# lmb-freiburg/neural-point-cloud-diffusion

Hardware: AMD Instinct MI355X
Metric: denoiser train steps/sec (+ rendered rays/sec under 'render'), SRN-Cars 512pt x 128d (higher is better)
Workload: dtype bf16; 1 GPU; BASELINE configs[1]: denoiser fwd/bwd + AdamW + EMA, 512 points x 128-d latents, width 1024 / 24 layers / 16 heads (seq 513), bf16 autocast; global_batch=64, per_gpu_batch=64, parallelism=dp1, rng=weights seed 1234 on every rank; timestep / noise draws seed 42 + rank

## Files before the change

include/npcd_hip.h:

```cpp
#ifndef NPCD_HIP_H
#define NPCD_HIP_H

#include <assert.h>
#include <stddef.h>
#include <stdint.h>

#ifdef __cplusplus
extern "C" {
#endif

#define NPCD_OK 0
#define NPCD_ERR_ARG (-1)
#define NPCD_ERR_UNSUPPORTED (-2)
#define NPCD_ERR_HIP (-3)

#define NPCD_BF16 0
#define NPCD_F16 1
#define NPCD_F32 2
#define NPCD_F64 3

int npcd_abi_version(void);
const char* npcd_error_string(int code);
const char* npcd_last_hip_error(void);

typedef struct npcd_attn_args {
    const void *q, *k, *v;
    void* out;
    float* lse;
    const void* dout;
    void *dq, *dk, *dv;
    float* delta;
    float* colsum_part;
    void* workspace;
    int64_t qkv_sb, qkv_sn, qkv_sh;
    int64_t out_sb, out_sn, out_sh;
    int64_t g_sb, g_sn, g_sh;
    int32_t B, n, H, d, dtype;
    float scale;
} npcd_attn_args;
static_assert(sizeof(npcd_attn_args) == 192 && offsetof(npcd_attn_args, scale) == 188, "npcd_attn_args is part of the ABI");

int64_t npcd_attn_fwd_workspace_floats(int B, int n, int H);
int npcd_attn_fwd(const npcd_attn_args* a, void* stream);

int64_t npcd_attn_fwd_fp8_workspace_bytes(int B, int n, int H);
int npcd_attn_fwd_fp8(const npcd_attn_args* a, void* stream);

int64_t npcd_attn_bwd_workspace_floats(int B, int n, int H);
int npcd_attn_bwd_colsum_rows(int B, int n, int H);
int npcd_attn_bwd(const npcd_attn_args* a, int passes, void* stream);

int64_t npcd_attn_bwd_fused_slab_floats(int B, int n, int H);
int npcd_attn_bwd_fused(const npcd_attn_args* a, void* stream);

typedef struct npcd_grid_params {
    float voxel_size[3];
    int32_t voxel_scale[3];
    int32_t kernel_size[3];
    int32_t max_points_per_voxel;
    int32_t max_occ_voxels_per_example;
    float range_min[3];
    float range_max[3];
    int32_t dims[3];
    int32_t cdims[3];
    int32_t grid_level;
} npcd_grid_params;
#define NPCD_GRID_FINE 0
#define NPCD_GRID_SCALED 1

int64_t npcd_grid_workspace_bytes(const npcd_grid_params* g, int B, int N);

int npcd_grid_build(const npcd_grid_params* g, const float* points, const int32_t* counts,
                    int B, int N, void* workspace, void* stream);

int npcd_grid_query(const npcd_grid_params* g, const void* workspace, const float* points,
                    int B, int N, int R, int S, int M, int k, float r, int mode,
                    const float* x, const float* rays_o, const float* rays_d,
                    const float* t0, const float* t1,
                    int32_t* sample_idx, float* sample_loc, int32_t* slot_sample, int32_t* nsel,
                    void* stream);

int npcd_grid_query_compact(const npcd_grid_params* g, const void* workspace, const float* points,
                            int B, int N, int R, int S, int M, int k, float r,
                            const float* rays_o, const float* rays_d, const float* t0, const float* t1,
                            int32_t* counter, int32_t capacity, int32_t* ray_base, int32_t* ray_nsel,
                            uint64_t* ray_bits, int32_t* nb_idx, float* pts, void* stream);

int64_t npcd_grid_query_order_ws_bytes(int B, int R, int M, int k);
int npcd_grid_query_compact_ordered(const npcd_grid_params* g, const void* workspace, const float* points,
                                    int B, int N, int R, int S, int M, int k, float r,
                                    const float* rays_o, const float* rays_d, const float* t0, const float* t1,
                                    int32_t* counter, int32_t capacity, int32_t* ray_base, int32_t* ray_nsel,
                                    uint64_t* ray_bits, int32_t* nb_idx, float* pts, void* order_ws, void* stream);

int64_t npcd_ray_gen_ws_floats(int V, int res, int n_ids);
int npcd_ray_gen(const float* extr, const float* intr, int V, int res, float box,
                 float* rays_o, float* rays_d, float* t0, float* t1, float* limits_ws, void* stream);
int npcd_ray_gen_subset(const float* extr, const float* intr, int V, int res, float box, const int32_t* pixel_ids, int n_ids,
                        float* rays_o, float* rays_d, float* t0, float* t1, float* limits_ws, void* stream);

#define NPCD_SHADE_NONFINITE_PAIRS 1
#define NPCD_SHADE_NONFINITE_HEADS 2
int64_t npcd_shade_wpack_bytes(int feat_dim, int n_freqs, int hidden);
int64_t npcd_shade_workspace_bytes(int max_points, int hidden);
int npcd_shade_pack_weights(const float* const* weights_host, const float* const* biases_host,
                            int feat_dim, int n_freqs, int hidden, void* wpack_host);
int npcd_shade_points(const void* wpack, int feat_dim, int n_freqs, int hidden,
                      const int32_t* nb_idx, const float* pts, const float* kp_pos, const float* kp_feat,
                      const int32_t* n_points_dev, int max_points, int k,
                      float* sigma, float* rgb, void* workspace, int32_t* status, void* stream);

int npcd_shade_points_dir(const void* wpack, int feat_dim, int n_freqs, int hidden,
                          const int32_t* nb_idx, const float* pts, const float* kp_pos, const float* kp_feat,
                          const int32_t* n_points_dev, int max_points, int k,
                          float* sigma, float* rgb, void* workspace, const float* dir_bias, const int32_t* point_ray,
                          int32_t* status, void* stream);

int64_t npcd_pairs_x2_wpack_bytes(int feat_dim);
int npcd_pairs_x2_pack(const float* const* weights_host, const float* const* biases_host, int feat_dim, void* wpack_host);
int npcd_pairs_x2(const void* wpack, int feat_dim, const int32_t* nb_idx, const float* pts, const float* kp_pos, const float* kp_feat,
                  const int32_t* n_points_dev, int max_points, int k, float* G, void* stream);
int64_t npcd_points_x2_wpack_bytes(void);
int npcd_points_x2_pack(const float* const* weights_host, const float* const* biases_host, int c0_in_dim, void* wpack_host);
int npcd_points_x2(const void* wpack, const float* feat, const int32_t* n_points_dev, int max_points, float* sigma, float* rgb,
                   const float* dir_bias, const int32_t* point_ray, void* stream);
int npcd_points_x2_train(const void* wpack, const float* feat, int max_points, float* save, float* pre, void* stream);
int npcd_points_x2_pack_dev(const float* const* weights_dev, const float* const* biases_dev, int c0_in_dim, void* wpack_dev, void* stream);

int64_t npcd_ray_march_ws_floats(int Nr);
int npcd_ray_march(const float* sigma, const float* rgb, const uint8_t* slot_valid, const float* slot_loc,
                   const int32_t* point_base, const float* rays_o, const float* rays_d, const float* t1,
                   int Nr, int M, int white_back, float* mask, float* depth, float* channels,
                   float* depth_ws, void* stream);

int npcd_ray_march_bwd(const float* sigma, const float* rgb, const uint8_t* slot_valid, const float* slot_loc,
                       const int32_t* point_base, const float* rays_o, const float* rays_d, const float* t1,
                       int Nr, int M, int white_back, const float* depth_ws, const float* g_mask, const float* g_depth,
                       const float* g_chan, float* dsigma, float* drgb, void* stream);

int npcd_add_ln_fwd_dt(const float* x_in, const void* delta, const float* gamma, const float* beta,
                       float* x_out, void* y, float* mean, float* rstd, int T, int W, float eps, int dtype, void* stream);
int npcd_ln_bwd_blocks(int T);
int npcd_ln_bwd_dt(const void* dy, const float* x, const float* mean, const float* rstd, const float* gamma,
                   const float* dres, float* dx, void* dxb, float* part_gamma, float* part_beta,
                   float* part_col, int T, int W, int dtype, void* stream);
int npcd_colsum_scratch_rows(void);
int npcd_colsum_finalize(const float* part, int nblk, int N, float* out, int accumulate, void* stream);
#define NPCD_COLSUM_MAX_JOBS 8
typedef struct NpcdColsumJob {
    const float* part;
    float* out;
    int nblk, N, accumulate, reserved;
} NpcdColsumJob;
int npcd_colsum_finalize_batch(const NpcdColsumJob* jobs, int njobs, void* stream);
int npcd_gelu_fwd_dt(const void* h, void* g, int64_t numel, int dtype, void* stream);
int npcd_colsum_blocks(int T);
int npcd_gelu_bwd_dt(const void* dg, const void* h, void* dh, float* part, int T, int N, int dtype, void* stream);
int npcd_colsum_dt(const void* a, float* part, int T, int N, int dtype, void* stream);
int npcd_small_wgrad_blocks(int T);
int npcd_small_wgrad(const void* dy, const void* x, float* part, int T, int J, int K, void* stream);
int npcd_adamw_ema_dt(float* p, float* g, float* m, float* v, float* ema, void* shadow, int shadow_dtype, int64_t numel,
                      float lr, float beta1, float beta2, float eps, float weight_decay, int step,
                      float ema_decay, int zero_grad, void* stream);
int npcd_cast_f32_dt(const float* src, void* dst, int64_t numel, int dtype, void* stream);

typedef struct NpcdScalerCtl {
    int32_t found_inf, step, growth_tracker, skipped;
    float loss_scale, inv_scale, grad_norm, clip_coef, bc1, bc2_sqrt;
    int32_t reserved[6];
} NpcdScalerCtl;
int npcd_grad_stats_blocks(void);
int npcd_grad_stats(const float* g, int64_t n, double* work, double* out, void* stream);
int npcd_scaler_finalize(const double* stats, int nslots, NpcdScalerCtl* ctl, int scaling, int clip, float max_norm,
                         float beta1, float beta2, float growth_factor, float backoff_factor, int growth_interval, void* stream);
int npcd_adamw_ema_gated(float* p, float* g, float* m, float* v, float* ema, void* shadow, int shadow_dtype, int64_t numel,
                         float lr, float beta1, float beta2, float eps, float weight_decay, double ema_decay, int zero_grad,
                         const NpcdScalerCtl* ctl, void* stream);

int npcd_wgrad_slices(int T, int N, int K);
int npcd_wgrad(const void* dy, const void* x, float* out, float* workspace, int T, int N, int K, int dtype, void* stream);
int npcd_wgrad_group(int count, const void* const* dy, const void* const* x, float* const* out, const int* N, const int* K, int T,
                     int dtype, void* stream);
int npcd_wgrad_group_blocks(int tiles_per_block, int max_products, int products_per_block);

int npcd_linear_fwd(const void* x, const void* w, const void* bias, void* y, int M, int N, int K, int dtype, void* stream);
int npcd_linear_gelu_fwd(const void* x, const void* w, const void* bias, void* h, void* g, int M, int N, int K, int dtype, void* stream);
int npcd_linear_dgelu_rows(int M);
int npcd_linear_dgelu_bwd(const void* dy, const void* wt, const void* h, void* dh, float* part, int M, int N, int K, int dtype, void* stream);
int npcd_linear128_fwd(const void* x, const void* w, const void* bias, void* y, int M, int N, int K, int dtype, void* stream);
int npcd_transpose_16(const void* in, void* out, int R, int C, void* stream);
int npcd_transpose16_group(int count, const void* const* in, void* const* out, const int* R, const int* C, void* stream);

int npcd_sum_slices(const float* part, float* out, int S, int64_t numel, void* stream);

int npcd_ddpm_reverse_step(const float* x_t, const void* eps, int eps_dtype, const float* noise, float* x_prev, float* x0_out,
                           const int64_t* t, int B, int64_t per_sample, const float* tab_recip, const float* tab_recipm1,
                           const float* tab_coef1, const float* tab_coef2, const float* tab_logvar, float clip_lo, float clip_hi,
                           int has_clip, void* stream);

#define NPCD_SAMPLER_REVERSE 0
#define NPCD_SAMPLER_HOLD 1
typedef struct NpcdSamplerTensor {
    const float* x_t;
    const void* eps;
    const float* noise;
    const float* known;
    float* out;
    float* x0_out;
    int64_t per_sample;
    float clip_lo, clip_hi;
    int32_t has_clip, mode, eps_dtype, reserved;
} NpcdSamplerTensor;
int npcd_sampler_step(const NpcdSamplerTensor* coords, const NpcdSamplerTensor* feats, const int64_t* t, const float* table, int T,
                      int B, int deterministic, void* stream);

int npcd_sampler_step_keep(const NpcdSamplerTensor* coords, const NpcdSamplerTensor* feats, const uint8_t* keep_coords,
                           const uint8_t* keep_feats, int64_t n_points, const int64_t* t, const float* table, int T, int B,
                           int deterministic, void* stream);

int npcd_sampler_step_multistep(const NpcdSamplerTensor* coords, const NpcdSamplerTensor* feats, float* hist_coords, float* hist_feats,
                                const uint8_t* keep_coords, const uint8_t* keep_feats, int64_t n_points, const int64_t* t,
                                const float* table, int T, int B, void* stream);

int npcd_q_sample(const float* x0, const float* noise, const int64_t* t, const float* tab_sqrt_acp, const float* tab_sqrt_1macp,
                  float* x_t, int B, int64_t per_sample, void* stream);
int npcd_eps_mse_blocks(void);
int npcd_eps_mse_fwd(const float* noise, const void* eps, int eps_dtype, int64_t numel, float* pointwise, float* part, float* loss,
                     void* stream);
int npcd_eps_mse_bwd(const float* noise, const void* eps, int eps_dtype, int64_t numel, const float* upstream_dev, void* grad,
                     void* stream);

int npcd_ray_march_compact(const float* sigma, const float* rgb, const uint64_t* ray_bits, const float* pts,
                           const int32_t* ray_base, const float* rays_o, const float* rays_d, const float* t1,
                           int Nr, int M, int capacity, int white_back, float* mask, float* depth, float* channels,
                           float* depth_ws, void* stream);

int64_t npcd_render_lim_words(int B, int R);
int npcd_render_rays_query(const npcd_grid_params* grid, const void* workspace, const float* points, int B, int N, const float* extr,
                           const float* intr, int views, int res, float box, int S, int M, int k, float r, float* rays_o, float* rays_d,
                           float* t0, float* t1, int32_t* counter, int32_t capacity, int32_t* ray_base, int32_t* ray_nsel,
                           uint64_t* ray_bits, int32_t* nb_idx, float* pts, void* order_ws, uint32_t* lim_part, void* stream);
int npcd_ray_march_compact_fused(const float* sigma, const float* rgb, const uint64_t* ray_bits, const float* pts, const int32_t* ray_base,
                                 const float* rays_o, const float* rays_d, const float* t0, const float* t1, const uint32_t* lim_part,
                                 int lim_pairs, int Nr, int M, int capacity, int white_back, float* mask, float* depth,
                                 float* channels, float* depth_ws, void* stream);

int npcd_pair_input_fwd(const int64_t* flat, const int64_t* owner, const float* pts, const float* kp_pos, const float* kp_feat,
                        int feat_dim, int n_freqs, int64_t n_pairs, float* x0, float* w, void* stream);
int npcd_pair_input_bwd(const int64_t* flat, const float* dx0, int feat_dim, int n_cols, int64_t n_pairs, float* dfeat, void* stream);
int npcd_leaky_bwd_blocks(int64_t rows);
int npcd_leaky_bwd_colsum(const void* dz, const void* z, void* dy, float* part, int64_t rows, int N, float slope, int dtype,
                          void* stream);
int npcd_pair_aggregate(int backward, const float* src, const float* w, const int64_t* off, const int64_t* cnt, int channels,
                        int64_t n_points, float* dst, void* stream);

#define NPCD_PAIR_MLP_BF16 0
#define NPCD_PAIR_MLP_X2 1
int64_t npcd_pair_mlp_wpack_bytes(int feat_dim, int precision);
int npcd_pair_mlp_pack(const float* const* weights_dev, const float* const* biases_dev, int feat_dim, int precision, void* wpack_dev,
                       void* stream);
int npcd_pair_mlp_fwd(const void* wpack, int feat_dim, int precision, const int64_t* nb_idx, const float* pts, const float* kp_pos,
                      const float* kp_feat, const int64_t* off, int64_t n_points, int k, int64_t n_pairs, void* x0, void* acts,
                      float* wn, float* G, void* stream);
int npcd_pair_mlp_bwd_slabs(int64_t n_pairs, int precision);
int64_t npcd_pair_mlp_bwd_workspace_floats(int feat_dim, int64_t n_pairs, int precision);
int npcd_pair_mlp_bwd(const void* wpack, int feat_dim, int precision, const float* dG, const int64_t* owner, const float* wn,
                      const void* x0, const void* acts, int64_t n_pairs, void* dact, float* dfeat, float* part, float* const* dW,
                      float* const* db, void* stream);

int npcd_split3_bf16(const float* x, const float* bias, void* out, int64_t rows, int K, int gelu, void* stream);
int npcd_add_ln_split3_bf16(const float* x, const float* o, const float* bias, const float* gamma, const float* beta, float* xnew,
                            void* out, int64_t rows, int W, float eps, void* stream);

#define NPCD_SPLIT_WEIGHTS_MAX 8
typedef struct NpcdSplitWeight {
    const float* w;
    void* fwd;
    void* dgrad;
    int N, K;
} NpcdSplitWeight;
int npcd_add_ln_split3_stats_bf16(const float* x, const float* o, const float* bias, const float* gamma, const float* beta, float* xnew,
                                  void* out, float* mean, float* rstd, int64_t rows, int W, float eps, void* stream);
int npcd_split_weights_bf16(const NpcdSplitWeight* desc, int count, void* stream);
int npcd_ln_bwd_split3_bf16(const float* dy, const float* x, const float* mean, const float* rstd, const float* gamma,
                            const float* dres, float* dx, void* dx3, float* part_gamma, float* part_beta, float* part_col, int T, int W,
                            void* stream);
int npcd_split3_colsum_bf16(const float* a, const float* h, const float* bias, void* out, float* part, int T, int N, int gelu,
                            void* stream);

int64_t npcd_stage1_reg_workspace_floats(int B);
int npcd_stage1_reg_fwd(const float* coords, const int32_t* nb, int64_t nb_ld, const float* feats, int64_t feats_ld, const float* mean,
                        const float* log_var, int64_t kl_ld, int B, int N, int k, int F, float weight_tv, float weight_kl, int dtype,
                        float* tv_pointwise, float* tv_total, float* kl_pointwise, float* kl_total, float* workspace, void* stream);
int npcd_stage1_reg_bwd(const float* coords, const int32_t* nb, int64_t nb_ld, const float* feats, int64_t feats_ld, const float* mean,
                        const float* log_var, int64_t kl_ld, int B, int N, int k, int F, float weight_tv, float weight_kl, int dtype,
                        const float* g_tv_total, const float* g_tv_pointwise, const float* g_kl_total, const float* g_kl_pointwise,
                        float* dfeats, float* dmean, float* dlog_var, void* stream);

int npcd_fps_resident_points(void);
int npcd_fps_max_points(void);
int npcd_fps(const float* points, const int32_t* lengths, const int32_t* ks, const int32_t* start, int64_t* idx_out, float* pts_out,
             int N, int P, int Kmax, void* stream);

int npcd_chamfer_max_points(void);
int npcd_chamfer_directed(const float* x, const int32_t* x_len, const float* y, const int32_t* y_len, float* out, int M, int P, int N,
                          int Q, void* stream);

int npcd_emd_max_points(void);
int npcd_emd_directed(const float* x, const int32_t* x_len, const float* y, const int32_t* y_len, float* out, int M, int P, int N, int Q,
                      void* stream);

int npcd_occupancy_max_resolution(void);
int npcd_occupancy_clouds_per_workgroup(int n, int P, int R);
int npcd_occupancy_grid(const float* points, const int32_t* lengths, const float* lattice, const uint8_t* k_lo, const uint8_t* k_hi,
                        int32_t* counts, int32_t* clouds, int32_t* cells, int n, int P, int R, void* stream);

int npcd_image_metrics_tile(int* rows_host, int* cols_host);
int64_t npcd_image_metrics_workspace_bytes(int V, int C, int H, int W, int w);
int npcd_image_metrics(const float* pred, const float* target, int V, int C, int H, int W, int64_t pred_sv, int64_t pred_sc,
                       int64_t pred_sh, int64_t pred_sw, int64_t target_sv, int64_t target_sc, int64_t target_sh, int64_t target_sw,
                       const double* taps, int w, double n, double data_range, double* workspace, double* mse, double* ssim, double* map,
                       void* stream);

int npcd_moments_tile(int* tile_host);
int npcd_moments_max_features(void);
int npcd_moments_update(const void* x, int dtype, int64_t ld, int64_t r0, int64_t r1, int D, const double* shift, double* sum, double* gram,
                        void* stream);
int npcd_moments_finish(const double* sum, const double* gram, const double* shift, int D, int64_t n, double* mean, double* cov,
                        void* stream);
int npcd_kid_tile(int* tile_host);
int64_t npcd_kid_workspace_bytes(int S, int m);
int npcd_kid_subsets(const void* fake, const void* real, int dtype, int Nf, int Nr, int D, int64_t ldf, int64_t ldr, const int32_t* idx_f,
                     const int32_t* idx_r, int S, int m, double* workspace, double* out, void* stream);

int npcd_feature_knn_max_k(void);
int64_t npcd_feature_rows_workspace_bytes(int n, int m, int k, int splits);
int npcd_feature_knn(const void* x, const void* y, int dtype, int n, int m, int D, int64_t ldx, int64_t ldy, int exclude_self, int k,
                     int splits, double* workspace, double* out, void* stream);
int npcd_feature_ball_counts(const void* x, const void* y, int dtype, int n, int m, int D, int64_t ldx, int64_t ldy, const double* rho_y,
                             int splits, double* workspace, int32_t* cnt, double* near, void* stream);

#ifdef __cplusplus
}
#endif
#endif
```

neural-point-cloud-diffusion_amd/csrc/elementwise.hip:

```cpp
#include <math.h>

#include <stdlib.h>

#include "common.h"

namespace npcd {

constexpr int kMaxChunks = 8;

template <class E>
struct V {
    typedef E x4 __attribute__((ext_vector_type(4)));
    typedef E x8 __attribute__((ext_vector_type(8)));
};
template <class X4>
__device__ __forceinline__ f32x4 to_f32(X4 v) { return f32x4{(float)v[0], (float)v[1], (float)v[2], (float)v[3]}; }
template <class E>
__device__ __forceinline__ typename V<E>::x4 from_f32(f32x4 v) { return typename V<E>::x4{(E)v[0], (E)v[1], (E)v[2], (E)v[3]}; }
__device__ __forceinline__ f32x4 bf16x4_to_f32(bf16x4 v) { return to_f32(v); }
__device__ __forceinline__ bf16x4 f32_to_bf16x4(f32x4 v) { return from_f32<__bf16>(v); }

template <class E, int NCH>
__global__ __launch_bounds__(256) void add_ln_fwd_kernel(const float* __restrict__ x_in, const E* __restrict__ delta,
                                                         const float* __restrict__ gamma, const float* __restrict__ beta,
                                                         float* __restrict__ x_out, E* __restrict__ y, float* __restrict__ mean,
                                                         float* __restrict__ rstd, int T, int W, float eps) {
    using e4 = typename V<E>::x4;
    const int lane = threadIdx.x & 63, wave = threadIdx.x >> 6;
    const int NW = gridDim.x * 4;
    int row = blockIdx.x * 4 + wave;
    if (row >= T) return;
    f32x4 gm[NCH], bt[NCH], v[NCH], nx[NCH];
    e4 nd[NCH];
#pragma unroll
    for (int ch = 0; ch < NCH; ++ch) {
        const int c = ch * 256 + lane * 4;
        gm[ch] = bt[ch] = nx[ch] = f32x4{0.f, 0.f, 0.f, 0.f};
        nd[ch] = e4{0, 0, 0, 0};
        if (c < W) {
            gm[ch] = *reinterpret_cast<const f32x4*>(gamma + c);
            bt[ch] = *reinterpret_cast<const f32x4*>(beta + c);
        }
    }
    auto load_row = [&](int r) {
        const int64_t base = (int64_t)r * W;
#pragma unroll
        for (int ch = 0; ch < NCH; ++ch) {
            const int c = ch * 256 + lane * 4;
            if (c < W) {
                nx[ch] = *reinterpret_cast<const f32x4*>(x_in + base + c);
                if (delta) nd[ch] = *reinterpret_cast<const e4*>(delta + base + c);
            }
        }
    };
    load_row(row);
    for (; row < T; row += NW) {
        const int64_t base = (int64_t)row * W;
        float s = 0.f;
#pragma unroll
        for (int ch = 0; ch < NCH; ++ch) {
            v[ch] = nx[ch];
            if (delta) v[ch] += to_f32(nd[ch]);
        }
        if (row + NW < T) load_row(row + NW);
#pragma unroll
        for (int ch = 0; ch < NCH; ++ch) {
            const int c = ch * 256 + lane * 4;
            if (c < W) {
                if (x_out) *reinterpret_cast<f32x4*>(x_out + base + c) = v[ch];
                s += (v[ch][0] + v[ch][1]) + (v[ch][2] + v[ch][3]);
            }
        }
        const float mu = wave_sum64(s) / (float)W;
        float q = 0.f;
#pragma unroll
        for (int ch = 0; ch < NCH; ++ch) {
            const int c = ch * 256 + lane * 4;
            if (c < W) {
                const f32x4 d = v[ch] - mu;
                q += (d[0] * d[0] + d[1] * d[1]) + (d[2] * d[2] + d[3] * d[3]);
            }
        }
        const float rs = rsqrtf(wave_sum64(q) / (float)W + eps);
#pragma unroll
        for (int ch = 0; ch < NCH; ++ch) {
            const int c = ch * 256 + lane * 4;
            if (c < W) *reinterpret_cast<e4*>(y + base + c) = from_f32<E>((v[ch] - mu) * rs * gm[ch] + bt[ch]);
        }
        if (lane == 0) {
            mean[row] = mu;
            rstd[row] = rs;
        }
    }
}

static inline int ln_rows_per_wave(int T) {
    const int one_round = (T + 4 * 512 - 1) / (4 * 512);
    if (one_round <= 32) return one_round < 1 ? 1 : one_round;
    return 16;
}

template <class E, int NCH, class D = E, bool SPLIT = false>
__global__ __launch_bounds__(256, 2) void ln_bwd_kernel(const D* __restrict__ dy, const float* __restrict__ x, const float* __restrict__ mean,
                                                     const float* __restrict__ rstd, const float* __restrict__ gamma,
                                                     const float* __restrict__ dres, float* __restrict__ dx, E* __restrict__ dxb,
                                                     float* __restrict__ part_gamma, float* __restrict__ part_beta,
                                                     float* __restrict__ part_col, int T, int W, int rows_per_wave) {
    using e4 = typename V<D>::x4;
    extern __shared__ __attribute__((aligned(16))) unsigned char dsmem[];
    float* red = reinterpret_cast<float*>(dsmem);
    const int lane = threadIdx.x & 63, wave = threadIdx.x >> 6;
    f32x4 ag[NCH], ab[NCH], ac[NCH];
#pragma unroll
    for (int ch = 0; ch < NCH; ++ch) ag[ch] = ab[ch] = ac[ch] = f32x4{0.f, 0.f, 0.f, 0.f};
    const int row0 = blockIdx.x * 4 + wave, NW = gridDim.x * 4;
    const int nrows = row0 < T ? min(rows_per_wave, (T - row0 + NW - 1) / NW) : 0;
    e4 dyA[NCH], dyB[NCH];
    f32x4 xA[NCH], xB[NCH], rA[NCH], rB[NCH];
    float muA = 0.f, rsA = 0.f, muB = 0.f, rsB = 0.f;
    auto load_row = [&](int row, e4 (&dyr)[NCH], f32x4 (&xr)[NCH], f32x4 (&rr2)[NCH], float& mu, float& rs) {
        const int64_t base = (int64_t)row * W;
        mu = mean[row];
        rs = rstd[row];
#pragma unroll
        for (int ch = 0; ch < NCH; ++ch) {
            const int c = ch * 256 + lane * 4;
            if (c < W) {
                dyr[ch] = *reinterpret_cast<const e4*>(dy + base + c);
                xr[ch] = *reinterpret_cast<const f32x4*>(x + base + c);
                if (dres) rr2[ch] = *reinterpret_cast<const f32x4*>(dres + base + c);
            }
        }
    };
    if (nrows > 0) load_row(row0, dyA, xA, rA, muA, rsA);
    for (int rr = 0; rr < nrows; ++rr) {
        const int row = row0 + rr * NW;
        const int64_t base = (int64_t)row * W;
        if (rr + 1 < nrows) load_row(row + NW, dyB, xB, rB, muB, rsB);
        const float mu = muA, rs = rsA;
        f32x4 gy[NCH], xh[NCH];
        float s1 = 0.f, s2 = 0.f;
#pragma unroll
        for (int ch = 0; ch < NCH; ++ch) {
            const int c = ch * 256 + lane * 4;
            gy[ch] = xh[ch] = f32x4{0.f, 0.f, 0.f, 0.f};
            if (c < W) {
                const f32x4 d = to_f32(dyA[ch]);
                xh[ch] = (xA[ch] - mu) * rs;
                ag[ch] += d * xh[ch];
                ab[ch] += d;
                gy[ch] = d * *reinterpret_cast<const f32x4*>(gamma + c);
                const f32x4 t = gy[ch] * xh[ch];
                s1 += (gy[ch][0] + gy[ch][1]) + (gy[ch][2] + gy[ch][3]);
                s2 += (t[0] + t[1]) + (t[2] + t[3]);
            }
        }
        const float c1 = wave_sum64(s1) / (float)W, c2 = wave_sum64(s2) / (float)W;
#pragma unroll
        for (int ch = 0; ch < NCH; ++ch) {
            const int c = ch * 256 + lane * 4;
            if (c < W) {
                f32x4 o = (gy[ch] - c1 - xh[ch] * c2) * rs;
                if (dres) o += rA[ch];
                *reinterpret_cast<f32x4*>(dx + base + c) = o;
                if (SPLIT && dxb) {
                    bf16x4 hi, lo;
#pragma unroll
                    for (int j = 0; j < 4; ++j) {
                        hi[j] = (__bf16)o[j];
                        lo[j] = (__bf16)(o[j] - (float)hi[j]);
                    }
                    __bf16* o3 = reinterpret_cast<__bf16*>(dxb) + 3 * base + c;
                    *reinterpret_cast<bf16x4*>(o3) = hi;
                    *reinterpret_cast<bf16x4*>(o3 + W) = lo;
                    *reinterpret_cast<bf16x4*>(o3 + 2 * W) = hi;
                } else if (dxb) {
                    *reinterpret_cast<typename V<E>::x4*>(dxb + base + c) = from_f32<E>(o);
                }
                ac[ch] += o;
            }
        }
#pragma unroll
        for (int ch = 0; ch < NCH; ++ch) {
            dyA[ch] = dyB[ch];
            xA[ch] = xB[ch];
            rA[ch] = rB[ch];
        }
        muA = muB;
        rsA = rsB;
    }
#pragma unroll
    for (int ch = 0; ch < NCH; ++ch) {
        const int c = ch * 256 + lane * 4;
        if (c < W) {
            *reinterpret_cast<f32x4*>(red + (0 * 4 + wave) * W + c) = ag[ch];
            *reinterpret_cast<f32x4*>(red + (1 * 4 + wave) * W + c) = ab[ch];
            *reinterpret_cast<f32x4*>(red + (2 * 4 + wave) * W + c) = ac[ch];
        }
    }
    __syncthreads();
    float* outs[3] = {part_gamma, part_beta, part_col};
    for (int q = 0; q < 3; ++q) {
        if (!outs[q]) continue;
        for (int c = threadIdx.x; c < W; c += 256) {
            const float* p = red + q * 4 * W + c;
            outs[q][(int64_t)blockIdx.x * W + c] = (p[0] + p[W]) + (p[2 * W] + p[3 * W]);
        }
    }
}

constexpr int kFinSlices = 16;

struct FinBatch {
    NpcdColsumJob job[NPCD_COLSUM_MAX_JOBS];
    int first1[NPCD_COLSUM_MAX_JOBS + 1];
    int first2[NPCD_COLSUM_MAX_JOBS + 1];
    int njobs;
};
__device__ __forceinline__ int fin_job(const int* first, int njobs, int bx) {
    int j = 0;
    while (j + 1 < njobs && bx >= first[j + 1]) ++j;
    return j;
}
__device__ __forceinline__ bool fin_two_stage(int nblk) { return nblk > 2 * kFinSlices; }

__global__ __launch_bounds__(256) void colsum_stage1_kernel(FinBatch fb) {
    __shared__ float red[4][64];
    const int j = fin_job(fb.first1, fb.njobs, blockIdx.x);
    const float* __restrict__ part = fb.job[j].part;
    const int nblk = fb.job[j].nblk, N = fb.job[j].N;
    if (!fin_two_stage(nblk)) return;
    float* __restrict__ stage = const_cast<float*>(part) + (int64_t)nblk * N;
    const int tx = threadIdx.x & 63, ty = threadIdx.x >> 6;
    const int c = (blockIdx.x - fb.first1[j]) * 64 + tx;
    const int per = (nblk + kFinSlices - 1) / kFinSlices;
    const int b0 = blockIdx.y * per, b1 = min(nblk, b0 + per);
    float s0 = 0.f, s1 = 0.f;
    if (c < N) {
        int b = b0 + ty;
        for (; b + 4 < b1; b += 8) {
            s0 += part[(int64_t)b * N + c];
            s1 += part[(int64_t)(b + 4) * N + c];
        }
        if (b < b1) s0 += part[(int64_t)b * N + c];
    }
    red[ty][tx] = s0 + s1;
    __syncthreads();
    if (ty == 0 && c < N) stage[(int64_t)blockIdx.y * N + c] = (red[0][tx] + red[1][tx]) + (red[2][tx] + red[3][tx]);
}

__global__ __launch_bounds__(256) void colsum_stage2_kernel(FinBatch fb) {
    const int j = fin_job(fb.first2, fb.njobs, blockIdx.x);
    const int nblk = fb.job[j].nblk, N = fb.job[j].N;
    const int c = (blockIdx.x - fb.first2[j]) * 256 + threadIdx.x;
    if (c >= N) return;
    const bool two = fin_two_stage(nblk);
    const float* __restrict__ src = two ? fb.job[j].part + (int64_t)nblk * N : fb.job[j].part;
    const int nrows = two ? kFinSlices : nblk;
    float s = 0.f;
    for (int k = 0; k < nrows; ++k) s += src[(int64_t)k * N + c];
    float* __restrict__ out = fb.job[j].out;
    out[c] = fb.job[j].accumulate ? out[c] + s : s;
}

__device__ __forceinline__ float gelu_f(float x) { return 0.5f * x * (1.f + erff(x * 0.70710678118654752f)); }
__device__ __forceinline__ float gelu_grad_f(float x) {
    return 0.5f * (1.f + erff(x * 0.70710678118654752f)) + x * 0.3989422804014327f * __expf(-0.5f * x * x);
}

__device__ __forceinline__ float gelu_fast(float x) {
    const float u = fabsf(x) * 0.70710678118654752f;
    const float t = __builtin_amdgcn_rcpf(__builtin_fmaf(0.3275911f, u, 1.f));
    const float e = __builtin_amdgcn_exp2f(x * x * -0.72134752044448170f);
    float poly = __builtin_fmaf(t, 1.061405429f, -1.453152027f);
    poly = __builtin_fmaf(poly, t, 1.421413741f);
    poly = __builtin_fmaf(poly, t, -0.284496736f);
    poly = __builtin_fmaf(poly, t, 0.254829592f);
    const float erf_abs = __builtin_fmaf(-poly * t, e, 1.f);
    return x * __builtin_fmaf(0.5f, copysignf(erf_abs, x), 0.5f);
}

template <class E, int VARIANT>
__global__ __launch_bounds__(256) void gelu_fwd_kernel(const typename V<E>::x8* __restrict__ h, typename V<E>::x8* __restrict__ g, int64_t n8) {
    using e8 = typename V<E>::x8;
    for (int64_t i = (int64_t)blockIdx.x * 256 + threadIdx.x; i < n8; i += (int64_t)gridDim.x * 256) {
        const e8 v = h[i];
        e8 o;
#pragma unroll
        for (int j = 0; j < 8; ++j) o[j] = (E)(VARIANT == 0 ? gelu_f((float)v[j]) : gelu_fast((float)v[j]));
        g[i] = o;
    }
}

static inline int col_rows(int T) {
    static const int forced = [] { const char* e = getenv("NPCD_COL_ROWS"); return e ? atoi(e) : 0; }();
    if (forced > 0) return forced;
    int r = T / 512;
    return r < 8 ? 8 : (r > 64 ? 64 : r);
}

__device__ __forceinline__ float gelu_grad_fast(float x) {
    const float u = fabsf(x) * 0.70710678118654752f;
    const float t = __builtin_amdgcn_rcpf(__builtin_fmaf(0.3275911f, u, 1.f));
    const float e = __builtin_amdgcn_exp2f(x * x * -0.72134752044448170f);
    float poly = __builtin_fmaf(t, 1.061405429f, -1.453152027f);
    poly = __builtin_fmaf(poly, t, 1.421413741f);
    poly = __builtin_fmaf(poly, t, -0.284496736f);
    poly = __builtin_fmaf(poly, t, 0.254829592f);
    const float erf_abs = __builtin_fmaf(-poly * t, e, 1.f);
    const float phi_cdf = __builtin_fmaf(0.5f, copysignf(erf_abs, x), 0.5f);
    return __builtin_fmaf(x * 0.3989422804014327f, e, phi_cdf);
}

template <class E, bool GELU, int VARIANT = 1>
__global__ __launch_bounds__(256) void colsum_kernel(const E* __restrict__ a, const E* __restrict__ hpre, E* __restrict__ out,
                                                     float* __restrict__ part, int T, int N, int rows) {
    using e8 = typename V<E>::x8;
    const int col = (blockIdx.x * 256 + threadIdx.x) * 8;
    if (col >= N) return;
    float acc[8];
#pragma unroll
    for (int j = 0; j < 8; ++j) acc[j] = 0.f;
    auto one = [&](const e8 v, const e8 hp, int64_t off) {
        e8 o;
#pragma unroll
        for (int j = 0; j < 8; ++j) {
            const float gp = VARIANT == 0 ? gelu_grad_f((float)hp[j]) : gelu_grad_fast((float)hp[j]);
            o[j] = (E)((float)v[j] * gp);
            acc[j] += (float)o[j];
        }
        *reinterpret_cast<e8*>(out + off) = o;
    };
    if (GELU && VARIANT == 2) {
        int rr = 0;
        for (; rr + 1 < rows; rr += 2) {
            const int r0 = rr * gridDim.y + blockIdx.y, r1 = r0 + gridDim.y;
            if (r1 >= T) break;
            const int64_t o0 = (int64_t)r0 * N + col, o1 = (int64_t)r1 * N + col;
            const e8 v0 = *reinterpret_cast<const e8*>(a + o0), h0 = *reinterpret_cast<const e8*>(hpre + o0);
            const e8 v1 = *reinterpret_cast<const e8*>(a + o1), h1 = *reinterpret_cast<const e8*>(hpre + o1);
            one(v0, h0, o0);
            one(v1, h1, o1);
        }
        for (; rr < rows; ++rr) {
            const int row = rr * gridDim.y + blockIdx.y;
            if (row >= T) break;
            const int64_t off = (int64_t)row * N + col;
            one(*reinterpret_cast<const e8*>(a + off), *reinterpret_cast<const e8*>(hpre + off), off);
        }
    } else {
        for (int rr = 0; rr < rows; ++rr) {
            const int row = rr * gridDim.y + blockIdx.y;
            if (row >= T) break;
            const int64_t off = (int64_t)row * N + col;
            const e8 v = (GELU && VARIANT == 3) ? __builtin_nontemporal_load(reinterpret_cast<const e8*>(a + off))
                                                    : *reinterpret_cast<const e8*>(a + off);
            if (GELU) {
                one(v, VARIANT == 3 ? __builtin_nontemporal_load(reinterpret_cast<const e8*>(hpre + off))
                                    : *reinterpret_cast<const e8*>(hpre + off), off);
            } else {
#pragma unroll
                for (int j = 0; j < 8; ++j) acc[j] += (float)v[j];
            }
        }
    }
    float* p = part + (int64_t)blockIdx.y * N + col;
    *reinterpret_cast<f32x4*>(p) = f32x4{acc[0], acc[1], acc[2], acc[3]};
    *reinterpret_cast<f32x4*>(p + 4) = f32x4{acc[4], acc[5], acc[6], acc[7]};
}

template <int J>
__global__ __launch_bounds__(256) void small_wgrad_kernel(const __bf16* __restrict__ dy, const __bf16* __restrict__ x, float* __restrict__ part,
                                                          int T, int K, int rows_per_block) {
    extern __shared__ float swg_red[];
    const int chunks = K >> 3, lanes = 256 / chunks;
    const int cc = threadIdx.x % chunks, rl = threadIdx.x / chunks;
    const int row0 = blockIdx.x * rows_per_block, row1 = min(T, row0 + rows_per_block);
    float acc[J][8];
#pragma unroll
    for (int j = 0; j < J; ++j)
#pragma unroll
        for (int i = 0; i < 8; ++i) acc[j][i] = 0.f;
    for (int row = row0 + rl; row < row1; row += lanes) {
        const bf16x8 v = *reinterpret_cast<const bf16x8*>(x + (int64_t)row * K + 8 * cc);
        float w[J];
#pragma unroll
        for (int j = 0; j < J; ++j) w[j] = (float)dy[(int64_t)row * J + j];
#pragma unroll
        for (int j = 0; j < J; ++j)
#pragma unroll
            for (int i = 0; i < 8; ++i) acc[j][i] = __builtin_fmaf(w[j], (float)v[i], acc[j][i]);
    }
#pragma unroll
    for (int j = 0; j < J; ++j)
#pragma unroll
        for (int i = 0; i < 8; ++i) swg_red[(rl * J + j) * K + 8 * cc + i] = acc[j][i];
    __syncthreads();
    for (int e = threadIdx.x; e < J * K; e += 256) {
        float sum = 0.f;
        for (int r2 = 0; r2 < lanes; ++r2) sum += swg_red[r2 * J * K + e];
        part[(int64_t)blockIdx.x * J * K + e] = sum;
    }
}

struct AdamArgs {
    float lr, beta1, beta2, eps, wd, bc1, bc2_sqrt, ema_w;
};

__device__ __forceinline__ void adamw_one(f32x4& pp, const f32x4 gg, f32x4& mm, f32x4& vv, const AdamArgs& a) {
    pp *= (1.f - a.lr * a.wd);
    mm = mm * a.beta1 + gg * (1.f - a.beta1);
    vv = vv * a.beta2 + gg * gg * (1.f - a.beta2);
    const float step = a.lr / a.bc1;
#pragma unroll
    for (int j = 0; j < 4; ++j) pp[j] -= step * (mm[j] / (sqrtf(vv[j]) / a.bc2_sqrt + a.eps));
}

template <class E, bool GATED>
__device__ __forceinline__ void adamw_ema_body(f32x4* __restrict__ p, f32x4* __restrict__ g, f32x4* __restrict__ m, f32x4* __restrict__ v,
                                               f32x4* __restrict__ ema, typename V<E>::x4* __restrict__ shadow, int64_t n4, AdamArgs a,
                                               int zero_grad, const NpcdScalerCtl* __restrict__ ctl, float skip_ema_w) {
    const int64_t stride = (int64_t)gridDim.x * 256;
    int64_t i = (int64_t)blockIdx.x * 256 + threadIdx.x;
    float gs = 1.f, gc = 1.f;
    if constexpr (GATED) {
        if (ctl->found_inf) {
            for (; i < n4; i += stride) {
                if (ema) {
                    const f32x4 e = ema[i], pp = p[i];
                    ema[i] = e + (pp - e) * skip_ema_w;
                }
                if (zero_grad) g[i] = f32x4{0.f, 0.f, 0.f, 0.f};
            }
            return;
        }
        gs = ctl->inv_scale;
        gc = ctl->clip_coef;
        a.bc1 = ctl->bc1;
        a.bc2_sqrt = ctl->bc2_sqrt;
    }
    auto grad = [&](f32x4 x) -> f32x4 {
        if constexpr (GATED) {
            x = (x * gs) * gc;
            asm volatile("" : "+v"(x));
        }
        return x;
    };
    for (; i + stride < n4; i += 2 * stride) {
        const int64_t k = i + stride;
        f32x4 p0 = p[i], p1 = p[k];
        const f32x4 g0 = grad(g[i]), g1 = grad(g[k]);
        f32x4 m0 = m[i], m1 = m[k], v0 = v[i], v1 = v[k];
        f32x4 e0 = {0.f, 0.f, 0.f, 0.f}, e1 = e0;
        if (ema) { e0 = ema[i]; e1 = ema[k]; }
        adamw_one(p0, g0, m0, v0, a);
        adamw_one(p1, g1, m1, v1, a);
        p[i] = p0; p[k] = p1;
        m[i] = m0; m[k] = m1;
        v[i] = v0; v[k] = v1;
        if (ema) { ema[i] = e0 + (p0 - e0) * a.ema_w; ema[k] = e1 + (p1 - e1) * a.ema_w; }
        if (shadow) { shadow[i] = from_f32<E>(p0); shadow[k] = from_f32<E>(p1); }
        if (zero_grad) { g[i] = f32x4{0.f, 0.f, 0.f, 0.f}; g[k] = f32x4{0.f, 0.f, 0.f, 0.f}; }
    }
    if (i < n4) {
        f32x4 pp = p[i];
        const f32x4 gg = grad(g[i]);
        f32x4 mm = m[i], vv = v[i];
        adamw_one(pp, gg, mm, vv, a);
        p[i] = pp;
        m[i] = mm;
        v[i] = vv;
        if (ema) {
            const f32x4 e = ema[i];
            ema[i] = e + (pp - e) * a.ema_w;
        }
        if (shadow) shadow[i] = from_f32<E>(pp);
        if (zero_grad) g[i] = f32x4{0.f, 0.f, 0.f, 0.f};
    }
}

template <class E>
__global__ __launch_bounds__(256) void adamw_ema_kernel(f32x4* __restrict__ p, f32x4* __restrict__ g, f32x4* __restrict__ m, f32x4* __restrict__ v,
                                                        f32x4* __restrict__ ema, typename V<E>::x4* __restrict__ shadow, int64_t n4, AdamArgs a, int zero_grad) {
    adamw_ema_body<E, false>(p, g, m, v, ema, shadow, n4, a, zero_grad, nullptr, 0.f);
}
template <class E>
__global__ __launch_bounds__(256) void adamw_ema_gated_kernel(f32x4* __restrict__ p, f32x4* __restrict__ g, f32x4* __restrict__ m,
                                                              f32x4* __restrict__ v, f32x4* __restrict__ ema, typename V<E>::x4* __restrict__ shadow,
                                                              int64_t n4, AdamArgs a, int zero_grad, const NpcdScalerCtl* __restrict__ ctl,
                                                              float skip_ema_w) {
    adamw_ema_body<E, true>(p, g, m, v, ema, shadow, n4, a, zero_grad, ctl, skip_ema_w);
}

constexpr int kStatBlocks = 512;

__device__ __forceinline__ void stat_one(float x, double& s, uint32_t& bad) {
    const bool ok = fabsf(x) <= 3.402823466e38f;
    const double d = ok ? (double)x : 0.0;
    s = fma(d, d, s);
    bad += ok ? 0u : 1u;
}
__device__ __forceinline__ void stat_four(f32x4 x, double& s, uint32_t& bad) {
#pragma unroll
    for (int j = 0; j < 4; ++j) stat_one(x[j], s, bad);
}
__device__ __forceinline__ double wave_sum_f64(double x) {
#pragma unroll
    for (int off = 32; off > 0; off >>= 1) x += __shfl_xor(x, off, 64);
    return x;
}
__device__ __forceinline__ void block_sum2(double& s, double& c) {
    __shared__ double red[2][4];
    s = wave_sum_f64(s);
    c = wave_sum_f64(c);
    if ((threadIdx.x & 63) == 0) { red[0][threadIdx.x >> 6] = s; red[1][threadIdx.x >> 6] = c; }
    __syncthreads();
    s = (red[0][0] + red[0][1]) + (red[0][2] + red[0][3]);
    c = (red[1][0] + red[1][1]) + (red[1][2] + red[1][3]);
}

__global__ __launch_bounds__(256) void grad_stats_kernel(const float* __restrict__ g, int64_t n, double* __restrict__ part) {
    const f32x4* g4 = reinterpret_cast<const f32x4*>(g);
    const int64_t n4 = n / 4, stride = (int64_t)gridDim.x * 256, gid = (int64_t)blockIdx.x * 256 + threadIdx.x;
    double s = 0.0;
    uint32_t bad = 0;
    int64_t i = gid;
    for (; i + stride < n4; i += 2 * stride) {
        const f32x4 x0 = g4[i], x1 = g4[i + stride];
        stat_four(x0, s, bad);
        stat_four(x1, s, bad);
    }
    if (i < n4) stat_four(g4[i], s, bad);
    if (gid < n - 4 * n4) stat_one(g[4 * n4 + gid], s, bad);
    double c = (double)bad;
    block_sum2(s, c);
    if (threadIdx.x == 0) { part[2 * blockIdx.x] = s; part[2 * blockIdx.x + 1] = c; }
}
__global__ __launch_bounds__(256) void grad_stats_sum_kernel(const double* __restrict__ part, int nblk, double* __restrict__ out) {
    double s = 0.0, c = 0.0;
    for (int b = threadIdx.x; b < nblk; b += 256) { s += part[2 * b]; c += part[2 * b + 1]; }
    block_sum2(s, c);
    if (threadIdx.x == 0) { out[0] = s; out[1] = c; }
}

__global__ __launch_bounds__(64) void scaler_finalize_kernel(const double* __restrict__ stats, int nslots, NpcdScalerCtl* __restrict__ ctl,
                                                             int scaling, int clip, float max_norm, float beta1, float beta2, float growth,
                                                             float backoff, int interval) {
    if (threadIdx.x != 0) return;
    double sumsq = 0.0, bad = 0.0;
    for (int k = 0; k < nslots; ++k) { sumsq += stats[2 * k]; bad += stats[2 * k + 1]; }
    NpcdScalerCtl c = *ctl;
    const float inv = scaling ? 1.f / c.loss_scale : 1.f;
    c.inv_scale = inv;
    c.found_inf = (scaling && bad > 0.0) ? 1 : 0;
    const float norm = bad > 0.0 ? INFINITY : (float)(sqrt(sumsq) * (double)inv);
    c.grad_norm = norm;
    c.clip_coef = clip ? fminf((1.f / (norm + 1e-6f)) * max_norm, 1.f) : 1.f;
    if (c.found_inf) {
        c.loss_scale *= backoff;
        c.growth_tracker = 0;
        c.skipped += 1;
    } else {
        c.step += 1;
// ... 106 lines not shown
        for (int64_t i = (int64_t)blockIdx.x * 256 + threadIdx.x; i < n4; i += (int64_t)gridDim.x * 256) {
            const f32x4 kn = reinterpret_cast<const f32x4*>(known)[i], z = reinterpret_cast<const f32x4*>(noise)[i];
            f32x4 o;
#pragma unroll
            for (int q = 0; q < 4; ++q) o[q] = __builtin_fmaf(k.h1, kn[q], k.h2 * z[q]);
            reinterpret_cast<f32x4*>(out)[i] = o;
        }
    } else {
        for (int64_t i = (int64_t)blockIdx.x * 256 + threadIdx.x; i < a.per_sample; i += (int64_t)gridDim.x * 256)
            out[i] = __builtin_fmaf(k.h1, known[i], k.h2 * noise[i]);
    }
}

__device__ __forceinline__ SamplerCoef sampler_coef(const int64_t* __restrict__ t, const float* __restrict__ table, int T, int b) {
    const int64_t ts = t[b];
    const float nan = __builtin_nanf("");
    SamplerCoef k{nan, nan, nan, nan, nan, nan, nan};
    if (ts >= 0 && ts < T) {
        const f32x4 lo = reinterpret_cast<const f32x4*>(table)[2 * ts], hi = reinterpret_cast<const f32x4*>(table)[2 * ts + 1];
        k = SamplerCoef{lo[0], lo[1], lo[2], lo[3], hi[0], hi[1], hi[2]};
    }
    return k;
}

__device__ __forceinline__ void sampler_by_mode(const NpcdSamplerTensor& a, int vec, const SamplerCoef& k, int64_t base) {
    if (a.mode == NPCD_SAMPLER_HOLD) {
        if (vec) sampler_hold<true>(a, k, base);
        else sampler_hold<false>(a, k, base);
    } else if (a.eps_dtype == NPCD_F32) {
        if (vec) sampler_reverse<float, true>(a, k, base);
        else sampler_reverse<float, false>(a, k, base);
    } else {
        if (vec) sampler_reverse<__bf16, true>(a, k, base);
        else sampler_reverse<__bf16, false>(a, k, base);
    }
}

__global__ __launch_bounds__(256) void sampler_step_kernel(SamplerArgs args, const int64_t* __restrict__ t, const float* __restrict__ table, int T) {
    const int z = blockIdx.z, b = blockIdx.y;
    const NpcdSamplerTensor& a = args.tz[z];
    sampler_by_mode(a, args.vec[z], sampler_coef(t, table, T, b), (int64_t)b * a.per_sample);
}

__device__ __forceinline__ int64_t sampler_col(int64_t i, int64_t n) {
    return ((uint64_t)(i | n) >> 32) == 0 ? (int64_t)((uint32_t)i % (uint32_t)n) : i % n;
}

template <class EPS, bool VEC>
__device__ __forceinline__ void sampler_keep(const NpcdSamplerTensor& a, const uint8_t* __restrict__ keep, int64_t n_points, int det,
                                             const SamplerCoef& k, int64_t base) {
    const float* __restrict__ x_t = a.x_t + base;
    const EPS* __restrict__ eps = static_cast<const EPS*>(a.eps) + base;
    const float* __restrict__ noise = a.noise + base;
    const float* __restrict__ known = a.known + base;
    float* __restrict__ out = a.out + base;
    float* __restrict__ x0_out = a.x0_out ? a.x0_out + base : nullptr;
    if constexpr (VEC) {
        const int64_t n4 = a.per_sample / 4, row4 = n_points / 4;
        for (int64_t i = (int64_t)blockIdx.x * 256 + threadIdx.x; i < n4; i += (int64_t)gridDim.x * 256) {
            const uint32_t m = reinterpret_cast<const uint32_t*>(keep)[sampler_col(i, row4)];
            const f32x4 x = reinterpret_cast<const f32x4*>(x_t)[i];
            const f32x4 e = to_f32(reinterpret_cast<const typename V<EPS>::x4*>(eps)[i]);
            const f32x4 z = reinterpret_cast<const f32x4*>(noise)[i], kn = reinterpret_cast<const f32x4*>(known)[i];
            f32x4 x0, o;
#pragma unroll
            for (int q = 0; q < 4; ++q) {
                const float f0 = sampler_x0(k, x[q], e[q], a.has_clip, a.clip_lo, a.clip_hi);
                float fo = __builtin_fmaf(k.c1, f0, k.c2 * x[q]);
                if (!det) fo = __builtin_fmaf(k.s, z[q], fo);
                const bool kept = ((m >> (8 * q)) & 0xffu) != 0;
                x0[q] = kept ? kn[q] : f0;
                o[q] = kept ? __builtin_fmaf(k.h1, kn[q], k.h2 * z[q]) : fo;
            }
            if (x0_out) reinterpret_cast<f32x4*>(x0_out)[i] = x0;
            reinterpret_cast<f32x4*>(out)[i] = o;
        }
    } else {
        for (int64_t i = (int64_t)blockIdx.x * 256 + threadIdx.x; i < a.per_sample; i += (int64_t)gridDim.x * 256) {
            const bool kept = keep[sampler_col(i, n_points)] != 0;
            const float x = x_t[i], z = noise[i], kn = known[i];
            const float f0 = sampler_x0(k, x, (float)eps[i], a.has_clip, a.clip_lo, a.clip_hi);
            float fo = __builtin_fmaf(k.c1, f0, k.c2 * x);
            if (!det) fo = __builtin_fmaf(k.s, z, fo);
            if (x0_out) x0_out[i] = kept ? kn : f0;
            out[i] = kept ? __builtin_fmaf(k.h1, kn, k.h2 * z) : fo;
        }
    }
}

struct SamplerKeepArgs {
    NpcdSamplerTensor tz[2];
    const uint8_t* keep[2];
    int64_t n_points;
    int vec[2];
    int det;
};

__global__ __launch_bounds__(256) void sampler_step_keep_kernel(SamplerKeepArgs args, const int64_t* __restrict__ t, const float* __restrict__ table,
                                                                int T) {
    const int z = blockIdx.z, b = blockIdx.y;
    const NpcdSamplerTensor& a = args.tz[z];
    const int vec = args.vec[z];
    const SamplerCoef k = sampler_coef(t, table, T, b);
    const int64_t base = (int64_t)b * a.per_sample;
    if (!args.keep[z]) {
        sampler_by_mode(a, vec, k, base);
        return;
    }
    const uint8_t* keep = args.keep[z] + (int64_t)b * args.n_points;
    if (a.eps_dtype == NPCD_F32) {
        if (vec) sampler_keep<float, true>(a, keep, args.n_points, args.det, k, base);
        else sampler_keep<float, false>(a, keep, args.n_points, args.det, k, base);
    } else {
        if (vec) sampler_keep<__bf16, true>(a, keep, args.n_points, args.det, k, base);
        else sampler_keep<__bf16, false>(a, keep, args.n_points, args.det, k, base);
    }
}

__device__ __forceinline__ float sampler_multistep_d(float w, float x0, float h) { return __builtin_fmaf(w, x0 - h, x0); }

template <class EPS, bool VEC, bool KEEP>
__device__ __forceinline__ void sampler_multistep(const NpcdSamplerTensor& a, float* __restrict__ hist, const uint8_t* __restrict__ keep,
                                                  int64_t n_points, const SamplerCoef& k, float w, int64_t base) {
    const float* __restrict__ x_t = a.x_t + base;
    const EPS* __restrict__ eps = static_cast<const EPS*>(a.eps) + base;
    const float* __restrict__ noise = KEEP ? a.noise + base : nullptr;
    const float* __restrict__ known = KEEP ? a.known + base : nullptr;
    float* __restrict__ out = a.out + base;
    float* __restrict__ x0_out = a.x0_out ? a.x0_out + base : nullptr;
    hist += base;
    const bool first_order = w == 0.f;
    if constexpr (VEC) {
        const int64_t n4 = a.per_sample / 4, row4 = KEEP ? n_points / 4 : 1;
        for (int64_t i = (int64_t)blockIdx.x * 256 + threadIdx.x; i < n4; i += (int64_t)gridDim.x * 256) {
            const f32x4 x = reinterpret_cast<const f32x4*>(x_t)[i];
            const f32x4 e = to_f32(reinterpret_cast<const typename V<EPS>::x4*>(eps)[i]);
            f32x4 h = f32x4{0.f, 0.f, 0.f, 0.f}, z = h, kn = h;
            if (!first_order) h = reinterpret_cast<const f32x4*>(hist)[i];
            uint32_t m = 0;
            if constexpr (KEEP) {
                m = reinterpret_cast<const uint32_t*>(keep)[sampler_col(i, row4)];
                z = reinterpret_cast<const f32x4*>(noise)[i];
                kn = reinterpret_cast<const f32x4*>(known)[i];
            }
            f32x4 x0, o;
#pragma unroll
            for (int q = 0; q < 4; ++q) {
                const float f0 = sampler_x0(k, x[q], e[q], a.has_clip, a.clip_lo, a.clip_hi);
                const float d = first_order ? f0 : sampler_multistep_d(w, f0, h[q]);
                const float fo = __builtin_fmaf(k.c1, d, k.c2 * x[q]);
                const bool kept = KEEP && ((m >> (8 * q)) & 0xffu) != 0;
                x0[q] = kept ? kn[q] : f0;
                o[q] = kept ? __builtin_fmaf(k.h1, kn[q], k.h2 * z[q]) : fo;
            }
            if (x0_out) reinterpret_cast<f32x4*>(x0_out)[i] = x0;
            reinterpret_cast<f32x4*>(hist)[i] = x0;
            reinterpret_cast<f32x4*>(out)[i] = o;
        }
    } else {
        for (int64_t i = (int64_t)blockIdx.x * 256 + threadIdx.x; i < a.per_sample; i += (int64_t)gridDim.x * 256) {
            const float x = x_t[i];
            const float f0 = sampler_x0(k, x, (float)eps[i], a.has_clip, a.clip_lo, a.clip_hi);
            const float d = first_order ? f0 : sampler_multistep_d(w, f0, hist[i]);
            float o = __builtin_fmaf(k.c1, d, k.c2 * x), x0 = f0;
            if constexpr (KEEP) {
                if (keep[sampler_col(i, n_points)] != 0) {
                    x0 = known[i];
                    o = __builtin_fmaf(k.h1, x0, k.h2 * noise[i]);
                }
            }
            if (x0_out) x0_out[i] = x0;
            hist[i] = x0;
            out[i] = o;
        }
    }
}

struct SamplerMultistepArgs {
    NpcdSamplerTensor tz[2];
    float* hist[2];
    const uint8_t* keep[2];
    int64_t n_points;
    int vec[2];
};

template <class EPS>
__device__ __forceinline__ void sampler_multistep_by_path(const NpcdSamplerTensor& a, float* hist, const uint8_t* keep, int64_t n_points, int vec,
                                                          const SamplerCoef& k, float w, int64_t base) {
    if (keep) {
        if (vec) sampler_multistep<EPS, true, true>(a, hist, keep, n_points, k, w, base);
        else sampler_multistep<EPS, false, true>(a, hist, keep, n_points, k, w, base);
    } else {
        if (vec) sampler_multistep<EPS, true, false>(a, hist, keep, n_points, k, w, base);
        else sampler_multistep<EPS, false, false>(a, hist, keep, n_points, k, w, base);
    }
}

__global__ __launch_bounds__(256) void sampler_step_multistep_kernel(SamplerMultistepArgs args, const int64_t* __restrict__ t,
                                                                     const float* __restrict__ table, int T) {
    const int z = blockIdx.z, b = blockIdx.y;
    const NpcdSamplerTensor& a = args.tz[z];
    const SamplerCoef k = sampler_coef(t, table, T, b);
    const int64_t base = (int64_t)b * a.per_sample;
    if (!args.keep[z] && a.mode == NPCD_SAMPLER_HOLD) {
        if (args.vec[z]) sampler_hold<true>(a, k, base);
        else sampler_hold<false>(a, k, base);
        return;
    }
    const int64_t ts = t[b];
    const float w = (ts >= 0 && ts < T) ? table[8 * ts + 7] : __builtin_nanf("");
    const uint8_t* keep = args.keep[z] ? args.keep[z] + (int64_t)b * args.n_points : nullptr;
    if (a.eps_dtype == NPCD_F32) sampler_multistep_by_path<float>(a, args.hist[z], keep, args.n_points, args.vec[z], k, w, base);
    else sampler_multistep_by_path<__bf16>(a, args.hist[z], keep, args.n_points, args.vec[z], k, w, base);
}

static bool al16(const void* p) { return (reinterpret_cast<uintptr_t>(p) & 15) == 0; }

}

using namespace npcd;

static inline int ln_fwd_blocks(int T) { const int b = (T + 3) / 4; return b < 2048 ? b : 2048; }

static inline bool dt16(int dtype) { return dtype == NPCD_BF16 || dtype == NPCD_F16; }

extern "C" int npcd_add_ln_fwd_dt(const float* x_in, const void* delta, const float* gamma, const float* beta, float* x_out, void* y,
                                  float* mean, float* rstd, int T, int W, float eps, int dtype, void* stream) {
    if (!x_in || !gamma || !beta || !y || !mean || !rstd || T <= 0 || W <= 0) return NPCD_ERR_ARG;
    if (W % 4 != 0 || W > 256 * kMaxChunks || !dt16(dtype)) return NPCD_ERR_UNSUPPORTED;
    if (!al16(x_in) || !al16(gamma) || !al16(beta) || (x_out && !al16(x_out)) || (reinterpret_cast<uintptr_t>(y) & 7) ||
        (delta && (reinterpret_cast<uintptr_t>(delta) & 7)))
        return NPCD_ERR_ARG;
#define NPCD_LAUNCH_LN_FWD(E, NCH)                                                                                            \
    hipLaunchKernelGGL((add_ln_fwd_kernel<E, NCH>), dim3(ln_fwd_blocks(T)), dim3(256), 0, static_cast<hipStream_t>(stream), x_in, \
                       static_cast<const E*>(delta), gamma, beta, x_out, static_cast<E*>(y), mean, rstd, T, W, eps)
#define NPCD_LN_FWD_W(E)                     \
    do {                                     \
        if (W <= 256) NPCD_LAUNCH_LN_FWD(E, 1);      \
        else if (W <= 512) NPCD_LAUNCH_LN_FWD(E, 2); \
        else if (W <= 1024) NPCD_LAUNCH_LN_FWD(E, 4);\
        else NPCD_LAUNCH_LN_FWD(E, 8);               \
    } while (0)
    if (dtype == NPCD_BF16) NPCD_LN_FWD_W(__bf16);
    else NPCD_LN_FWD_W(_Float16);
#undef NPCD_LN_FWD_W
#undef NPCD_LAUNCH_LN_FWD
    NPCD_HIP_CHECK(hipGetLastError());
    return NPCD_OK;
}

extern "C" int npcd_ln_bwd_blocks(int T) { const int r = ln_rows_per_wave(T); return (T + 4 * r - 1) / (4 * r); }

extern "C" int npcd_ln_bwd_dt(const void* dy, const float* x, const float* mean, const float* rstd, const float* gamma, const float* dres,
                              float* dx, void* dxb, float* part_gamma, float* part_beta, float* part_col, int T, int W, int dtype, void* stream) {
    if (!dy || !x || !mean || !rstd || !gamma || !dx || T <= 0 || W <= 0) return NPCD_ERR_ARG;
    if (W % 4 != 0 || W > 256 * kMaxChunks || !dt16(dtype)) return NPCD_ERR_UNSUPPORTED;
    if (!al16(x) || !al16(gamma) || !al16(dx) || (dres && !al16(dres))) return NPCD_ERR_ARG;
    const int nblk = npcd_ln_bwd_blocks(T);
    const size_t lds = (size_t)3 * 4 * W * sizeof(float);
    hipStream_t st = static_cast<hipStream_t>(stream);
    static DynLds lds_attr_b, lds_attr_h;
    if (dtype == NPCD_BF16) NPCD_HIP_CHECK(lds_attr_b.ensure(reinterpret_cast<const void*>(ln_bwd_kernel<__bf16, 8>), 3 * 4 * 2048 * 4));
    else NPCD_HIP_CHECK(lds_attr_h.ensure(reinterpret_cast<const void*>(ln_bwd_kernel<_Float16, 8>), 3 * 4 * 2048 * 4));
#define NPCD_LAUNCH_LN_BWD(E, NCH)                                                                                             \
    hipLaunchKernelGGL((ln_bwd_kernel<E, NCH>), dim3(nblk), dim3(256), lds, st, static_cast<const E*>(dy), x, mean, rstd, gamma, \
                       dres, dx, static_cast<E*>(dxb), part_gamma, part_beta, part_col, T, W, ln_rows_per_wave(T))
#define NPCD_LN_BWD_W(E)                     \
    do {                                     \
        if (W <= 256) NPCD_LAUNCH_LN_BWD(E, 1);      \
        else if (W <= 512) NPCD_LAUNCH_LN_BWD(E, 2); \
        else if (W <= 1024) NPCD_LAUNCH_LN_BWD(E, 4);\
        else NPCD_LAUNCH_LN_BWD(E, 8);               \
    } while (0)
    if (dtype == NPCD_BF16) NPCD_LN_BWD_W(__bf16);
    else NPCD_LN_BWD_W(_Float16);
#undef NPCD_LN_BWD_W
#undef NPCD_LAUNCH_LN_BWD
    NPCD_HIP_CHECK(hipGetLastError());
    return NPCD_OK;
}
extern "C" int npcd_ln_bwd_split3_bf16(const float* dy, const float* x, const float* mean, const float* rstd, const float* gamma,
                                       const float* dres, float* dx, void* dx3, float* part_gamma, float* part_beta, float* part_col, int T,
                                       int W, void* stream) {
    if (!dy || !x || !mean || !rstd || !gamma || !dx || T <= 0 || W <= 0) return NPCD_ERR_ARG;
    if (W % 4 != 0 || W > 256 * kMaxChunks) return NPCD_ERR_UNSUPPORTED;
    if (!al16(dy) || !al16(x) || !al16(gamma) || !al16(dx) || (dres && !al16(dres)) || (dx3 && !al16(dx3))) return NPCD_ERR_ARG;
    const int nblk = npcd_ln_bwd_blocks(T);
    const size_t lds = (size_t)3 * 4 * W * sizeof(float);
    hipStream_t st = static_cast<hipStream_t>(stream);
    static DynLds lds_attr;
    NPCD_HIP_CHECK(lds_attr.ensure(reinterpret_cast<const void*>(ln_bwd_kernel<__bf16, 8, float, true>), 3 * 4 * 2048 * 4));
#define NPCD_LAUNCH_LN_BWD3(NCH)                                                                                                        \
    hipLaunchKernelGGL((ln_bwd_kernel<__bf16, NCH, float, true>), dim3(nblk), dim3(256), lds, st, dy, x, mean, rstd, gamma, dres, dx, \
                       static_cast<__bf16*>(dx3), part_gamma, part_beta, part_col, T, W, ln_rows_per_wave(T))
    if (W <= 256) NPCD_LAUNCH_LN_BWD3(1);
    else if (W <= 512) NPCD_LAUNCH_LN_BWD3(2);
    else if (W <= 1024) NPCD_LAUNCH_LN_BWD3(4);
    else NPCD_LAUNCH_LN_BWD3(8);
#undef NPCD_LAUNCH_LN_BWD3
    NPCD_HIP_CHECK(hipGetLastError());
    return NPCD_OK;
}


__global__ __launch_bounds__(1024) void colsum_onepass_kernel(FinBatch fb) {
    __shared__ float red[16][64];
    const int j = fin_job(fb.first1, fb.njobs, blockIdx.x);
    const float* __restrict__ part = fb.job[j].part;
    const int nblk = fb.job[j].nblk, N = fb.job[j].N;
    const int tx = threadIdx.x & 63, ty = threadIdx.x >> 6;
    const int c = (blockIdx.x - fb.first1[j]) * 64 + tx;
    float s0 = 0.f, s1 = 0.f;
    if (c < N) {
        int b = ty;
        for (; b + 16 < nblk; b += 32) {
            s0 += part[(int64_t)b * N + c];
            s1 += part[(int64_t)(b + 16) * N + c];
        }
        if (b < nblk) s0 += part[(int64_t)b * N + c];
    }
    red[ty][tx] = s0 + s1;
    __syncthreads();
    if (ty == 0 && c < N) {
        float q[4];
#pragma unroll
        for (int g = 0; g < 4; ++g) q[g] = (red[4 * g][tx] + red[4 * g + 1][tx]) + (red[4 * g + 2][tx] + red[4 * g + 3][tx]);
        const float s = (q[0] + q[1]) + (q[2] + q[3]);
        float* __restrict__ out = fb.job[j].out;
        out[c] = fb.job[j].accumulate ? out[c] + s : s;
    }
}

extern "C" int npcd_colsum_scratch_rows(void) { return kFinSlices; }

extern "C" int npcd_colsum_finalize_batch(const NpcdColsumJob* jobs, int njobs, void* stream) {
    if (!jobs || njobs <= 0 || njobs > NPCD_COLSUM_MAX_JOBS) return NPCD_ERR_ARG;
    FinBatch fb;
    fb.njobs = njobs;
    bool any_two_stage = false;
    int n1 = 0, n2 = 0;
    for (int j = 0; j < njobs; ++j) {
        if (!jobs[j].part || !jobs[j].out || jobs[j].nblk <= 0 || jobs[j].N <= 0) return NPCD_ERR_ARG;
        fb.job[j] = jobs[j];
        fb.first1[j] = n1;
        fb.first2[j] = n2;
        n1 += (jobs[j].N + 63) / 64;
        n2 += (jobs[j].N + 255) / 256;
        any_two_stage |= jobs[j].nblk > 2 * kFinSlices;
    }
    for (int j = njobs; j <= NPCD_COLSUM_MAX_JOBS; ++j) { fb.first1[j] = n1; fb.first2[j] = n2; }
    hipStream_t st = static_cast<hipStream_t>(stream);
    static const bool onepass = [] { const char* e = getenv("NPCD_COLSUM_ONEPASS"); return e && atoi(e) > 0; }();
    if (onepass) {
        hipLaunchKernelGGL(colsum_onepass_kernel, dim3(n1), dim3(1024), 0, st, fb);
        NPCD_HIP_CHECK(hipGetLastError());
        return NPCD_OK;
    }
    if (any_two_stage) hipLaunchKernelGGL(colsum_stage1_kernel, dim3(n1, kFinSlices), dim3(256), 0, st, fb);
    hipLaunchKernelGGL(colsum_stage2_kernel, dim3(n2), dim3(256), 0, st, fb);
    NPCD_HIP_CHECK(hipGetLastError());
    return NPCD_OK;
}

extern "C" int npcd_colsum_finalize(const float* part, int nblk, int N, float* out, int accumulate, void* stream) {
    NpcdColsumJob job;
    job.part = part; job.out = out; job.nblk = nblk; job.N = N; job.accumulate = accumulate; job.reserved = 0;
    return npcd_colsum_finalize_batch(&job, 1, stream);
}

extern "C" int npcd_gelu_fwd_dt(const void* h, void* g, int64_t numel, int dtype, void* stream) {
    if (!h || !g || numel <= 0) return NPCD_ERR_ARG;
    if (numel % 8 != 0 || !al16(h) || !al16(g) || !dt16(dtype)) return NPCD_ERR_UNSUPPORTED;
    const int64_t n8 = numel / 8;
    const int grid = (int)((n8 + 255) / 256 < 16384 ? (n8 + 255) / 256 : 16384);
    static const int variant = [] { const char* e = getenv("NPCD_GELU_FWD_VARIANT"); return e ? atoi(e) : 1; }();
    hipStream_t st = static_cast<hipStream_t>(stream);
#define NPCD_LAUNCH_GELU_FWD(E, VV)                                                                                                 \
    hipLaunchKernelGGL((gelu_fwd_kernel<E, VV>), dim3(grid), dim3(256), 0, st, static_cast<const typename V<E>::x8*>(h), \
                       static_cast<typename V<E>::x8*>(g), n8)
    if (dtype == NPCD_BF16) {
        if (variant == 0) NPCD_LAUNCH_GELU_FWD(__bf16, 0);
        else NPCD_LAUNCH_GELU_FWD(__bf16, 1);
    } else {
        NPCD_LAUNCH_GELU_FWD(_Float16, 1);
    }
#undef NPCD_LAUNCH_GELU_FWD
    NPCD_HIP_CHECK(hipGetLastError());
    return NPCD_OK;
}

extern "C" int npcd_colsum_blocks(int T) { const int r = col_rows(T); return (T + r - 1) / r; }

extern "C" int npcd_gelu_bwd_dt(const void* dg, const void* h, void* dh, float* part, int T, int N, int dtype, void* stream) {
    if (!dg || !h || !dh || !part || T <= 0 || N <= 0) return NPCD_ERR_ARG;
    if (N % 8 != 0 || !al16(dg) || !al16(h) || !al16(dh) || !al16(part) || !dt16(dtype)) return NPCD_ERR_UNSUPPORTED;
    dim3 grid((N / 8 + 255) / 256, npcd_colsum_blocks(T));
    static const int variant = [] { const char* e = getenv("NPCD_GELU_BWD_VARIANT"); return e ? atoi(e) : 1; }();
#define NPCD_LAUNCH_GELU_BWD(E, VV)                                                                                                    \
    hipLaunchKernelGGL((colsum_kernel<E, true, VV>), grid, dim3(256), 0, static_cast<hipStream_t>(stream), static_cast<const E*>(dg), \
                       static_cast<const E*>(h), static_cast<E*>(dh), part, T, N, col_rows(T))
    if (dtype == NPCD_F16) NPCD_LAUNCH_GELU_BWD(_Float16, 1);
    else if (variant == 0) NPCD_LAUNCH_GELU_BWD(__bf16, 0);
    else if (variant == 2) NPCD_LAUNCH_GELU_BWD(__bf16, 2);
    else if (variant == 3) NPCD_LAUNCH_GELU_BWD(__bf16, 3);
    else NPCD_LAUNCH_GELU_BWD(__bf16, 1);
#undef NPCD_LAUNCH_GELU_BWD
    NPCD_HIP_CHECK(hipGetLastError());
    return NPCD_OK;
}

extern "C" int npcd_colsum_dt(const void* a, float* part, int T, int N, int dtype, void* stream) {
    if (!a || !part || T <= 0 || N <= 0) return NPCD_ERR_ARG;
    if (N % 8 != 0 || !al16(a) || !al16(part) || !dt16(dtype)) return NPCD_ERR_UNSUPPORTED;
    dim3 grid((N / 8 + 255) / 256, npcd_colsum_blocks(T));
    if (dtype == NPCD_BF16)
        hipLaunchKernelGGL((colsum_kernel<__bf16, false>), grid, dim3(256), 0, static_cast<hipStream_t>(stream), static_cast<const __bf16*>(a),
                           static_cast<const __bf16*>(nullptr), static_cast<__bf16*>(nullptr), part, T, N, col_rows(T));
    else
        hipLaunchKernelGGL((colsum_kernel<_Float16, false>), grid, dim3(256), 0, static_cast<hipStream_t>(stream), static_cast<const _Float16*>(a),
                           static_cast<const _Float16*>(nullptr), static_cast<_Float16*>(nullptr), part, T, N, col_rows(T));
    NPCD_HIP_CHECK(hipGetLastError());
    return NPCD_OK;
}

extern "C" int npcd_small_wgrad_blocks(int T) { return T <= 0 ? -1 : (T + 255) / 256 < 1024 ? (T + 255) / 256 : 1024; }

extern "C" int npcd_small_wgrad(const void* dy, const void* x, float* part, int T, int J, int K, void* stream) {
    if (!dy || !x || !part || T <= 0) return NPCD_ERR_ARG;
    if (J < 1 || J > 4 || K < 64 || K > 2048 || (K & (K - 1)) || !al16(x) || !al16(part)) return NPCD_ERR_UNSUPPORTED;
    const int nblk = npcd_small_wgrad_blocks(T), rpb = (T + nblk - 1) / nblk;
    const size_t lds = (size_t)(256 / (K / 8)) * J * K * sizeof(float);
    hipStream_t st = static_cast<hipStream_t>(stream);
    const __bf16* d = static_cast<const __bf16*>(dy);
    const __bf16* xx = static_cast<const __bf16*>(x);
    switch (J) {
        case 1: hipLaunchKernelGGL(small_wgrad_kernel<1>, dim3(nblk), dim3(256), lds, st, d, xx, part, T, K, rpb); break;
        case 2: hipLaunchKernelGGL(small_wgrad_kernel<2>, dim3(nblk), dim3(256), lds, st, d, xx, part, T, K, rpb); break;
        case 3: hipLaunchKernelGGL(small_wgrad_kernel<3>, dim3(nblk), dim3(256), lds, st, d, xx, part, T, K, rpb); break;
        default: hipLaunchKernelGGL(small_wgrad_kernel<4>, dim3(nblk), dim3(256), lds, st, d, xx, part, T, K, rpb); break;
    }
    NPCD_HIP_CHECK(hipGetLastError());
    return NPCD_OK;
}

extern "C" int npcd_adamw_ema_dt(float* p, float* g, float* m, float* v, float* ema, void* shadow, int shadow_dtype, int64_t numel, float lr,
                                 float beta1, float beta2, float eps, float weight_decay, int step, float ema_decay, int zero_grad, void* stream) {
    if (!p || !g || !m || !v || numel <= 0 || step <= 0) return NPCD_ERR_ARG;
    if (numel % 4 != 0 || !al16(p) || !al16(g) || !al16(m) || !al16(v) || (ema && !al16(ema)) ||
        (shadow && ((reinterpret_cast<uintptr_t>(shadow) & 7) || !dt16(shadow_dtype))))
        return NPCD_ERR_UNSUPPORTED;
    AdamArgs a;
    a.lr = lr; a.beta1 = beta1; a.beta2 = beta2; a.eps = eps; a.wd = weight_decay;
    a.bc1 = (float)(1.0 - pow((double)beta1, (double)step));
    a.bc2_sqrt = (float)sqrt(1.0 - pow((double)beta2, (double)step));
    a.ema_w = 1.f - ema_decay;
    const int64_t n4 = numel / 4;
    const int grid = (int)((n4 + 255) / 256 < 8192 ? (n4 + 255) / 256 : 8192);
    hipStream_t st = static_cast<hipStream_t>(stream);
    if (shadow && shadow_dtype == NPCD_F16)
        hipLaunchKernelGGL(adamw_ema_kernel<_Float16>, dim3(grid), dim3(256), 0, st, reinterpret_cast<f32x4*>(p), reinterpret_cast<f32x4*>(g),
                           reinterpret_cast<f32x4*>(m), reinterpret_cast<f32x4*>(v), reinterpret_cast<f32x4*>(ema),
                           static_cast<V<_Float16>::x4*>(shadow), n4, a, zero_grad);
    else
        hipLaunchKernelGGL(adamw_ema_kernel<__bf16>, dim3(grid), dim3(256), 0, st, reinterpret_cast<f32x4*>(p), reinterpret_cast<f32x4*>(g),
                           reinterpret_cast<f32x4*>(m), reinterpret_cast<f32x4*>(v), reinterpret_cast<f32x4*>(ema),
                           static_cast<V<__bf16>::x4*>(shadow), n4, a, zero_grad);
    NPCD_HIP_CHECK(hipGetLastError());
    return NPCD_OK;
}

extern "C" int npcd_adamw_ema_gated(float* p, float* g, float* m, float* v, float* ema, void* shadow, int shadow_dtype, int64_t numel, float lr,
                                    float beta1, float beta2, float eps, float weight_decay, double ema_decay, int zero_grad,
                                    const NpcdScalerCtl* ctl, void* stream) {
    if (!p || !g || !m || !v || !ctl || numel <= 0) return NPCD_ERR_ARG;
    if (numel % 4 != 0 || !al16(p) || !al16(g) || !al16(m) || !al16(v) || (ema && !al16(ema)) || (reinterpret_cast<uintptr_t>(ctl) & 15) ||
        (shadow && ((reinterpret_cast<uintptr_t>(shadow) & 7) || !dt16(shadow_dtype))))
        return NPCD_ERR_UNSUPPORTED;
    AdamArgs a;
    a.lr = lr; a.beta1 = beta1; a.beta2 = beta2; a.eps = eps; a.wd = weight_decay;
    a.bc1 = 1.f; a.bc2_sqrt = 1.f;
    a.ema_w = 1.f - (float)ema_decay;
    const float skip_w = (float)(1.0 - ema_decay);
    const int64_t n4 = numel / 4;
    const int grid = (int)((n4 + 255) / 256 < 8192 ? (n4 + 255) / 256 : 8192);
    hipStream_t st = static_cast<hipStream_t>(stream);
    if (shadow && shadow_dtype == NPCD_F16)
        hipLaunchKernelGGL(adamw_ema_gated_kernel<_Float16>, dim3(grid), dim3(256), 0, st, reinterpret_cast<f32x4*>(p), reinterpret_cast<f32x4*>(g),
                           reinterpret_cast<f32x4*>(m), reinterpret_cast<f32x4*>(v), reinterpret_cast<f32x4*>(ema),
                           static_cast<V<_Float16>::x4*>(shadow), n4, a, zero_grad, ctl, skip_w);
    else
        hipLaunchKernelGGL(adamw_ema_gated_kernel<__bf16>, dim3(grid), dim3(256), 0, st, reinterpret_cast<f32x4*>(p), reinterpret_cast<f32x4*>(g),
                           reinterpret_cast<f32x4*>(m), reinterpret_cast<f32x4*>(v), reinterpret_cast<f32x4*>(ema),
                           static_cast<V<__bf16>::x4*>(shadow), n4, a, zero_grad, ctl, skip_w);
    NPCD_HIP_CHECK(hipGetLastError());
    return NPCD_OK;
}

extern "C" int npcd_grad_stats_blocks(void) { return kStatBlocks; }

extern "C" int npcd_grad_stats(const float* g, int64_t n, double* work, double* out, void* stream) {
    if (!g || !work || !out || n <= 0) return NPCD_ERR_ARG;
    if (!al16(g) || (reinterpret_cast<uintptr_t>(work) & 7) || (reinterpret_cast<uintptr_t>(out) & 7)) return NPCD_ERR_UNSUPPORTED;
    const int64_t n4 = n / 4, want = (n4 + 511) / 512;
    const int grid = (int)(want < 1 ? 1 : want < kStatBlocks ? want : kStatBlocks);
    hipStream_t st = static_cast<hipStream_t>(stream);
    hipLaunchKernelGGL(grad_stats_kernel, dim3(grid), dim3(256), 0, st, g, n, work);
    hipLaunchKernelGGL(grad_stats_sum_kernel, dim3(1), dim3(256), 0, st, work, grid, out);
    NPCD_HIP_CHECK(hipGetLastError());
    return NPCD_OK;
}

extern "C" int npcd_scaler_finalize(const double* stats, int nslots, NpcdScalerCtl* ctl, int scaling, int clip, float max_norm, float beta1,
                                    float beta2, float growth_factor, float backoff_factor, int growth_interval, void* stream) {
    if (!stats || !ctl || nslots <= 0 || growth_interval <= 0) return NPCD_ERR_ARG;
    if ((reinterpret_cast<uintptr_t>(stats) & 7) || (reinterpret_cast<uintptr_t>(ctl) & 15)) return NPCD_ERR_UNSUPPORTED;
    hipLaunchKernelGGL(scaler_finalize_kernel, dim3(1), dim3(64), 0, static_cast<hipStream_t>(stream), stats, nslots, ctl, scaling, clip, max_norm,
                       beta1, beta2, growth_factor, backoff_factor, growth_interval);
    NPCD_HIP_CHECK(hipGetLastError());
    return NPCD_OK;
}

extern "C" int npcd_ddpm_reverse_step(const float* x_t, const void* eps, int eps_dtype, const float* noise, float* x_prev, float* x0_out,
                                      const int64_t* t, int B, int64_t per_sample, const float* tab_recip, const float* tab_recipm1,
                                      const float* tab_coef1, const float* tab_coef2, const float* tab_logvar, float clip_lo, float clip_hi,
                                      int has_clip, void* stream) {
    if (!x_t || !eps || !noise || !x_prev || !t || B <= 0 || per_sample <= 0) return NPCD_ERR_ARG;
    if (!tab_recip || !tab_recipm1 || !tab_coef1 || !tab_coef2 || !tab_logvar) return NPCD_ERR_ARG;
    if (eps_dtype != NPCD_F32 && eps_dtype != NPCD_BF16) return NPCD_ERR_UNSUPPORTED;
    const DdpmTables tab{tab_recip, tab_recipm1, tab_coef1, tab_coef2, tab_logvar};
    const int gx = (int)((per_sample + 255) / 256 < 1024 ? (per_sample + 255) / 256 : 1024);
    hipStream_t st = static_cast<hipStream_t>(stream);
    if (eps_dtype == NPCD_F32)
        hipLaunchKernelGGL(ddpm_reverse_kernel<float>, dim3(gx, B), dim3(256), 0, st, x_t, static_cast<const float*>(eps), noise, x_prev, x0_out, t,
                           per_sample, tab, clip_lo, clip_hi, has_clip);
    else
        hipLaunchKernelGGL(ddpm_reverse_kernel<__bf16>, dim3(gx, B), dim3(256), 0, st, x_t, static_cast<const __bf16*>(eps), noise, x_prev, x0_out, t,
                           per_sample, tab, clip_lo, clip_hi, has_clip);
    NPCD_HIP_CHECK(hipGetLastError());
    return NPCD_OK;
}

static int sampler_check_mode(const NpcdSamplerTensor& a, int deterministic, bool* vec_out) {
    if (!a.out || a.per_sample <= 0) return NPCD_ERR_ARG;
    bool vec = a.per_sample % 4 == 0 && al16(a.out);
    if (a.mode == NPCD_SAMPLER_HOLD) {
        if (!a.known || !a.noise) return NPCD_ERR_ARG;
        vec = vec && al16(a.known) && al16(a.noise);
    } else if (a.mode == NPCD_SAMPLER_REVERSE) {
        if (!a.x_t || !a.eps || (!a.noise && !deterministic)) return NPCD_ERR_ARG;
        if (a.eps_dtype != NPCD_F32 && a.eps_dtype != NPCD_BF16) return NPCD_ERR_UNSUPPORTED;
        vec = vec && al16(a.x_t) && (!a.noise || al16(a.noise)) && (!a.x0_out || al16(a.x0_out)) &&
              (reinterpret_cast<uintptr_t>(a.eps) & (a.eps_dtype == NPCD_F32 ? 15 : 7)) == 0;
    } else {
        return NPCD_ERR_ARG;
    }
    *vec_out = vec;
    return NPCD_OK;
}

static int sampler_grid(const NpcdSamplerTensor& a, bool vec) {
    const int64_t items = vec ? a.per_sample / 4 : a.per_sample;
    return (int)((items + 255) / 256 < 1024 ? (items + 255) / 256 : 1024);
}

extern "C" int npcd_sampler_step(const NpcdSamplerTensor* coords, const NpcdSamplerTensor* feats, const int64_t* t, const float* table, int T,
                                 int B, int deterministic, void* stream) {
    if (!coords || !feats || !t || !table || T <= 0 || B <= 0) return NPCD_ERR_ARG;
    if (B > 65535 || !al16(table)) return NPCD_ERR_UNSUPPORTED;
    SamplerArgs args;
    int gx = 1;
    for (int z = 0; z < 2; ++z) {
        const NpcdSamplerTensor& a = z ? *feats : *coords;
        bool vec = false;
        const int rc = sampler_check_mode(a, deterministic, &vec);
        if (rc != NPCD_OK) return rc;
        args.tz[z] = a;
        args.vec[z] = vec ? 1 : 0;
        const int g = sampler_grid(a, vec);
        gx = g > gx ? g : gx;
    }
    hipLaunchKernelGGL(sampler_step_kernel, dim3(gx, B, 2), dim3(256), 0, static_cast<hipStream_t>(stream), args, t, table, T);
    NPCD_HIP_CHECK(hipGetLastError());
    return NPCD_OK;
}

extern "C" int npcd_sampler_step_keep(const NpcdSamplerTensor* coords, const NpcdSamplerTensor* feats, const uint8_t* keep_coords,
                                      const uint8_t* keep_feats, int64_t n_points, const int64_t* t, const float* table, int T, int B,
                                      int deterministic, void* stream) {
    if (!coords || !feats || !t || !table || T <= 0 || B <= 0 || n_points <= 0) return NPCD_ERR_ARG;
    if (B > 65535 || !al16(table)) return NPCD_ERR_UNSUPPORTED;
    SamplerKeepArgs args;
    args.n_points = n_points;
    args.det = deterministic ? 1 : 0;
    int gx = 1;
    for (int z = 0; z < 2; ++z) {
        const NpcdSamplerTensor& a = z ? *feats : *coords;
        const uint8_t* keep = z ? keep_feats : keep_coords;
        bool vec = false;
        if (!keep) {
            const int rc = sampler_check_mode(a, deterministic, &vec);
            if (rc != NPCD_OK) return rc;
        } else {
            if (!a.out || !a.x_t || !a.eps || !a.noise || !a.known || a.per_sample <= 0 || a.per_sample % n_points != 0) return NPCD_ERR_ARG;
            if (a.eps_dtype != NPCD_F32 && a.eps_dtype != NPCD_BF16) return NPCD_ERR_UNSUPPORTED;
            vec = n_points % 4 == 0 && (reinterpret_cast<uintptr_t>(keep) & 3) == 0 && al16(a.out) && al16(a.x_t) && al16(a.noise) &&
                  al16(a.known) && (!a.x0_out || al16(a.x0_out)) &&
                  (reinterpret_cast<uintptr_t>(a.eps) & (a.eps_dtype == NPCD_F32 ? 15 : 7)) == 0;
        }
        args.tz[z] = a;
        args.keep[z] = keep;
        args.vec[z] = vec ? 1 : 0;
        const int g = sampler_grid(a, vec);
        gx = g > gx ? g : gx;
    }
    hipLaunchKernelGGL(sampler_step_keep_kernel, dim3(gx, B, 2), dim3(256), 0, static_cast<hipStream_t>(stream), args, t, table, T);
    NPCD_HIP_CHECK(hipGetLastError());
    return NPCD_OK;
}

extern "C" int npcd_sampler_step_multistep(const NpcdSamplerTensor* coords, const NpcdSamplerTensor* feats, float* hist_coords,
                                           float* hist_feats, const uint8_t* keep_coords, const uint8_t* keep_feats, int64_t n_points,
                                           const int64_t* t, const float* table, int T, int B, void* stream) {
    if (!coords || !feats || !t || !table || T <= 0 || B <= 0) return NPCD_ERR_ARG;
    if ((keep_coords || keep_feats) && n_points <= 0) return NPCD_ERR_ARG;
    if (B > 65535 || !al16(table)) return NPCD_ERR_UNSUPPORTED;
    SamplerMultistepArgs args;
    args.n_points = n_points;
    int gx = 1;
    for (int z = 0; z < 2; ++z) {
        const NpcdSamplerTensor& a = z ? *feats : *coords;
        const uint8_t* keep = z ? keep_feats : keep_coords;
        float* hist = z ? hist_feats : hist_coords;
        bool vec = false;
        if (!keep) {
            const int rc = sampler_check_mode(a, 1, &vec);
            if (rc != NPCD_OK) return rc;
        } else {
            if (!a.out || !a.x_t || !a.eps || !a.noise || !a.known || a.per_sample <= 0 || a.per_sample % n_points != 0) return NPCD_ERR_ARG;
            if (a.eps_dtype != NPCD_F32 && a.eps_dtype != NPCD_BF16) return NPCD_ERR_UNSUPPORTED;
            vec = n_points % 4 == 0 && (reinterpret_cast<uintptr_t>(keep) & 3) == 0 && al16(a.out) && al16(a.x_t) && al16(a.noise) &&
                  al16(a.known) && (!a.x0_out || al16(a.x0_out)) &&
                  (reinterpret_cast<uintptr_t>(a.eps) & (a.eps_dtype == NPCD_F32 ? 15 : 7)) == 0;
        }
        if (keep || a.mode != NPCD_SAMPLER_HOLD) {
            if (!hist) return NPCD_ERR_ARG;
            vec = vec && al16(hist);
        }
        args.tz[z] = a;
        args.hist[z] = hist;
        args.keep[z] = keep;
        args.vec[z] = vec ? 1 : 0;
        const int g = sampler_grid(a, vec);
        gx = g > gx ? g : gx;
    }
    hipLaunchKernelGGL(sampler_step_multistep_kernel, dim3(gx, B, 2), dim3(256), 0, static_cast<hipStream_t>(stream), args, t, table, T);
    NPCD_HIP_CHECK(hipGetLastError());
    return NPCD_OK;
}

namespace npcd {
__global__ __launch_bounds__(256) void q_sample_kernel(const float* __restrict__ x0, const float* __restrict__ noise, const int64_t* __restrict__ t,
                                                       const float* __restrict__ tab_a, const float* __restrict__ tab_s, float* __restrict__ xt,
                                                       int64_t per_sample) {
#pragma clang fp contract(off)
    const int b = blockIdx.y;
    const float ca = tab_a[t[b]], cs = tab_s[t[b]];
    const int64_t base = (int64_t)b * per_sample;
    for (int64_t i = (int64_t)blockIdx.x * 256 + threadIdx.x; i < per_sample; i += (int64_t)gridDim.x * 256) {
        const float p0 = ca * x0[base + i], p1 = cs * noise[base + i];
// ... 109 lines not shown
```

neural-point-cloud-diffusion_amd/npcd/hip/__init__.py:

```python
import ctypes
import os
from ctypes import POINTER, c_char_p, c_double, c_float, c_int, c_int32, c_int64, c_void_p

import torch

_PKG_ROOT = os.path.dirname(os.path.dirname(os.path.dirname(os.path.abspath(__file__))))
LIB_PATH = os.environ.get("NPCD_HIP_LIB") or os.path.join(_PKG_ROOT, "lib", "libnpcd_hip.so")

NPCD_BF16, NPCD_F16, NPCD_F32 = 0, 1, 2
NPCD_F64 = 3
NPCD_GRID_FINE, NPCD_GRID_SCALED = 0, 1
_DTYPE_CODE = {torch.bfloat16: NPCD_BF16, torch.float16: NPCD_F16, torch.float32: NPCD_F32}


class GridParams(ctypes.Structure):
    _fields_ = [("voxel_size", c_float * 3), ("voxel_scale", c_int32 * 3), ("kernel_size", c_int32 * 3),
                ("max_points_per_voxel", c_int32), ("max_occ_voxels_per_example", c_int32),
                ("range_min", c_float * 3), ("range_max", c_float * 3), ("dims", c_int32 * 3), ("cdims", c_int32 * 3),
                ("grid_level", c_int32)]


_P = c_void_p
SIGNATURES = {
    "npcd_abi_version": (c_int, []),
    "npcd_error_string": (c_char_p, [c_int]),
    "npcd_last_hip_error": (c_char_p, []),
    "npcd_attn_fwd": (c_int, [_P, _P]),
    "npcd_attn_fwd_workspace_floats": (c_int64, [c_int, c_int, c_int]),
    "npcd_ray_march_bwd": (c_int, [_P] * 8 + [c_int, c_int, c_int] + [_P] * 6 + [_P]),
    "npcd_leaky_bwd_blocks": (c_int, [c_int64]),
    "npcd_leaky_bwd_colsum": (c_int, [_P, _P, _P, _P, c_int64, c_int, c_float, c_int, _P]),
    "npcd_pair_input_fwd": (c_int, [_P] * 5 + [c_int, c_int, c_int64, _P, _P, _P]),
    "npcd_pair_input_bwd": (c_int, [_P, _P, c_int, c_int, c_int64, _P, _P]),
    "npcd_pair_aggregate": (c_int, [c_int, _P, _P, _P, _P, c_int, c_int64, _P, _P]),
    "npcd_attn_bwd": (c_int, [_P, c_int, _P]),
    "npcd_attn_bwd_workspace_floats": (c_int64, [c_int, c_int, c_int]),
    "npcd_attn_bwd_colsum_rows": (c_int, [c_int, c_int, c_int]),
    "npcd_attn_fwd_fp8_workspace_bytes": (c_int64, [c_int, c_int, c_int]),
    "npcd_attn_fwd_fp8": (c_int, [_P, _P]),
    "npcd_attn_bwd_fused_slab_floats": (c_int64, [c_int, c_int, c_int]),
    "npcd_attn_bwd_fused": (c_int, [_P, _P]),
    "npcd_grid_workspace_bytes": (c_int64, [POINTER(GridParams), c_int, c_int]),
    "npcd_grid_build": (c_int, [POINTER(GridParams), _P, _P, c_int, c_int, _P, _P]),
    "npcd_grid_query": (c_int, [POINTER(GridParams), _P, _P] + [c_int] * 6 + [c_float, c_int] + [_P] * 9 + [_P]),
    "npcd_grid_query_compact": (c_int, [POINTER(GridParams), _P, _P] + [c_int] * 6 + [c_float] + [_P] * 5 + [c_int32] + [_P] * 5 + [_P]),
    "npcd_grid_query_compact_ordered": (c_int, [POINTER(GridParams), _P, _P] + [c_int] * 6 + [c_float] + [_P] * 5 + [c_int32] + [_P] * 5
                                        + [_P, _P]),
    "npcd_grid_query_order_ws_bytes": (c_int64, [c_int] * 4),
    "npcd_ray_march_compact": (c_int, [_P] * 8 + [c_int, c_int, c_int, c_int] + [_P] * 4 + [_P]),
    "npcd_render_lim_words": (c_int64, [c_int, c_int]),
    "npcd_render_rays_query": (c_int, [POINTER(GridParams), _P, _P, c_int, c_int, _P, _P, c_int, c_int, c_float, c_int, c_int, c_int, c_float]
                               + [_P] * 5 + [c_int32] + [_P] * 7 + [_P]),
    "npcd_ray_march_compact_fused": (c_int, [_P] * 10 + [c_int, c_int, c_int, c_int, c_int] + [_P] * 4 + [_P]),
    "npcd_ray_gen": (c_int, [_P, _P, c_int, c_int, c_float] + [_P] * 5 + [_P]),
    "npcd_ray_gen_subset": (c_int, [_P, _P, c_int, c_int, c_float, _P, c_int] + [_P] * 5 + [_P]),
    "npcd_shade_wpack_bytes": (c_int64, [c_int, c_int, c_int]),
    "npcd_shade_workspace_bytes": (c_int64, [c_int, c_int]),
    "npcd_shade_pack_weights": (c_int, [POINTER(_P), POINTER(_P), c_int, c_int, c_int, _P]),
    "npcd_pairs_x2_wpack_bytes": (c_int64, [c_int]),
    "npcd_pairs_x2_pack": (c_int, [POINTER(_P), POINTER(_P), c_int, _P]),
    "npcd_pairs_x2": (c_int, [_P, c_int, _P, _P, _P, _P, _P, c_int, c_int, _P, _P]),
    "npcd_points_x2_wpack_bytes": (c_int64, []),
    "npcd_points_x2_pack": (c_int, [POINTER(_P), POINTER(_P), c_int, _P]),
    "npcd_points_x2": (c_int, [_P, _P, _P, c_int, _P, _P, _P, _P, _P]),
    "npcd_points_x2_train": (c_int, [_P, _P, c_int, _P, _P, _P]),
    "npcd_points_x2_pack_dev": (c_int, [POINTER(_P), POINTER(_P), c_int, _P, _P]),
    "npcd_shade_points": (c_int, [_P, c_int, c_int, c_int] + [_P] * 5 + [c_int, c_int] + [_P] * 3 + [_P] + [_P]),
    "npcd_shade_points_dir": (c_int, [_P, c_int, c_int, c_int] + [_P] * 5 + [c_int, c_int] + [_P] * 3 + [_P, _P] + [_P] + [_P]),
    "npcd_ray_march_ws_floats": (c_int64, [c_int]),
    "npcd_ray_gen_ws_floats": (c_int64, [c_int, c_int, c_int]),
    "npcd_ray_march": (c_int, [_P] * 8 + [c_int, c_int, c_int] + [_P] * 4 + [_P]),
    "npcd_ln_bwd_blocks": (c_int, [c_int]),
    "npcd_colsum_scratch_rows": (c_int, []),
    "npcd_colsum_finalize": (c_int, [_P, c_int, c_int, _P, c_int, _P]),
    "npcd_colsum_finalize_batch": (c_int, [_P, c_int, _P]),
    "npcd_ddpm_reverse_step": (c_int, [_P, _P, c_int, _P, _P, _P, _P, c_int, c_int64, _P, _P, _P, _P, _P, c_float, c_float, c_int, _P]),
    "npcd_sampler_step": (c_int, [_P, _P, _P, _P, c_int, c_int, c_int, _P]),
    "npcd_sampler_step_keep": (c_int, [_P, _P, _P, _P, c_int64, _P, _P, c_int, c_int, c_int, _P]),
    "npcd_sampler_step_multistep": (c_int, [_P, _P, _P, _P, _P, _P, c_int64, _P, _P, c_int, c_int, _P]),
    "npcd_colsum_blocks": (c_int, [c_int]),
    "npcd_add_ln_fwd_dt": (c_int, [_P] * 8 + [c_int, c_int, c_float, c_int, _P]),
    "npcd_ln_bwd_dt": (c_int, [_P] * 11 + [c_int, c_int, c_int, _P]),
    "npcd_gelu_fwd_dt": (c_int, [_P, _P, c_int64, c_int, _P]),
    "npcd_gelu_bwd_dt": (c_int, [_P, _P, _P, _P, c_int, c_int, c_int, _P]),
    "npcd_colsum_dt": (c_int, [_P, _P, c_int, c_int, c_int, _P]),
    "npcd_adamw_ema_dt": (c_int, [_P] * 6 + [c_int, c_int64] + [c_float] * 5 + [c_int, c_float, c_int, _P]),
    "npcd_cast_f32_dt": (c_int, [_P, _P, c_int64, c_int, _P]),
    "npcd_grad_stats_blocks": (c_int, []),
    "npcd_grad_stats": (c_int, [_P, c_int64, _P, _P, _P]),
    "npcd_scaler_finalize": (c_int, [_P, c_int, _P, c_int, c_int] + [c_float] * 5 + [c_int, _P]),
    "npcd_adamw_ema_gated": (c_int, [_P] * 6 + [c_int, c_int64] + [c_float] * 5 + [c_double, c_int, _P, _P]),
    "npcd_wgrad_slices": (c_int, [c_int, c_int, c_int]),
    "npcd_wgrad": (c_int, [_P, _P, _P, _P, c_int, c_int, c_int, c_int, _P]),
    "npcd_wgrad_group": (c_int, [c_int, POINTER(_P), POINTER(_P), POINTER(_P), POINTER(c_int), POINTER(c_int), c_int, c_int, _P]),
    "npcd_wgrad_group_blocks": (c_int, [c_int, c_int, c_int]),
    "npcd_sum_slices": (c_int, [_P, _P, c_int, c_int64, _P]),
    "npcd_linear_fwd": (c_int, [_P, _P, _P, _P, c_int, c_int, c_int, c_int, _P]),
    "npcd_linear128_fwd": (c_int, [_P, _P, _P, _P, c_int, c_int, c_int, c_int, _P]),
    "npcd_linear_gelu_fwd": (c_int, [_P, _P, _P, _P, _P, c_int, c_int, c_int, c_int, _P]),
    "npcd_linear_dgelu_rows": (c_int, [c_int]),
    "npcd_linear_dgelu_bwd": (c_int, [_P, _P, _P, _P, _P, c_int, c_int, c_int, c_int, _P]),
    "npcd_transpose_16": (c_int, [_P, _P, c_int, c_int, _P]),
    "npcd_transpose16_group": (c_int, [c_int, POINTER(_P), POINTER(_P), POINTER(c_int), POINTER(c_int), _P]),
    "npcd_small_wgrad_blocks": (c_int, [c_int]),
    "npcd_small_wgrad": (c_int, [_P, _P, _P, c_int, c_int, c_int, _P]),
    "npcd_q_sample": (c_int, [_P] * 6 + [c_int, c_int64, _P]),
    "npcd_eps_mse_blocks": (c_int, []),
    "npcd_eps_mse_fwd": (c_int, [_P, _P, c_int, c_int64, _P, _P, _P, _P]),
    "npcd_eps_mse_bwd": (c_int, [_P, _P, c_int, c_int64, _P, _P, _P]),
    "npcd_split3_bf16": (c_int, [_P, _P, _P, c_int64, c_int, c_int, _P]),
    "npcd_add_ln_split3_bf16": (c_int, [_P] * 7 + [c_int64, c_int, c_float, _P]),
    "npcd_add_ln_split3_stats_bf16": (c_int, [_P] * 9 + [c_int64, c_int, c_float, _P]),
    "npcd_split_weights_bf16": (c_int, [_P, c_int, _P]),
    "npcd_ln_bwd_split3_bf16": (c_int, [_P] * 11 + [c_int, c_int, _P]),
    "npcd_split3_colsum_bf16": (c_int, [_P] * 5 + [c_int, c_int, c_int, _P]),
    "npcd_pair_mlp_wpack_bytes": (c_int64, [c_int, c_int]),
    "npcd_pair_mlp_pack": (c_int, [POINTER(_P), POINTER(_P), c_int, c_int, _P, _P]),
    "npcd_pair_mlp_fwd": (c_int, [_P, c_int, c_int] + [_P] * 5 + [c_int64, c_int, c_int64] + [_P] * 4 + [_P]),
    "npcd_pair_mlp_bwd_slabs": (c_int, [c_int64, c_int]),
    "npcd_pair_mlp_bwd_workspace_floats": (c_int64, [c_int, c_int64, c_int]),
    "npcd_pair_mlp_bwd": (c_int, [_P, c_int, c_int] + [_P] * 5 + [c_int64] + [_P] * 3 + [POINTER(_P), POINTER(_P), _P]),
    "npcd_stage1_reg_workspace_floats": (c_int64, [c_int]),
    "npcd_stage1_reg_fwd": (c_int, [_P, _P, c_int64, _P, c_int64, _P, _P, c_int64] + [c_int] * 4 + [c_float, c_float, c_int] + [_P] * 5 + [_P]),
    "npcd_stage1_reg_bwd": (c_int, [_P, _P, c_int64, _P, c_int64, _P, _P, c_int64] + [c_int] * 4 + [c_float, c_float, c_int] + [_P] * 7 + [_P]),
    "npcd_fps_resident_points": (c_int, []),
    "npcd_fps_max_points": (c_int, []),
    "npcd_fps": (c_int, [_P] * 6 + [c_int, c_int, c_int, _P]),
    "npcd_chamfer_max_points": (c_int, []),
    "npcd_chamfer_directed": (c_int, [_P] * 5 + [c_int] * 4 + [_P]),
    "npcd_emd_max_points": (c_int, []),
    "npcd_emd_directed": (c_int, [_P] * 5 + [c_int] * 4 + [_P]),
    "npcd_occupancy_max_resolution": (c_int, []),
    "npcd_occupancy_clouds_per_workgroup": (c_int, [c_int, c_int, c_int]),
    "npcd_occupancy_grid": (c_int, [_P] * 8 + [c_int] * 3 + [_P]),
    "npcd_image_metrics_tile": (c_int, [POINTER(c_int), POINTER(c_int)]),
    "npcd_image_metrics_workspace_bytes": (c_int64, [c_int] * 5),
    "npcd_image_metrics": (c_int, [_P, _P] + [c_int] * 4 + [c_int64] * 8 + [_P, c_int, c_double, c_double] + [_P] * 4 + [_P]),
    "npcd_moments_tile": (c_int, [POINTER(c_int)]),
    "npcd_moments_max_features": (c_int, []),
    "npcd_moments_update": (c_int, [_P, c_int, c_int64, c_int64, c_int64, c_int, _P, _P, _P, _P]),
    "npcd_moments_finish": (c_int, [_P, _P, _P, c_int, c_int64, _P, _P, _P]),
    "npcd_kid_tile": (c_int, [POINTER(c_int)]),
    "npcd_kid_workspace_bytes": (c_int64, [c_int, c_int]),
    "npcd_kid_subsets": (c_int, [_P, _P, c_int, c_int, c_int, c_int, c_int64, c_int64, _P, _P, c_int, c_int, _P, _P, _P]),
    "npcd_feature_knn_max_k": (c_int, []),
    "npcd_feature_rows_workspace_bytes": (c_int64, [c_int] * 4),
    "npcd_feature_knn": (c_int, [_P, _P, c_int, c_int, c_int, c_int, c_int64, c_int64, c_int, c_int, c_int, _P, _P, _P]),
    "npcd_feature_ball_counts": (c_int, [_P, _P, c_int, c_int, c_int, c_int, c_int64, c_int64, _P, c_int, _P, _P, _P, _P]),
}

_lib = None


def lib() -> ctypes.CDLL:
    global _lib
    if _lib is None:
        if not os.path.exists(LIB_PATH):
            raise RuntimeError(
                f"libnpcd_hip.so not found at {LIB_PATH}: build it with "
                f"`python neural-point-cloud-diffusion_amd/csrc/build.py` (or __graft_entry__.build()). "
                f"There is no CPU / PyTorch fallback for the NPCD hot path.")
        handle = ctypes.CDLL(LIB_PATH)
        missing = []
        for name, (res, args) in SIGNATURES.items():
            try:
                fn = getattr(handle, name)
            except AttributeError:
                missing.append(name)
                continue
            fn.restype, fn.argtypes = res, args
        handle.npcd_missing = tuple(missing)
        _lib = handle
    return _lib


def check(rc: int, what: str):
    if rc != 0:
        L = lib()
        msg = L.npcd_error_string(rc).decode()
        if rc == -3:
            msg += ": " + L.npcd_last_hip_error().decode()
        raise RuntimeError(f"{what} failed: {msg} (code {rc})")


def require_gpu(*tensors: torch.Tensor):
    for t in tensors:
        if t is not None and not t.is_cuda:
            raise RuntimeError("npcd.hip operators need GPU tensors (MI355X); got a tensor on "
                               f"{t.device}. There is no CPU fallback in the product path.")


def dtype_code(t: torch.Tensor) -> int:
    try:
        return _DTYPE_CODE[t.dtype]
    except KeyError:
        raise RuntimeError(f"unsupported dtype {t.dtype}") from None


def ptr(t):
    return c_void_p(0 if t is None else t.data_ptr())


_raw_stream = getattr(torch._C, "_cuda_getCurrentRawStream", None)


def stream_ptr():
    if _raw_stream is not None:
        return c_void_p(_raw_stream(torch.cuda.current_device()))
    return c_void_p(torch.cuda.current_stream().cuda_stream)
```

neural-point-cloud-diffusion_amd/npcd/hip/elementwise.py:

```python
import ctypes

import torch

from . import arena, check, dtype_code, lib, ptr, require_gpu, stream_ptr

_f32, _bf16, _f16 = torch.float32, torch.bfloat16, torch.float16
MAX_JOBS = 8

KERNEL_EVENTS = None


def _timed(tag, fn):
    if KERNEL_EVENTS is None or tag not in KERNEL_EVENTS:
        return fn()
    e0, e1 = torch.cuda.Event(enable_timing=True), torch.cuda.Event(enable_timing=True)
    e0.record()
    rc = fn()
    e1.record()
    KERNEL_EVENTS[tag].append((e0, e1))
    return rc


class ColsumJob(ctypes.Structure):
    _fields_ = [("part", ctypes.c_void_p), ("out", ctypes.c_void_p), ("nblk", ctypes.c_int), ("N", ctypes.c_int),
                ("accumulate", ctypes.c_int), ("reserved", ctypes.c_int)]


class ColsumBatch:

    def __init__(self):
        self.jobs = []

    def add(self, part, nblk, N, out, accumulate=False):
        self.jobs.append((part, nblk, N, out, accumulate))

    def flush(self):
        L, s = lib(), stream_ptr()
        for i in range(0, len(self.jobs), MAX_JOBS):
            chunk = self.jobs[i:i + MAX_JOBS]
            arr = (ColsumJob * len(chunk))()
            for a, (part, nblk, N, out, acc) in zip(arr, chunk):
                a.part, a.out, a.nblk, a.N, a.accumulate, a.reserved = part.data_ptr(), out.data_ptr(), nblk, N, int(acc), 0
            check(L.npcd_colsum_finalize_batch(ctypes.cast(arr, ctypes.c_void_p), len(chunk), s), "npcd_colsum_finalize_batch")
        self.jobs = []


def _finish(batch, part, nblk, N, out):
    if batch is not None:
        batch.add(part, nblk, N, out)
    else:
        check(lib().npcd_colsum_finalize(ptr(part), nblk, N, ptr(out), 0, stream_ptr()), "npcd_colsum_finalize")


def add_ln_fwd(x_in, delta, gamma, beta, eps=1e-5, want_sum=True, dtype=_bf16):
    require_gpu(x_in)
    T, W = x_in.shape
    dev = x_in.device
    if delta is not None:
        dtype = delta.dtype
    x_out = arena.empty_like(x_in) if (delta is not None and want_sum) else None
    y = arena.empty((T, W), dtype, dev)
    mean = arena.empty(T, _f32, dev)
    rstd = arena.empty(T, _f32, dev)
    check(_timed("add_ln_fwd" if delta is not None and want_sum else "ln_fwd",
                 lambda: lib().npcd_add_ln_fwd_dt(ptr(x_in), ptr(delta), ptr(gamma), ptr(beta), ptr(x_out), ptr(y), ptr(mean), ptr(rstd), T, W,
                                                  float(eps), dtype_code(y), stream_ptr())), "npcd_add_ln_fwd")
    return x_out, y, mean, rstd


def ln_bwd(dy, x, mean, rstd, gamma, dres, dgamma_out, dbeta_out, dcol_out=None, want_bf16=True, batch=None):
    T, W = x.shape
    dev = x.device
    L = lib()
    nblk = L.npcd_ln_bwd_blocks(T)
    dx = arena.empty((T, W), _f32, dev)
    dxb = arena.empty((T, W), dy.dtype, dev) if want_bf16 else None
    parts = arena.empty((3, nblk + L.npcd_colsum_scratch_rows(), W), _f32, dev)
    full = dres is not None and want_bf16
    check(_timed("ln_bwd" if full else "ln_bwd_partial",
                 lambda: L.npcd_ln_bwd_dt(ptr(dy), ptr(x), ptr(mean), ptr(rstd), ptr(gamma), ptr(dres), ptr(dx), ptr(dxb), ptr(parts[0]),
                                          ptr(parts[1]), ptr(parts[2]) if dcol_out is not None else ptr(None), T, W, dtype_code(dy), stream_ptr())),
          "npcd_ln_bwd")
    _finish(batch, parts[0], nblk, W, dgamma_out)
    _finish(batch, parts[1], nblk, W, dbeta_out)
    if dcol_out is not None:
        _finish(batch, parts[2], nblk, W, dcol_out)
    return dx, dxb


def gelu_fwd(h):
    g = arena.empty_like(h)
    check(_timed("gelu_fwd", lambda: lib().npcd_gelu_fwd_dt(ptr(h), ptr(g), h.numel(), dtype_code(h), stream_ptr())), "npcd_gelu_fwd")
    return g


def gelu_bwd(dg, h, dbias_out, batch=None, out=None, part_rows=None):
    T, N = h.shape
    L = lib()
    nblk = L.npcd_colsum_blocks(T)
    dh = arena.empty_like(h) if out is None else out
    if part_rows is not None:
        check(_timed("gelu_bwd", lambda: L.npcd_gelu_bwd_dt(ptr(dg), ptr(h), ptr(dh), ptr(part_rows), T, N, dtype_code(h), stream_ptr())), "npcd_gelu_bwd")
        return dh, nblk
    part = arena.empty((nblk + L.npcd_colsum_scratch_rows(), N), _f32, h.device)
    check(_timed("gelu_bwd", lambda: L.npcd_gelu_bwd_dt(ptr(dg), ptr(h), ptr(dh), ptr(part), T, N, dtype_code(h), stream_ptr())), "npcd_gelu_bwd")
    _finish(batch, part, nblk, N, dbias_out)
    return dh


def colsum_bf16(a, out, batch=None):
    T, N = a.shape
    L = lib()
    nblk = L.npcd_colsum_blocks(T)
    part = arena.empty((nblk + L.npcd_colsum_scratch_rows(), N), _f32, a.device)
    check(L.npcd_colsum_dt(ptr(a), ptr(part), T, N, dtype_code(a), stream_ptr()), "npcd_colsum")
    _finish(batch, part, nblk, N, out)
    return out


def adamw_ema(p, g, m, v, ema, shadow, lr, beta1, beta2, eps, weight_decay, step, ema_decay, zero_grad=True):
    require_gpu(p)
    check(lib().npcd_adamw_ema_dt(ptr(p), ptr(g), ptr(m), ptr(v), ptr(ema), ptr(shadow), dtype_code(shadow) if shadow is not None else 0,
                                  p.numel(), float(lr), float(beta1), float(beta2), float(eps), float(weight_decay), int(step),
                                  float(ema_decay if ema_decay is not None else 0.0), int(bool(zero_grad)), stream_ptr()), "npcd_adamw_ema")



CTL_FOUND_INF, CTL_STEP, CTL_GROWTH_TRACKER, CTL_SKIPPED = 0, 1, 2, 3
CTL_LOSS_SCALE, CTL_INV_SCALE, CTL_GRAD_NORM, CTL_CLIP_COEF, CTL_BC1, CTL_BC2_SQRT = 4, 5, 6, 7, 8, 9
CTL_WORDS = 16


def scaler_record(device, loss_scale=1.0, step=0):
    ctl = torch.zeros(CTL_WORDS, dtype=torch.int32, device=device)
    ctl[CTL_STEP] = int(step)
    ctl.view(_f32)[CTL_LOSS_SCALE] = float(loss_scale)
    return ctl


def grad_stats_work(device):
    return torch.empty(2 * lib().npcd_grad_stats_blocks(), dtype=torch.float64, device=device)


def grad_stats(g, out, work):
    require_gpu(g)
    check(lib().npcd_grad_stats(ptr(g), g.numel(), ptr(work), ptr(out), stream_ptr()), "npcd_grad_stats")


def scaler_finalize(stats, nslots, ctl, scaling, max_norm, beta1, beta2, growth_factor=2.0, backoff_factor=0.5, growth_interval=2000):
    check(lib().npcd_scaler_finalize(ptr(stats), int(nslots), ptr(ctl), int(bool(scaling)), int(max_norm is not None),
                                     float(max_norm if max_norm is not None else 0.0), float(beta1), float(beta2), float(growth_factor),
                                     float(backoff_factor), int(growth_interval), stream_ptr()), "npcd_scaler_finalize")


def adamw_ema_gated(p, g, m, v, ema, shadow, lr, beta1, beta2, eps, weight_decay, ema_decay, ctl, zero_grad=True):
    require_gpu(p)
    check(lib().npcd_adamw_ema_gated(ptr(p), ptr(g), ptr(m), ptr(v), ptr(ema), ptr(shadow), dtype_code(shadow) if shadow is not None else 0,
                                     p.numel(), float(lr), float(beta1), float(beta2), float(eps), float(weight_decay),
                                     float(ema_decay if ema_decay is not None else 0.0), int(bool(zero_grad)), ptr(ctl), stream_ptr()),
          "npcd_adamw_ema_gated")

def small_wgrad(dy, x):
    T, J = dy.shape
    K = x.shape[1]
    if not (1 <= J <= 4 and 64 <= K <= 2048 and K & (K - 1) == 0 and dy.dtype == _bf16 and x.dtype == _bf16 and dy.is_contiguous()
            and x.is_contiguous() and T > 0):
        return None
    L = lib()
    nblk = L.npcd_small_wgrad_blocks(T)
    part = arena.empty((nblk + L.npcd_colsum_scratch_rows(), J * K), _f32, x.device)
    out = arena.empty((J, K), _f32, x.device)
    check(L.npcd_small_wgrad(ptr(dy), ptr(x), ptr(part), T, J, K, stream_ptr()), "npcd_small_wgrad")
    check(L.npcd_colsum_finalize(ptr(part), nblk, J * K, ptr(out), 0, stream_ptr()), "npcd_colsum_finalize")
    return out


def wgrad(dy, x, out):
    T, N = dy.shape
    K = x.shape[1]
    if (N % 256 or K % 256 or dy.dtype != x.dtype or dy.dtype not in (_bf16, _f16) or not dy.is_contiguous() or not x.is_contiguous()
            or not out.is_contiguous() or out.dtype != _f32):
        return False
    L = lib()
    S = L.npcd_wgrad_slices(T, N, K)
    ws = arena.empty((S, N, K), _f32, dy.device) if S > 1 else None
    check(L.npcd_wgrad(ptr(dy), ptr(x), ptr(out), ptr(ws), T, N, K, dtype_code(dy), stream_ptr()), "npcd_wgrad")
    return True


WGRAD_GROUP_MAX = 16


def wgrad_group(triples):
    import ctypes
    n = len(triples)
    if not 1 <= n <= WGRAD_GROUP_MAX:
        return False
    T, dt = triples[0][0].shape[0], triples[0][0].dtype
    for dy, x, out in triples:
        if (dy.shape[0] != T or x.shape[0] != T or dy.dtype != dt or x.dtype != dt or dt not in (_bf16, _f16) or dy.shape[1] % 256 or x.shape[1] % 256
                or not dy.is_contiguous() or not x.is_contiguous() or not out.is_contiguous() or out.dtype != _f32
                or tuple(out.shape) != (dy.shape[1], x.shape[1])):
            return False
    if len({t[2].data_ptr() for t in triples}) != n:
        return False
    P = ctypes.c_void_p * n
    I = ctypes.c_int * n
    check(lib().npcd_wgrad_group(n, P(*[ptr(t[0]) for t in triples]), P(*[ptr(t[1]) for t in triples]), P(*[ptr(t[2]) for t in triples]),
                                 I(*[t[0].shape[1] for t in triples]), I(*[t[1].shape[1] for t in triples]), T, dtype_code(triples[0][0]), stream_ptr()),
          "npcd_wgrad_group")
    return True


def wgrad_group_blocks_rule(tiles_per_block, max_products, products_per_block, cus):
    if tiles_per_block <= 0 or products_per_block <= 0 or cus <= 0:
        return 0
    G = 1
    while G * products_per_block <= max_products:
        tiles = G * tiles_per_block
        rounds = -(-tiles // cus)
        if tiles * 100 >= rounds * cus * 95:
            return G
        G += 1
    return 0


def wgrad_group_blocks(shapes):
    if not shapes or any(N % 256 or K % 256 for N, K in shapes):
        return 0
    return int(lib().npcd_wgrad_group_blocks(sum((N // 256) * (K // 256) for N, K in shapes), WGRAD_GROUP_MAX, len(shapes)))


def sum_slices(part, out):
    S, n = part.shape[0], out.numel()
    if S not in (2, 4, 8) or n % 4 or not part.is_contiguous() or not out.is_contiguous() or part.dtype != _f32 or out.dtype != _f32:
        return False
    check(lib().npcd_sum_slices(ptr(part), ptr(out), S, n, stream_ptr()), "npcd_sum_slices")
    return True


def cast_f32_bf16(src, dst):
    check(lib().npcd_cast_f32_dt(ptr(src), ptr(dst), src.numel(), dtype_code(dst), stream_ptr()), "npcd_cast_f32")
    return dst


def split3(x, bias=None, gelu=False):
    require_gpu(x)
    x = x.contiguous()
    T, K = x.shape
    out = arena.empty((T, 3 * K), torch.bfloat16, x.device)
    b = None if bias is None else bias.to(torch.float32).contiguous()
    check(lib().npcd_split3_bf16(ptr(x), ptr(b), ptr(out), T, K, 1 if gelu else 0, stream_ptr()), "npcd_split3_bf16")
    return out


def add_ln_split3(x, gamma, beta, o=None, bias=None, eps=1e-5):
    require_gpu(x)
    T, W = x.shape
    if W % 256 or W // 256 not in (1, 2, 3, 4, 8, 16):
        return None
    x = x.contiguous()
    out = arena.empty((T, 3 * W), torch.bfloat16, x.device)
    xnew = None
    if o is not None:
        o = o.contiguous()
        bias = bias.to(torch.float32).contiguous()
        xnew = arena.empty_like(x)
    check(lib().npcd_add_ln_split3_bf16(ptr(x), ptr(o), ptr(bias), ptr(gamma.contiguous()), ptr(beta.contiguous()), ptr(xnew), ptr(out), T, W,
                                        float(eps), stream_ptr()), "npcd_add_ln_split3_bf16")
    return (x if xnew is None else xnew), out


class SplitWeight(ctypes.Structure):
    _fields_ = [("w", ctypes.c_void_p), ("fwd", ctypes.c_void_p), ("dgrad", ctypes.c_void_p), ("N", ctypes.c_int), ("K", ctypes.c_int)]


def split_weights(ws):
    require_gpu(*ws)
    if not all(w.is_contiguous() and w.dtype == _f32 for w in ws):
        raise RuntimeError("split_weights takes contiguous fp32 weights (the views of a trainer's flat parameter buffer)")
    out = []
    arr = (SplitWeight * len(ws))()
    for a, w in zip(arr, ws):
        N, K = w.shape
        f, d = arena.empty((N, 3 * K), _bf16, w.device), arena.empty((3 * N, K), _bf16, w.device)
        a.w, a.fwd, a.dgrad, a.N, a.K = w.data_ptr(), f.data_ptr(), d.data_ptr(), N, K
        out.append((f, d))
    check(lib().npcd_split_weights_bf16(ctypes.cast(arr, ctypes.c_void_p), len(ws), stream_ptr()), "npcd_split_weights_bf16")
    return out


def add_ln_split3_stats(x, gamma, beta, o=None, bias=None, eps=1e-5):
    require_gpu(x)
    T, W = x.shape
    if W % 256 or W // 256 not in (1, 2, 3, 4, 8, 16):
        raise RuntimeError(f"npcd_add_ln_split3_stats_bf16 takes widths 256, 512, 768, 1024, 2048 and 4096 (got {W})")
    x = x.contiguous()
    out = arena.empty((T, 3 * W), _bf16, x.device)
    mean, rstd = arena.empty(T, _f32, x.device), arena.empty(T, _f32, x.device)
    xnew = None
    if o is not None:
        o, bias = o.contiguous(), bias.to(_f32).contiguous()
        xnew = arena.empty_like(x)
    check(lib().npcd_add_ln_split3_stats_bf16(ptr(x), ptr(o), ptr(bias), ptr(gamma.contiguous()), ptr(beta.contiguous()), ptr(xnew), ptr(out),
                                              ptr(mean), ptr(rstd), T, W, float(eps), stream_ptr()), "npcd_add_ln_split3_stats_bf16")
    return (x if xnew is None else xnew), out, mean, rstd


def ln_bwd_split3(dy, x, mean, rstd, gamma, dres, dgamma_out, dbeta_out, dcol_out=None, want_split=True, batch=None):
    T, W = x.shape
    dev = x.device
    L = lib()
    nblk = L.npcd_ln_bwd_blocks(T)
    dx = arena.empty((T, W), _f32, dev)
    dx3 = arena.empty((T, 3 * W), _bf16, dev) if want_split else None
    parts = arena.empty((3, nblk + L.npcd_colsum_scratch_rows(), W), _f32, dev)
    check(L.npcd_ln_bwd_split3_bf16(ptr(dy), ptr(x), ptr(mean), ptr(rstd), ptr(gamma), ptr(dres), ptr(dx), ptr(dx3), ptr(parts[0]), ptr(parts[1]),
                                    ptr(parts[2]) if dcol_out is not None else ptr(None), T, W, stream_ptr()), "npcd_ln_bwd_split3_bf16")
    _finish(batch, parts[0], nblk, W, dgamma_out)
    _finish(batch, parts[1], nblk, W, dbeta_out)
    if dcol_out is not None:
        _finish(batch, parts[2], nblk, W, dcol_out)
    return dx, dx3


def split3_colsum(a, colsum_out, h=None, bias=None, batch=None):
    require_gpu(a)
    T, N = a.shape
    L = lib()
    nblk = L.npcd_colsum_blocks(T)
    out = arena.empty((T, 3 * N), _bf16, a.device)
    part = arena.empty((nblk + L.npcd_colsum_scratch_rows(), N), _f32, a.device)
    b = None if bias is None else bias.to(_f32).contiguous()
    check(L.npcd_split3_colsum_bf16(ptr(a), ptr(h), ptr(b), ptr(out), ptr(part), T, N, int(h is not None), stream_ptr()), "npcd_split3_colsum_bf16")
    _finish(batch, part, nblk, N, colsum_out)
    return out


def ddpm_reverse_step(x_t, eps, noise, t, tables, clip=None, want_x0=False):
    require_gpu(x_t)
    x_t, noise, eps = x_t.contiguous(), noise.contiguous(), eps.contiguous()
    B = x_t.shape[0]
    out = arena.empty_like(x_t)
    x0 = arena.empty_like(x_t) if want_x0 else None
    code = {torch.float32: 2, torch.bfloat16: 0}[eps.dtype]
    lo, hi = (float(clip[0]), float(clip[1])) if clip is not None else (0.0, 0.0)
    check(lib().npcd_ddpm_reverse_step(ptr(x_t), ptr(eps), code, ptr(noise), ptr(out), ptr(x0), ptr(t), B, x_t.numel() // B,
                                       *[ptr(tb) for tb in tables], lo, hi, int(clip is not None), stream_ptr()), "npcd_ddpm_reverse_step")
    return out, x0


class SamplerTensor(ctypes.Structure):
    _fields_ = [("x_t", ctypes.c_void_p), ("eps", ctypes.c_void_p), ("noise", ctypes.c_void_p), ("known", ctypes.c_void_p),
                ("out", ctypes.c_void_p), ("x0_out", ctypes.c_void_p), ("per_sample", ctypes.c_int64), ("clip_lo", ctypes.c_float),
                ("clip_hi", ctypes.c_float), ("has_clip", ctypes.c_int32), ("mode", ctypes.c_int32), ("eps_dtype", ctypes.c_int32),
                ("reserved", ctypes.c_int32)]


SAMPLER_REVERSE, SAMPLER_HOLD = 0, 1


def _sampler_tensor(spec, B):
    mode = spec.get("mode", "reverse")
    if mode not in ("reverse", "hold", "keep"):
        raise ValueError("sampler_step: mode is 'reverse', 'hold' or 'keep'")
    hold = mode == "hold"
    keep = [None if spec.get(k) is None else spec[k].contiguous() for k in ("x_t", "eps", "noise", "known")]
    x_t, eps, noise, known = keep
    like = known if hold else x_t
    if like is None:
        like = next((v for v in keep if v is not None), None)
    if like is None or like.shape[0] != B:
        raise RuntimeError("sampler_step: every tensor is [B, ...] with the B of t")
    for v in (x_t, noise, known):
        if v is not None and (v.dtype != _f32 or v.shape != like.shape):
            raise RuntimeError("sampler_step: x_t, noise and known are fp32 tensors of one shape")
    if eps is not None and eps.shape != like.shape:
        raise RuntimeError("sampler_step: eps has the shape of x_t")
    require_gpu(*[v for v in keep if v is not None])
    mask = None
    if mode == "keep":
        mask = spec.get("keep")
        if mask is None or mask.dtype not in (torch.bool, torch.uint8) or mask.dim() != 2 or mask.shape[0] != B or like.dim() < 2 \
                or mask.shape[1] != like.shape[-1]:
            raise RuntimeError("sampler_step: keep is a bool or uint8 [B, N] tensor, the tensors are [B, ..., N]")
        require_gpu(mask)
        mask = mask.contiguous()
        mask = mask.view(torch.uint8) if mask.dtype == torch.bool else mask
        keep.append(mask)
    out = spec.get("out")
# ... 103 lines not shown
```

neural-point-cloud-diffusion_amd/npcd/models/diffusion/fused.py:

```python
import math

import torch

from ...hip import arena as harena
from ...hip import attention as hattn
from ...hip import elementwise as ew
from ...hip import linear as hlin

_bf16, _f32 = torch.bfloat16, torch.float32
_BLOCK_PARAMS = ("ln_1.weight", "ln_1.bias", "attn.c_qkv.weight", "attn.c_qkv.bias", "attn.c_proj.weight", "attn.c_proj.bias",
                 "ln_2.weight", "ln_2.bias", "mlp.c_fc.weight", "mlp.c_fc.bias", "mlp.c_proj.weight", "mlp.c_proj.bias")
_LINEARS = ("attn_c_qkv", "attn_c_proj", "mlp_c_fc", "mlp_c_proj")


import os


def _env_on(name):
    return os.environ.get(name, "") not in ("", "0")


_SPLIT = 0 if os.environ.get("NPCD_NO_GEMM_SPLIT") else 256
_SPLIT_MIN = int(os.environ.get("NPCD_GEMM_SPLIT_MIN", "16000"))
_SPLIT_BIG_FIRST = not os.environ.get("NPCD_GEMM_SPLIT_SMALL_FIRST")
_ATTN_COLSUM = not os.environ.get("NPCD_NO_ATTN_COLSUM")
_SUM_KERNEL = not os.environ.get("NPCD_NO_SUM_KERNEL")
_OWN_WGRAD = _env_on("NPCD_OWN_WGRAD")
_OWN_DGELU = _env_on("NPCD_OWN_DGELU")
_DGRAD_NN = _env_on("NPCD_DGRAD_NN")
_DGRAD_T_MIN_T = int(os.environ.get("NPCD_DGRAD_T_MIN_T", "16000"))


_SPLIT_WIDE_N = int(os.environ.get("NPCD_GEMM_SPLIT_WIDE_N", "4096"))


def _split_gemm(fn, T, N=0):
    wide = _SPLIT_WIDE_N > 0 and N >= _SPLIT_WIDE_N and T > _SPLIT
    Tm = T - T % _SPLIT if (_SPLIT and (T >= _SPLIT_MIN or wide)) else T
    if Tm == 0 or Tm == T:
        fn(slice(0, T))
        return
    if _SPLIT_BIG_FIRST:
        fn(slice(0, Tm))
        fn(slice(Tm, T))
        return
    fn(slice(Tm, T))
    fn(slice(0, Tm))


_LIN128 = not os.environ.get("NPCD_NO_LIN128")
_LIN128_MAX_T = int(os.environ.get("NPCD_LIN128_MAX_T", "4200"))


def _linear(bias, x, w16):
    T = x.shape[0]
    out = harena.empty((T, w16.shape[0]), x.dtype, x.device)
    N, K = w16.shape
    if (_LIN128 and N == 1024 and K == 1024 and T <= _LIN128_MAX_T and x.is_cuda and x.is_contiguous() and w16.is_contiguous()
            and bias.is_contiguous() and x.dtype == w16.dtype == bias.dtype and hlin.supported128(T, N, K)):
        return hlin.linear128_fwd(x, w16, bias, out)
    wt = w16.t()
    _split_gemm(lambda r: torch.addmm(bias, x[r], wt, out=out[r]), T, N)
    return out


def _dgrad(dy, w16, wT=None):
    T = dy.shape[0]
    out = harena.empty((T, w16.shape[1]), dy.dtype, dy.device)
    b = w16 if wT is None else wT.t()
    _split_gemm(lambda r: torch.mm(dy[r], b, out=out[r]), T, w16.shape[1])
    return out


def _wgrad(dy, x, out):
    if _OWN_WGRAD and ew.wgrad(dy, x, out):
        return
    T = dy.shape[0]
    small = out.numel() <= (1 << 20)
    S = 8 if small else 4
    S = min(S, max(1, T // (2048 if small else 4096)))
    while S > 1 and T % S:
        S //= 2
    if S == 1:
        torch.mm(dy.t(), x, out_dtype=_f32, out=out)
        return
    part = torch.bmm(dy.view(S, T // S, -1).transpose(1, 2), x.view(S, T // S, -1), out_dtype=_f32)
    if not (_SUM_KERNEL and ew.sum_slices(part, out)):
        torch.sum(part, dim=0, out=out)


def _parse_wgrad_stream(value):
    if value is None or value == "":
        return True, 20000
    if value == "0":
        return False, 0
    if value == "1":
        return True, 1 << 62
    try:
        return True, int(value)
    except ValueError:
        raise ValueError(f"NPCD_WGRAD_STREAM={value!r}: expected unset, 0 (off), 1 (on at every size) or a token-row limit") from None


_WGRAD_STREAM, _WGRAD_STREAM_MAX_T = _parse_wgrad_stream(os.environ.get("NPCD_WGRAD_STREAM"))
_side = {}


def _side_stream(device):
    s = _side.get(device)
    if s is None:
        s = _side[device] = torch.cuda.Stream(device=device, priority=int(os.environ.get("NPCD_WGRAD_STREAM_PRIO", "0")))
    return s


def _wgrad_side_ok(T):
    return _WGRAD_STREAM and T <= _WGRAD_STREAM_MAX_T


_WGRAD_GROUP = os.environ.get("NPCD_WGRAD_GROUP", "1") != "0"
_WGRAD_GROUP_MAX_T = int(os.environ.get("NPCD_WGRAD_GROUP_MAX_T", "17000"))
_JOIN_PER_BLOCK = _env_on("NPCD_WGRAD_JOIN_PER_BLOCK")
_STEP_ARENA = os.environ.get("NPCD_STEP_ARENA", "1") != "0"
_STEP_ARENA_MAX_T = int(os.environ.get("NPCD_STEP_ARENA_MAX_T", "20000"))


def _parse_wgrad_multiblock(value):
    modes = {None: "on", "": "on", "1": "on", "0": "off", "force": "force"}
    if value not in modes:
        raise ValueError(f"NPCD_WGRAD_MULTIBLOCK={value!r}: expected unset, 0 (off), 1 (on) or force (skip the fill rule)")
    return modes[value]


_WGRAD_MULTIBLOCK = _parse_wgrad_multiblock(os.environ.get("NPCD_WGRAD_MULTIBLOCK"))
_WGRAD_MULTIBLOCK_MIN_T = int(os.environ.get("NPCD_WGRAD_MULTIBLOCK_MIN_T", "20000"))
_multiblock_blocks = {}


def _wgrad_multiblock_blocks(T, W, dtype, device):
    if (_WGRAD_MULTIBLOCK == "off" or T < _WGRAD_MULTIBLOCK_MIN_T or _wgrad_side_ok(T) or device.type != "cuda"
            or dtype not in (torch.bfloat16, torch.float16)):
        return 0
    if _WGRAD_MULTIBLOCK == "force":
        return ew.WGRAD_GROUP_MAX // len(_LINEARS)
    key = (W, device.index)
    if key not in _multiblock_blocks:
        with torch.cuda.device(device):
            _multiblock_blocks[key] = ew.wgrad_group_blocks([(3 * W, W), (W, W), (4 * W, W), (W, 4 * W)])
    return _multiblock_blocks[key]


def _wgrad_fork(pending, device, before=None):
    side = _side_stream(device)
    with torch.cuda.stream(side):
        if before is not None:
            before()
    side.wait_stream(torch.cuda.current_stream())
    with torch.cuda.stream(side):
        for dy, x, out in pending:
            dy.record_stream(side)
            x.record_stream(side)
        if not (_WGRAD_GROUP and pending and pending[0][0].shape[0] <= _WGRAD_GROUP_MAX_T and ew.wgrad_group(pending)):
            for dy, x, out in pending:
                _wgrad(dy, x, out)
    pending.clear()


def _wgrad_join(device):
    torch.cuda.current_stream().wait_stream(_side_stream(device))


def _no_engine():
    return None


import contextlib

_NULL = contextlib.nullcontext()


class _BlockViews:
    fp32_class = False

    def __deepcopy__(self, memo):
        return None

    def __reduce__(self):
        return (_no_engine, ())

    def __init__(self, backbone, flat, reducer=None):
        self.heads = backbone.resblocks[0].attn.heads
        self.width = backbone.width
        self.reducer = reducer
        self._offset = {id(p): off for p, off in zip(flat.params, flat.offsets)}
        self.blocks = []
        for blk in backbone.resblocks:
            named = dict(blk.named_parameters())
            entry = {"params": [named[n] for n in _BLOCK_PARAMS]}
            for n in _BLOCK_PARAMS:
                p = named[n]
                off = self._offset[id(p)]
                key = n.replace(".", "_")
                entry[key] = p.data
                entry[key + "_g"] = flat.grad[off:off + p.numel()].view_as(p)
            self.blocks.append(entry)
        self.block_ranges, self.wait_range = None, None

    def shadow_written(self):
        pass


class FusedBackboneEngine(_BlockViews):

    def __init__(self, backbone, flat, shadow, reducer=None):
        super().__init__(backbone, flat, reducer)
        for blk, entry in zip(backbone.resblocks, self.blocks):
            named = dict(blk.named_parameters())
            for n in _BLOCK_PARAMS:
                p = named[n]
                off = self._offset[id(p)]
                entry[n.replace(".", "_") + "_16"] = shadow[off:off + p.numel()].view_as(p)

        self._flat, self._shadow = flat, shadow
        self.dtype = shadow.dtype
        self._stamped = [p for e in self.blocks for p in e["params"]]
        self._stamp = self._versions()
        self.shadow_epoch = 0
        self._shadowT, self._wT = None, None
        self._wT_stamp = [None] * len(self.blocks)
        self.transposed_refreshes = 0
        self.arena = harena.StepArena() if _STEP_ARENA else None

    def shadow_written(self):
        self.shadow_epoch += 1

    def wants_transposed(self, T):
        return _OWN_DGELU or (not _DGRAD_NN and T >= _DGRAD_T_MIN_T)

    def refresh_transposed(self, bi):
        if self._wT_stamp[bi] == self.shadow_epoch:
            return
        if self._shadowT is None:
            sizes = [entry[k + "_weight_16"].numel() for entry in self.blocks for k in _LINEARS]
            self._shadowT = torch.empty(sum(sizes), dtype=self._shadow.dtype, device=self._shadow.device)
            self._wT, off = [], 0
            for entry in self.blocks:
                views = []
                for k in _LINEARS:
                    N, K = entry[k + "_weight_16"].shape
                    views.append(self._shadowT[off:off + N * K].view(K, N))
                    off += N * K
                self._wT.append(views)
        e = self.blocks[bi]
        hlin.transpose16_group([(e[k + "_weight_16"], v) for k, v in zip(_LINEARS, self._wT[bi])])
        for k, v in zip(_LINEARS, self._wT[bi]):
            e[k + "_weight_16T"] = v
        self._wT_stamp[bi] = self.shadow_epoch
        self.transposed_refreshes += 1

    def _versions(self):
        return [p._version for p in self._stamped]

    def sync_shadow(self, force=False):
        v = self._versions()
        if force or v != self._stamp:
            if self.wait_range is not None:
                self.wait_range()
            for p, off in zip(self._flat.params, self._flat.offsets):
                if p.data_ptr() != self._flat.flat.data_ptr() + off * self._flat.flat.element_size():
                    raise RuntimeError("a parameter of the fused backbone was re-homed outside the trainer's flat buffer "
                                       "(p.data replaced): build a new DiffusionTrainer for this model")
            ew.cast_f32_bf16(self._flat.flat, self._shadow)
            self.shadow_written()
            self._stamp = v

    def __call__(self, x):
        self.sync_shadow()
        return _BackboneFn.apply(x, self)


class InferenceWeights:

    def __init__(self, backbone):
        self.heads = backbone.resblocks[0].attn.heads
        self.params = [[dict(blk.named_parameters())[n] for n in _BLOCK_PARAMS] for blk in backbone.resblocks]
        self.stamp, self.blocks = None, None

    def current(self):
        stamp = [(p._version, p.data_ptr()) for ps in self.params for p in ps]
        if stamp != self.stamp:
            self.blocks = []
            for ps in self.params:
                e = {}
                for n, p in zip(_BLOCK_PARAMS, ps):
                    key = n.replace(".", "_")
                    e[key] = p.data
                    if not n.startswith("ln_"):
                        e[key + "_16"] = p.data.to(_bf16)
                self.blocks.append(e)
            self.stamp = stamp
        return self.blocks


class InferenceWeightsX2:

    def __init__(self, backbone):
        self.heads = backbone.resblocks[0].attn.heads
        self.params = [[dict(blk.named_parameters())[n] for n in _BLOCK_PARAMS] for blk in backbone.resblocks]
        self.stamp, self.blocks = None, None

    def current(self):
        stamp = [(p._version, p.data_ptr()) for ps in self.params for p in ps]
        if stamp != self.stamp:
            self.blocks = []
            for ps in self.params:
                e = {}
                for n, p in zip(_BLOCK_PARAMS, ps):
                    key = n.replace(".", "_")
                    w = p.data.to(_f32)
                    if n.endswith("weight") and not n.startswith("ln_"):
                        hi = w.to(_bf16)
                        lo = (w - hi.float()).to(_bf16)
                        e[key + "_x3"] = torch.cat((hi, hi, lo), dim=1).contiguous()
                    else:
                        e[key] = w.contiguous()
                self.blocks.append(e)
            self.stamp = stamp
        return self.blocks


def backbone_forward_x2(x, blocks, heads):
    import torch.nn.functional as F
    B, n, W = x.shape
    T, d = B * n, W // heads
    scale = 1.0 / math.sqrt(d)
    f32 = _f32

    def lin(a3, e, name):
        return torch.mm(a3, e[name + "_weight_x3"].t(), out_dtype=f32)
    def ln_split(xs, e, ln, o=None, bias=None):
        r = ew.add_ln_split3(xs, e[ln + "_weight"], e[ln + "_bias"], o, bias)
        if r is not None:
            return r
        if o is not None:
            xs = xs + o + bias
        return xs, ew.split3(F.layer_norm(xs, (W,), e[ln + "_weight"], e[ln + "_bias"]))
    with torch.autocast("cuda", enabled=False):
        xs = x.reshape(T, W).contiguous()
        o, ob = None, None
        for e in blocks:
            xs, y1 = ln_split(xs, e, "ln_1", o, ob)
            qkv = lin(y1, e, "attn_c_qkv").add_(e["attn_c_qkv_bias"]).view(B, n, heads, 3 * d)
            a, _ = hattn._fwd(qkv[..., :d], qkv[..., d:2 * d], qkv[..., 2 * d:], scale)
            xs, y2 = ln_split(xs, e, "ln_2", lin(ew.split3(a.reshape(T, W)), e, "attn_c_proj"), e["attn_c_proj_bias"])
            h = lin(y2, e, "mlp_c_fc")
            o, ob = lin(ew.split3(h, bias=e["mlp_c_fc_bias"], gelu=True), e, "mlp_c_proj"), e["mlp_c_proj_bias"]
        xs = xs + o + ob
    return xs.view(B, n, W)


def backbone_forward(x, blocks, heads, dtype=_bf16):
    B, n, W = x.shape
    T, d = B * n, W // heads
    scale = 1.0 / math.sqrt(d)
    with torch.autocast("cuda", enabled=False):
        xs = x.reshape(T, W).contiguous()
        delta = None
        for e in blocks:
            x1, y1, _, _ = ew.add_ln_fwd(xs, delta, e["ln_1_weight"], e["ln_1_bias"], dtype=dtype)
            x_cur = xs if x1 is None else x1
            q4 = _linear(e["attn_c_qkv_bias_16"], y1, e["attn_c_qkv_weight_16"]).view(B, n, heads, 3 * d)
            a, _ = hattn._fwd(q4[..., :d], q4[..., d:2 * d], q4[..., 2 * d:], scale)
            o = _linear(e["attn_c_proj_bias_16"], a.view(T, W), e["attn_c_proj_weight_16"])
            xs, y2, _, _ = ew.add_ln_fwd(x_cur, o, e["ln_2_weight"], e["ln_2_bias"])
            g = ew.gelu_fwd(_linear(e["mlp_c_fc_bias_16"], y2, e["mlp_c_fc_weight_16"]))
            delta = _linear(e["mlp_c_proj_bias_16"], g, e["mlp_c_proj_weight_16"])
        out = xs + delta
    return out.view(B, n, W)


class _BackboneFn(torch.autograd.Function):
    @staticmethod
    def forward(ctx, x, eng):
        B, n, W = x.shape
        T = B * n
        arena = eng.arena if (eng.arena is not None and x.is_cuda and T <= _STEP_ARENA_MAX_T) else None
        token = arena.begin() if arena is not None else 0
        if not token:
            arena = None
        ctx.arena, ctx.arena_token = arena, token
        if arena is None:
            return _BackboneFn._forward(ctx, x, eng)
        ctx.arena_guard = harena.StepGuard(arena, token)
        try:
            with arena.active():
                return _BackboneFn._forward(ctx, x, eng)
        except BaseException:
            arena.end(token)
            raise

    @staticmethod
    def _forward(ctx, x, eng):
        B, n, W = x.shape
        T, H = B * n, eng.heads
        d = W // H
        scale = 1.0 / math.sqrt(d)
        saved = []
        with torch.autocast("cuda", enabled=False):
            xs = x.reshape(T, W).contiguous()
            delta = None
            ctx.transposed = transposed = x.is_cuda and eng.wants_transposed(T)
            for bi, e in enumerate(eng.blocks):
                if eng.wait_range is not None:
                    eng.wait_range(*eng.block_ranges[bi])
                if transposed:
                    eng.refresh_transposed(bi)
                x1, y1, mean1, rstd1 = ew.add_ln_fwd(xs, delta, e["ln_1_weight"], e["ln_1_bias"], dtype=eng.dtype)
                x_cur = xs if x1 is None else x1
                qkv = _linear(e["attn_c_qkv_bias_16"], y1, e["attn_c_qkv_weight_16"])
                q4 = qkv.view(B, n, H, 3 * d)
                a, lse = hattn._fwd(q4[..., :d], q4[..., d:2 * d], q4[..., 2 * d:], scale)
                a = a.view(T, W)
                o = _linear(e["attn_c_proj_bias_16"], a, e["attn_c_proj_weight_16"])
                x2, y2, mean2, rstd2 = ew.add_ln_fwd(x_cur, o, e["ln_2_weight"], e["ln_2_bias"])
                h = _linear(e["mlp_c_fc_bias_16"], y2, e["mlp_c_fc_weight_16"])
                g = ew.gelu_fwd(h)
                delta = _linear(e["mlp_c_proj_bias_16"], g, e["mlp_c_proj_weight_16"])
                saved.append((x_cur, mean1, rstd1, y1, qkv, a, lse, x2, mean2, rstd2, y2, h, g))
                xs = x2
            out = xs + delta
        ctx.eng, ctx.saved, ctx.dims, ctx.scale = eng, saved, (B, n, W, H, d), scale
        return out.view(B, n, W)

    @staticmethod
    def backward(ctx, dout):
        if any(s is None for s in ctx.saved):
            raise RuntimeError("the fused backbone engine does not support retain_graph / double backward: run a new forward "
                               "for every backward")
        arena = ctx.arena
        if arena is None:
            return _BackboneFn._backward(ctx, dout)
        try:
            with arena.active():
                return _BackboneFn._backward(ctx, dout)
        finally:
            arena.end(ctx.arena_token)

    @staticmethod
    def _backward(ctx, dout):
        eng, (B, n, W, H, d), scale = ctx.eng, ctx.dims, ctx.scale
        T = B * n
        with torch.autocast("cuda", enabled=False):
            dx = dout.reshape(T, W).contiguous().float()
            dxb = dx.to(eng.dtype)
            last = eng.blocks[-1]
            last["mlp_c_proj_bias_g"].copy_(dx.sum(dim=0))
            side, pending = _wgrad_side_ok(T), []
            dgrad_t = ctx.transposed and not _DGRAD_NN and T >= _DGRAD_T_MIN_T

            reducing = eng.reducer is not None and eng.reducer.active

            def ready(entry):
                if reducing:
                    for p in entry["params"]:
                        eng.reducer.mark_ready(p)
            group = 0 if side else _wgrad_multiblock_blocks(T, W, eng.dtype, dx.device)
            tail = len(eng.blocks) % group if group else len(eng.blocks)
            queued, queued_blocks = [], []
            for bi in range(len(eng.blocks) - 1, -1, -1):
                e = eng.blocks[bi]
                x_cur, mean1, rstd1, y1, qkv, a, lse, x2, mean2, rstd2, y2, h, g = ctx.saved[bi]
                ctx.saved[bi] = None
                sums = ew.ColsumBatch()
                wg = pending.append if side else queued.append if bi >= tail else (lambda t: _wgrad(*t))
                Tm = T - T % 256
                w2 = e["mlp_c_proj_weight_16"]
                if (_OWN_DGELU and ctx.transposed and Tm > 0 and hlin.supported(Tm, 4 * W, W) and dxb.is_contiguous() and h.is_contiguous()
                        and w2.is_contiguous() and dxb.dtype == w2.dtype == h.dtype and dxb.dtype in (torch.bfloat16, torch.float16)):
                    wT = e["mlp_c_proj_weight_16T"]
                    dh = harena.empty_like(h)
                    extra = ew.lib().npcd_colsum_blocks(T - Tm) if Tm < T else 0
                    _, part, rows = hlin.linear_dgelu_bwd(dxb[:Tm], wT, h[:Tm], out=dh[:Tm], extra_part_rows=extra)
                    if Tm < T:
                        dg = torch.mm(dxb[Tm:], wT.t() if dgrad_t else w2)
                        ew.gelu_bwd(dg, h[Tm:], None, out=dh[Tm:], part_rows=part[rows:])
                        del dg
                    sums.add(part, rows + extra, 4 * W, e["mlp_c_fc_bias_g"])
                    wg((dxb, g, e["mlp_c_proj_weight_g"]))
                    del g, h
                else:
                    dg = _dgrad(dxb, w2, e["mlp_c_proj_weight_16T"] if dgrad_t else None)
                    wg((dxb, g, e["mlp_c_proj_weight_g"]))
                    dh = ew.gelu_bwd(dg, h, e["mlp_c_fc_bias_g"], batch=sums)
                    del dg, g, h
                dy2 = _dgrad(dh, e["mlp_c_fc_weight_16"], e["mlp_c_fc_weight_16T"] if dgrad_t else None)
                wg((dh, y2, e["mlp_c_fc_weight_g"]))
                del dh, y2
                dx2, dx2b = ew.ln_bwd(dy2, x2, mean2, rstd2, e["ln_2_weight"], dx, e["ln_2_weight_g"], e["ln_2_bias_g"],
                                      e["attn_c_proj_bias_g"], batch=sums)
                del dy2, x2, dx, dxb
                da = _dgrad(dx2b, e["attn_c_proj_weight_16"], e["attn_c_proj_weight_16T"] if dgrad_t else None)
                wg((dx2b, a, e["attn_c_proj_weight_g"]))
                dqkv = harena.empty_like(qkv)
                q4, g4 = qkv.view(B, n, H, 3 * d), dqkv.view(B, n, H, 3 * d)
                cpart = hattn.colsum_part_for(g4[..., :d]) if _ATTN_COLSUM else None
                hattn._bwd(q4[..., :d], q4[..., d:2 * d], q4[..., 2 * d:], a.view(B, n, H, d), da.view(B, n, H, d), lse,
                           g4[..., :d], g4[..., d:2 * d], g4[..., 2 * d:], scale, colsum_part=cpart[0] if cpart else None)
                del da, a, qkv, dx2b
                if cpart:
                    sums.add(cpart[0], cpart[1], 3 * W, e["attn_c_qkv_bias_g"])
                else:
                    ew.colsum_bf16(dqkv, e["attn_c_qkv_bias_g"], batch=sums)
                dy1 = _dgrad(dqkv, e["attn_c_qkv_weight_16"], e["attn_c_qkv_weight_16T"] if dgrad_t else None)
                wg((dqkv, y1, e["attn_c_qkv_weight_g"]))
                del dqkv, y1
                prev_bias_g = eng.blocks[bi - 1]["mlp_c_proj_bias_g"] if bi > 0 else None
                with (harena.paused() if bi == 0 else _NULL):
                    dx, dxb = ew.ln_bwd(dy1, x_cur, mean1, rstd1, e["ln_1_weight"], dx2, e["ln_1_weight_g"], e["ln_1_bias_g"],
                                        prev_bias_g, want_bf16=bi > 0, batch=sums)
                del dy1, dx2
                sums.flush()
                if side and _JOIN_PER_BLOCK:
                    if bi + 1 < len(eng.blocks):
                        _wgrad_join(dx.device)
                        ready(eng.blocks[bi + 1])
                    _wgrad_fork(pending, dx.device)
                elif side:
                    above = eng.blocks[bi + 1] if (reducing and bi + 1 < len(eng.blocks)) else None
                    _wgrad_fork(pending, dx.device, before=None if above is None else (lambda: ready(above)))
                elif bi >= tail:
                    queued_blocks.append(e)
                    if (len(eng.blocks) - bi) % group == 0:
                        if not ew.wgrad_group(queued):
                            for t in queued:
                                _wgrad(*t)
                        queued.clear()
                        for qe in queued_blocks:
                            ready(qe)
                        queued_blocks.clear()
                else:
                    ready(e)
            if side:
                _wgrad_join(dx.device)
                ready(eng.blocks[0])
        return dx.view(B, n, W), None


SPLIT_WIDTHS = (256, 512, 768, 1024, 2048)
_X2_LINEARS = ("attn_c_qkv", "attn_c_proj", "mlp_c_fc", "mlp_c_proj")


def x2_supported(width, heads):
    if heads <= 0 or width % heads or width // heads != 64:
        return (f"head dim {width // heads if heads > 0 and width % heads == 0 else width / max(heads, 1)}: the fp32 attention backward "
                f"is built for head dim 64 only")
    if width not in SPLIT_WIDTHS:
        return f"width {width}: the split-operand kernels take widths {', '.join(map(str, SPLIT_WIDTHS))}"
    return None


def _mm_x2(a3, w3):
    return torch.mm(a3, w3, out_dtype=_f32)


def _wgrad_x2(dy3, x3, out):
    T, N = dy3.shape[0], out.shape[0]
    K = out.shape[1]
    d, x = dy3.view(T, 3, N), x3.view(T, 3, K)
    part = harena.empty((3, N, K), _f32, out.device)
    torch.bmm(d[:, 0:2].permute(1, 2, 0), x[:, 1:3].permute(1, 0, 2), out_dtype=_f32, out=part[0:2])
    torch.mm(d[:, 0].t(), x[:, 0], out_dtype=_f32, out=part[2])
    torch.sum(part, dim=0, out=out)


_X2_WGRAD = os.environ.get("NPCD_X2_WGRAD", "library")
if _X2_WGRAD not in ("library", "own"):
    raise ValueError(f"NPCD_X2_WGRAD={_X2_WGRAD!r}: expected library or own")


def _stack_x2(a3, lo_first):
    T, N = a3.shape[0], a3.shape[1] // 3
    v = a3.view(T, 3, N)
    out = harena.empty((3, T, N), _bf16, a3.device)
    if lo_first:
        out[0].copy_(v[:, 1])
        out[1:].copy_(v[:, 0::2].transpose(0, 1))
    else:
        out.copy_(v.transpose(0, 1))
    return out.view(3 * T, N)


def _wgrad_own(pending):
    triples = [(_stack_x2(dy3, False), _stack_x2(x3, True), out) for dy3, x3, out in pending]
    pending.clear()
    if triples[0][0].shape[0] <= _WGRAD_GROUP_MAX_T:
        ok = ew.wgrad_group(triples)
    else:
        ok = all(ew.wgrad(dy, x, out) for dy, x, out in triples)
    if not ok:
        raise RuntimeError("fp32-class weight gradients: the own kernels do not take these shapes (NPCD_X2_WGRAD=library does)")


class FusedBackboneEngineX2(_BlockViews):
    fp32_class = True

    def __init__(self, backbone, flat, reducer=None):
        why = x2_supported(backbone.width, backbone.resblocks[0].attn.heads)
        if why is not None:
            raise ValueError(f"fp32_class training: {why}")
        super().__init__(backbone, flat, reducer)

    def __call__(self, x):
        return _BackboneX2Fn.apply(x, self)


class _BackboneX2Fn(torch.autograd.Function):
    @staticmethod
    def forward(ctx, x, eng):
        B, n, W = x.shape
        T, H = B * n, eng.heads
        d = W // H
        scale = 1.0 / math.sqrt(d)
        saved = []
        with torch.autocast("cuda", enabled=False):
            xs = x.reshape(T, W).contiguous().float()
            o, ob = None, None
            for bi, e in enumerate(eng.blocks):
                if eng.wait_range is not None:
                    eng.wait_range(*eng.block_ranges[bi])
                split = dict(zip(_X2_LINEARS, ew.split_weights([e[k + "_weight"] for k in _X2_LINEARS])))
                x_cur, y1, mean1, rstd1 = ew.add_ln_split3_stats(xs, e["ln_1_weight"], e["ln_1_bias"], o, ob)
                qkv = _mm_x2(y1, split["attn_c_qkv"][0].t()).add_(e["attn_c_qkv_bias"])
                q4 = qkv.view(B, n, H, 3 * d)
                a, lse = hattn._fwd_f32(q4[..., :d], q4[..., d:2 * d], q4[..., 2 * d:], scale, want_lse=True)
                a = a.view(T, W)
                o = _mm_x2(ew.split3(a), split["attn_c_proj"][0].t())
                x2, y2, mean2, rstd2 = ew.add_ln_split3_stats(x_cur, e["ln_2_weight"], e["ln_2_bias"], o, e["attn_c_proj_bias"])
                h = _mm_x2(y2, split["mlp_c_fc"][0].t())
                o, ob = _mm_x2(ew.split3(h, bias=e["mlp_c_fc_bias"], gelu=True), split["mlp_c_proj"][0].t()), e["mlp_c_proj_bias"]
                saved.append((x_cur, mean1, rstd1, y1, qkv, a, lse, x2, mean2, rstd2, y2, h, {k: v[1] for k, v in split.items()}))
                del split
                xs = x2
            out = xs + o + ob
        ctx.eng, ctx.saved, ctx.dims, ctx.scale = eng, saved, (B, n, W, H, d), scale
        return out.view(B, n, W)

    @staticmethod
    def backward(ctx, dout):
        if any(s is None for s in ctx.saved):
            raise RuntimeError("the fused backbone engine does not support retain_graph / double backward: run a new forward "
                               "for every backward")
        eng, (B, n, W, H, d), scale = ctx.eng, ctx.dims, ctx.scale
        T = B * n
        with torch.autocast("cuda", enabled=False):
            dx = dout.reshape(T, W).contiguous().float()
            eng.blocks[-1]["mlp_c_proj_bias_g"].copy_(dx.sum(dim=0))
            dx3 = ew.split3(dx)
            reducing = eng.reducer is not None and eng.reducer.active
            for bi in range(len(eng.blocks) - 1, -1, -1):
                e = eng.blocks[bi]
                x_cur, mean1, rstd1, y1, qkv, a, lse, x2, mean2, rstd2, y2, h, wd = ctx.saved[bi]
                ctx.saved[bi] = None
                sums = ew.ColsumBatch()
                pending = []
                wg = (lambda *t: pending.append(t)) if _X2_WGRAD == "own" else _wgrad_x2
                dg = _mm_x2(dx3, wd["mlp_c_proj"])
                wg(dx3, ew.split3(h, bias=e["mlp_c_fc_bias"], gelu=True), e["mlp_c_proj_weight_g"])
                dh3 = ew.split3_colsum(dg, e["mlp_c_fc_bias_g"], h=h, bias=e["mlp_c_fc_bias"], batch=sums)
                del dg, h
                dy2 = _mm_x2(dh3, wd["mlp_c_fc"])
                wg(dh3, y2, e["mlp_c_fc_weight_g"])
                del dh3, y2
                dx2, dx2_3 = ew.ln_bwd_split3(dy2, x2, mean2, rstd2, e["ln_2_weight"], dx, e["ln_2_weight_g"], e["ln_2_bias_g"],
                                              e["attn_c_proj_bias_g"], batch=sums)
                del dy2, x2, dx, dx3
                da = _mm_x2(dx2_3, wd["attn_c_proj"])
                wg(dx2_3, ew.split3(a), e["attn_c_proj_weight_g"])
                del dx2_3
                dqkv = torch.empty_like(qkv)
                q4, g4, a4 = qkv.view(B, n, H, 3 * d), dqkv.view(B, n, H, 3 * d), a.view(B, n, H, d)
                hattn._bwd_f32(q4[..., :d], q4[..., d:2 * d], q4[..., 2 * d:], a4, da.view(B, n, H, d), lse,
                               g4[..., :d], g4[..., d:2 * d], g4[..., 2 * d:], scale)
                del da, a, qkv, lse
                dqkv3 = ew.split3_colsum(dqkv, e["attn_c_qkv_bias_g"], batch=sums)
                del dqkv
                dy1 = _mm_x2(dqkv3, wd["attn_c_qkv"])
                wg(dqkv3, y1, e["attn_c_qkv_weight_g"])
                del dqkv3, y1
                prev_bias_g = eng.blocks[bi - 1]["mlp_c_proj_bias_g"] if bi > 0 else None
                dx, dx3 = ew.ln_bwd_split3(dy1, x_cur, mean1, rstd1, e["ln_1_weight"], dx2, e["ln_1_weight_g"], e["ln_1_bias_g"],
                                           prev_bias_g, want_split=bi > 0, batch=sums)
                del dy1, dx2
                if pending:
                    _wgrad_own(pending)
                sums.flush()
                if reducing:
                    for p in e["params"]:
                        eng.reducer.mark_ready(p)
        return dx.view(B, n, W), None
```

neural-point-cloud-diffusion_amd/npcd/models/diffusion/transformer.py:

```python
import math
import os
from typing import Tuple

import torch
import torch.nn as nn
import torch.nn.functional as F

from ...hip.attention import attention_qkvpacked

_NO_FAST_GLUE = bool(os.environ.get("NPCD_NO_FAST_GLUE"))


def timestep_embedding(t: torch.Tensor, dim: int, max_period: float = 10000.0) -> torch.Tensor:
    half = dim // 2
    j = torch.arange(half, dtype=torch.float32, device=t.device)
    freqs = torch.exp(j * (-math.log(max_period)) / half)
    ang = t.reshape(-1, 1) * freqs.reshape(1, -1)
    emb = torch.cat((torch.cos(ang), torch.sin(ang)), dim=1)
    if dim & 1:
        emb = F.pad(emb, (0, 1))
    return emb


def _normal_init(linear: nn.Linear, std: float):
    nn.init.normal_(linear.weight, std=std)
    nn.init.zeros_(linear.bias)


class QKVMultiheadAttention(nn.Module):

    def __init__(self, *, heads: int, dropout: float = 0.0, use_flash_attn: bool = True):
        super().__init__()
        if dropout:
            raise NotImplementedError("attention dropout is 0 everywhere in the reference")
        self.heads = heads
        self.use_flash_attn = use_flash_attn

    def forward(self, qkv: torch.Tensor) -> torch.Tensor:
        return attention_qkvpacked(qkv, self.heads)


class MultiheadAttention(nn.Module):
    def __init__(self, *, width: int, heads: int, init_scale: float = 1.0, use_flash_attn: bool = True):
        super().__init__()
        self.width, self.heads = width, heads
        self.c_qkv = nn.Linear(width, 3 * width)
        self.c_proj = nn.Linear(width, width)
        self.attention = QKVMultiheadAttention(heads=heads, use_flash_attn=use_flash_attn)
        _normal_init(self.c_qkv, init_scale)
        _normal_init(self.c_proj, init_scale)

    def forward(self, x):
        return self.c_proj(self.attention(self.c_qkv(x)))


class MLP(nn.Module):
    def __init__(self, *, width: int, init_scale: float = 1.0):
        super().__init__()
        self.width = width
        self.c_fc = nn.Linear(width, 4 * width)
        self.c_proj = nn.Linear(4 * width, width)
        _normal_init(self.c_fc, init_scale)
        _normal_init(self.c_proj, init_scale)

    def forward(self, x):
        return self.c_proj(F.gelu(self.c_fc(x)))


class ResidualAttentionBlock(nn.Module):

    def __init__(self, *, width: int, heads: int, init_scale: float = 1.0, use_flash_attn: bool = True):
        super().__init__()
        self.attn = MultiheadAttention(width=width, heads=heads, init_scale=init_scale, use_flash_attn=use_flash_attn)
        self.ln_1 = nn.LayerNorm(width)
        self.ln_2 = nn.LayerNorm(width)
        self.mlp = MLP(width=width, init_scale=init_scale)

    def forward(self, x):
        x = x + self.attn(self.ln_1(x))
        return x + self.mlp(self.ln_2(x))


class Transformer(nn.Module):
    def __init__(self, *, width: int, layers: int, heads: int, init_scale: float = 0.25, use_flash_attn: bool = True):
        super().__init__()
        self.width, self.layers = width, layers
        std = init_scale * math.sqrt(1.0 / width)
        self.resblocks = nn.ModuleList(
            ResidualAttentionBlock(width=width, heads=heads, init_scale=std, use_flash_attn=use_flash_attn)
            for _ in range(layers))
        self.fused_engine = None
        self._infer_weights = None
        self._infer_weights_x2 = None
        self.fp32_class = False

    def forward(self, x):
        eng = self.fused_engine
        if eng is not None and eng.fp32_class:
            if x.is_cuda and x.dtype == torch.float32 and torch.is_grad_enabled() and not torch.is_autocast_enabled():
                return eng(x)
            if eng.wait_range is not None:
                eng.wait_range()
            eng = None
        if x.is_cuda and x.dtype == torch.float32 and torch.is_autocast_enabled():
            act = torch.get_autocast_dtype("cuda")
            if torch.is_grad_enabled():
                if eng is not None and eng.dtype == act:
                    return eng(x)
            elif eng is not None and eng.dtype == act:
                from . import fused
                if eng.wait_range is not None:
                    eng.wait_range()
                eng.sync_shadow()
                return fused.backbone_forward(x, eng.blocks, eng.heads, eng.dtype)
            elif eng is None and act == torch.bfloat16:
                from . import fused
                if self._infer_weights is None:
                    self._infer_weights = fused.InferenceWeights(self)
                return fused.backbone_forward(x, self._infer_weights.current(), self._infer_weights.heads)
        if eng is not None and eng.wait_range is not None:
            eng.wait_range()
        if (self.fp32_class and x.is_cuda and x.dtype == torch.float32 and not torch.is_autocast_enabled() and not torch.is_grad_enabled()
                and self.width // self.resblocks[0].attn.heads == 64 and self.width % 8 == 0):
            from . import fused
            if self._infer_weights_x2 is None:
                self._infer_weights_x2 = fused.InferenceWeightsX2(self)
            return fused.backbone_forward_x2(x, self._infer_weights_x2.current(), self._infer_weights_x2.heads)
        for blk in self.resblocks:
            x = blk(x)
        return x


class _TimeTokenCat(torch.autograd.Function):

    @staticmethod
    def forward(ctx, temb, tokens, bias):
        B, N, W = tokens.shape
        h = torch.empty((B, N + 1, W), dtype=tokens.dtype, device=tokens.device)
        h[:, 0] = temb
        h[:, 1:] = tokens
        ctx.bias_dtype = bias.dtype
        return h

    @staticmethod
    def backward(ctx, dh):
        from ...hip import elementwise as ew
        dh = dh.contiguous()
        B, n, W = dh.shape
        db = None
        if ctx.needs_input_grad[2]:
            db = torch.empty(W, dtype=torch.float32, device=dh.device)
            ew.colsum_bf16(dh.view(B * n, W), db)
            db -= dh[:, 0].float().sum(dim=0)
            db = db.to(ctx.bias_dtype)
        return dh[:, 0], dh[:, 1:], db


class _LayerNormToBF16(torch.autograd.Function):

    @staticmethod
    def forward(ctx, x, gamma, beta, eps):
        from ...hip import elementwise as ew
        B, n, W = x.shape
        x2 = x.reshape(B * n, W).contiguous()
        _, y, mean, rstd = ew.add_ln_fwd(x2, None, gamma, beta, eps=eps, dtype=torch.get_autocast_dtype("cuda"))
        ctx.save_for_backward(x2, mean, rstd, gamma)
        return y.view(B, n, W)

    @staticmethod
    def backward(ctx, dy):
        from ...hip import elementwise as ew
        x2, mean, rstd, gamma = ctx.saved_tensors
        B, n, W = dy.shape
        dgamma, dbeta = torch.empty(W, dtype=torch.float32, device=dy.device), torch.empty(W, dtype=torch.float32, device=dy.device)
        dx, _ = ew.ln_bwd(dy.reshape(B * n, W).contiguous(), x2, mean, rstd, gamma, None, dgamma, dbeta, want_bf16=False)
        return dx.view(B, n, W), dgamma.to(gamma.dtype), dbeta.to(gamma.dtype), None


class NPCDTransformer(nn.Module):

    def __init__(self, *, coords_dim: int, feats_dim: int, width: int = 512, layers: int = 12, heads: int = 8,
                 init_scale: float = 0.25, use_flash_attn: bool = True):
        super().__init__()
        self.coords_dim, self.feats_dim = coords_dim, feats_dim
        self.input_channels = self.output_channels = coords_dim + feats_dim
        self.time_embed = MLP(width=width, init_scale=init_scale * math.sqrt(1.0 / width))
        self.ln_pre = nn.LayerNorm(width)
        self.backbone = Transformer(width=width, layers=layers, heads=heads, init_scale=init_scale,
                                    use_flash_attn=use_flash_attn)
        self.ln_post = nn.LayerNorm(width)
        self.input_proj = nn.Linear(self.input_channels, width)
        self.output_proj = nn.Linear(width, self.output_channels)
        nn.init.zeros_(self.output_proj.weight)
        nn.init.zeros_(self.output_proj.bias)

    def forward(self, coords: torch.Tensor, feats: torch.Tensor, t: torch.Tensor) -> Tuple[torch.Tensor, torch.Tensor]:
        x = torch.cat((coords, feats), dim=1).transpose(1, 2)
        temb = self.time_embed(timestep_embedding(t, self.backbone.width))
        if (x.is_cuda and torch.is_grad_enabled() and torch.is_autocast_enabled()
                and torch.get_autocast_dtype("cuda") in (torch.bfloat16, torch.float16) and self.backbone.width % 8 == 0 and not _NO_FAST_GLUE):
            tokens = F.linear(x, self.input_proj.weight, self.input_proj.bias.detach())
            h = _TimeTokenCat.apply(temb.to(tokens.dtype), tokens, self.input_proj.bias)
        else:
            tokens = self.input_proj(x)
            h = torch.cat((temb.unsqueeze(1).to(tokens.dtype), tokens), dim=1)
        h = self.backbone(self.ln_pre(h))
        W = h.shape[-1]
        if (h.is_cuda and h.dtype == torch.float32 and torch.is_grad_enabled() and torch.is_autocast_enabled() and W % 4 == 0 and W <= 2048
                and torch.get_autocast_dtype("cuda") in (torch.bfloat16, torch.float16) and self.ln_post.weight.dtype == torch.float32
                and not _NO_FAST_GLUE):
            h = _LayerNormToBF16.apply(h, self.ln_post.weight, self.ln_post.bias, self.ln_post.eps)
        else:
            h = self.ln_post(h)
        eps = self.output_proj(h[:, 1:]).transpose(1, 2)
        return eps[:, :self.coords_dim], eps[:, self.coords_dim:]
```

Before: 12.85 steps/s.

## Fuse embedding concat into ln_pre and ln_post head into fused transformer engine

Adds an embed+LayerNorm kernel that reads the time token and point tokens directly, with no concatenated tensor, and computes the input-bias gradient in its backward. It also folds the final residual add and ln_post into the fused transformer engine's last step. That kernel writes only the point rows in compact bf16, so the separate slice/cast and the backward LN pass are dropped. The goal is to remove several elementwise launches and full-activation round trips at the model head and tail. The cost is more complex autograd plumbing and extra colsum ordering fields.

```diff
diff --git a/include/npcd_hip.h b/include/npcd_hip.h
--- a/include/npcd_hip.h
+++ b/include/npcd_hip.h
@@ -144,14 +144,26 @@
 int npcd_ln_bwd_dt(const void* dy, const float* x, const float* mean, const float* rstd, const float* gamma,
                    const float* dres, float* dx, void* dxb, float* part_gamma, float* part_beta,
                    float* part_col, int T, int W, int dtype, void* stream);
+int npcd_add_ln_fwd_points(const float* x_in, const void* delta, const float* gamma, const float* beta, float* x_out, void* y,
+                           float* mean, float* rstd, int T, int W, int seq, float eps, int dtype, void* stream);
+int npcd_ln_bwd_points(const void* dy, const float* x, const float* mean, const float* rstd, const float* gamma,
+                       const float* dres, float* dx, void* dxb, float* part_gamma, float* part_beta, float* part_col, int T, int W,
+                       int seq, int dtype, void* stream);
+int npcd_embed_ln_fwd(const void* tokens, const void* temb, const float* gamma, const float* beta, float* y, float* mean,
+                      float* rstd, int B, int N, int W, float eps, int dtype, void* stream);
+int npcd_embed_ln_bwd(const float* dy, const void* tokens, const void* temb, const float* mean, const float* rstd,
+                      const float* gamma, void* dtokens, void* dtemb, float* part_gamma, float* part_beta, float* part_col,
+                      int B, int N, int W, int dtype, void* stream);
 int npcd_colsum_scratch_rows(void);
 int npcd_colsum_finalize(const float* part, int nblk, int N, float* out, int accumulate, void* stream);
 #define NPCD_COLSUM_MAX_JOBS 8
 typedef struct NpcdColsumJob {
     const float* part;
     float* out;
-    int nblk, N, accumulate, reserved;
+    int nblk, N, accumulate;
+    int order;
 } NpcdColsumJob;
+#define NPCD_COLSUM_PAIRWISE 1
 int npcd_colsum_finalize_batch(const NpcdColsumJob* jobs, int njobs, void* stream);
 int npcd_gelu_fwd_dt(const void* h, void* g, int64_t numel, int dtype, void* stream);
 int npcd_colsum_blocks(int T);
diff --git a/neural-point-cloud-diffusion_amd/csrc/elementwise.hip b/neural-point-cloud-diffusion_amd/csrc/elementwise.hip
--- a/neural-point-cloud-diffusion_amd/csrc/elementwise.hip
+++ b/neural-point-cloud-diffusion_amd/csrc/elementwise.hip
@@ -20,11 +20,11 @@
 __device__ __forceinline__ f32x4 bf16x4_to_f32(bf16x4 v) { return to_f32(v); }
 __device__ __forceinline__ bf16x4 f32_to_bf16x4(f32x4 v) { return from_f32<__bf16>(v); }
 
-template <class E, int NCH>
-__global__ __launch_bounds__(256) void add_ln_fwd_kernel(const float* __restrict__ x_in, const E* __restrict__ delta,
-                                                         const float* __restrict__ gamma, const float* __restrict__ beta,
-                                                         float* __restrict__ x_out, E* __restrict__ y, float* __restrict__ mean,
-                                                         float* __restrict__ rstd, int T, int W, float eps) {
+template <class E, int NCH, bool POINTS>
+__device__ __forceinline__ void add_ln_fwd_rows(const float* __restrict__ x_in, const E* __restrict__ delta,
+                                                const float* __restrict__ gamma, const float* __restrict__ beta,
+                                                float* __restrict__ x_out, E* __restrict__ y, float* __restrict__ mean,
+                                                float* __restrict__ rstd, int T, int W, float eps, int seq) {
     using e4 = typename V<E>::x4;
     const int lane = threadIdx.x & 63, wave = threadIdx.x >> 6;
     const int NW = gridDim.x * 4;
@@ -85,13 +85,32 @@
 #pragma unroll
         for (int ch = 0; ch < NCH; ++ch) {
             const int c = ch * 256 + lane * 4;
-            if (c < W) *reinterpret_cast<e4*>(y + base + c) = from_f32<E>((v[ch] - mu) * rs * gm[ch] + bt[ch]);
+            if (c < W) {
+                const e4 o = from_f32<E>((v[ch] - mu) * rs * gm[ch] + bt[ch]);
+                if (!POINTS) *reinterpret_cast<e4*>(y + base + c) = o;
+                else if (row % seq != 0) *reinterpret_cast<e4*>(y + (int64_t)(row - row / seq - 1) * W + c) = o;
+            }
         }
         if (lane == 0) {
             mean[row] = mu;
             rstd[row] = rs;
         }
     }
+}
+
+template <class E, int NCH>
+__global__ __launch_bounds__(256) void add_ln_fwd_kernel(const float* __restrict__ x_in, const E* __restrict__ delta,
+                                                         const float* __restrict__ gamma, const float* __restrict__ beta,
+                                                         float* __restrict__ x_out, E* __restrict__ y, float* __restrict__ mean,
+                                                         float* __restrict__ rstd, int T, int W, float eps) {
+    add_ln_fwd_rows<E, NCH, false>(x_in, delta, gamma, beta, x_out, y, mean, rstd, T, W, eps, 0);
+}
+template <class E, int NCH>
+__global__ __launch_bounds__(256) void add_ln_fwd_points_kernel(const float* __restrict__ x_in, const E* __restrict__ delta,
+                                                                const float* __restrict__ gamma, const float* __restrict__ beta,
+                                                                float* __restrict__ x_out, E* __restrict__ y, float* __restrict__ mean,
+                                                                float* __restrict__ rstd, int T, int W, float eps, int seq) {
+    add_ln_fwd_rows<E, NCH, true>(x_in, delta, gamma, beta, x_out, y, mean, rstd, T, W, eps, seq);
 }
 
 static inline int ln_rows_per_wave(int T) {
@@ -100,12 +119,12 @@
     return 16;
 }
 
-template <class E, int NCH, class D = E, bool SPLIT = false>
-__global__ __launch_bounds__(256, 2) void ln_bwd_kernel(const D* __restrict__ dy, const float* __restrict__ x, const float* __restrict__ mean,
-                                                     const float* __restrict__ rstd, const float* __restrict__ gamma,
-                                                     const float* __restrict__ dres, float* __restrict__ dx, E* __restrict__ dxb,
-                                                     float* __restrict__ part_gamma, float* __restrict__ part_beta,
-                                                     float* __restrict__ part_col, int T, int W, int rows_per_wave) {
+template <class E, int NCH, class D, bool SPLIT, bool POINTS>
+__device__ __forceinline__ void ln_bwd_rows(const D* __restrict__ dy, const float* __restrict__ x, const float* __restrict__ mean,
+                                            const float* __restrict__ rstd, const float* __restrict__ gamma,
+                                            const float* __restrict__ dres, float* __restrict__ dx, E* __restrict__ dxb,
+                                            float* __restrict__ part_gamma, float* __restrict__ part_beta,
+                                            float* __restrict__ part_col, int T, int W, int rows_per_wave, int seq) {
     using e4 = typename V<D>::x4;
     extern __shared__ __attribute__((aligned(16))) unsigned char dsmem[];
     float* red = reinterpret_cast<float*>(dsmem);
@@ -126,7 +145,9 @@
         for (int ch = 0; ch < NCH; ++ch) {
             const int c = ch * 256 + lane * 4;
             if (c < W) {
-                dyr[ch] = *reinterpret_cast<const e4*>(dy + base + c);
+                if (!POINTS) dyr[ch] = *reinterpret_cast<const e4*>(dy + base + c);
+                else if (row % seq != 0) dyr[ch] = *reinterpret_cast<const e4*>(dy + (int64_t)(row - row / seq - 1) * W + c);
+                else dyr[ch] = e4{0, 0, 0, 0};
                 xr[ch] = *reinterpret_cast<const f32x4*>(x + base + c);
                 if (dres) rr2[ch] = *reinterpret_cast<const f32x4*>(dres + base + c);
             }
@@ -202,6 +223,189 @@
     float* outs[3] = {part_gamma, part_beta, part_col};
     for (int q = 0; q < 3; ++q) {
         if (!outs[q]) continue;
+        for (int c = threadIdx.x; c < W; c += 256) {
+            const float* p = red + q * 4 * W + c;
+            outs[q][(int64_t)blockIdx.x * W + c] = (p[0] + p[W]) + (p[2 * W] + p[3 * W]);
+        }
+    }
+}
+
+template <class E, int NCH, class D = E, bool SPLIT = false>
+__global__ __launch_bounds__(256, 2) void ln_bwd_kernel(const D* __restrict__ dy, const float* __restrict__ x, const float* __restrict__ mean,
+                                                     const float* __restrict__ rstd, const float* __restrict__ gamma,
+                                                     const float* __restrict__ dres, float* __restrict__ dx, E* __restrict__ dxb,
+                                                     float* __restrict__ part_gamma, float* __restrict__ part_beta,
+                                                     float* __restrict__ part_col, int T, int W, int rows_per_wave) {
+    ln_bwd_rows<E, NCH, D, SPLIT, false>(dy, x, mean, rstd, gamma, dres, dx, dxb, part_gamma, part_beta, part_col, T, W, rows_per_wave, 0);
+}
+template <class E, int NCH>
+__global__ __launch_bounds__(256, 2) void ln_bwd_points_kernel(const E* __restrict__ dy, const float* __restrict__ x,
+                                                            const float* __restrict__ mean, const float* __restrict__ rstd,
+                                                            const float* __restrict__ gamma, const float* __restrict__ dres,
+                                                            float* __restrict__ dx, E* __restrict__ dxb, float* __restrict__ part_gamma,
+                                                            float* __restrict__ part_beta, float* __restrict__ part_col, int T, int W,
+                                                            int rows_per_wave, int seq) {
+    ln_bwd_rows<E, NCH, E, false, true>(dy, x, mean, rstd, gamma, dres, dx, dxb, part_gamma, part_beta, part_col, T, W, rows_per_wave, seq);
+}
+
+template <class E>
+__device__ __forceinline__ E* embed_row(E* tokens, E* temb, int row, int N, int W) {
+    const int b = row / (N + 1), j = row - b * (N + 1);
+    return j == 0 ? temb + (int64_t)b * W : tokens + ((int64_t)b * N + (j - 1)) * W;
+}
+
+template <class E, int NCH>
+__global__ __launch_bounds__(256) void embed_ln_fwd_kernel(const E* __restrict__ tokens, const E* __restrict__ temb,
+                                                           const float* __restrict__ gamma, const float* __restrict__ beta,
+                                                           float* __restrict__ y, float* __restrict__ mean, float* __restrict__ rstd,
+                                                           int T, int N, int W, float eps) {
+    using e4 = typename V<E>::x4;
+    const int lane = threadIdx.x & 63, wave = threadIdx.x >> 6;
+    const int NW = gridDim.x * 4;
+    int row = blockIdx.x * 4 + wave;
+    if (row >= T) return;
+    f32x4 gm[NCH], bt[NCH], v[NCH];
+    e4 nx[NCH];
+#pragma unroll
+    for (int ch = 0; ch < NCH; ++ch) {
+        const int c = ch * 256 + lane * 4;
+        gm[ch] = bt[ch] = f32x4{0.f, 0.f, 0.f, 0.f};
+        nx[ch] = e4{0, 0, 0, 0};
+        if (c < W) {
+            gm[ch] = *reinterpret_cast<const f32x4*>(gamma + c);
+            bt[ch] = *reinterpret_cast<const f32x4*>(beta + c);
+        }
+    }
+    auto load_row = [&](int r) {
+        const E* src = embed_row(tokens, temb, r, N, W);
+#pragma unroll
+        for (int ch = 0; ch < NCH; ++ch) {
+            const int c = ch * 256 + lane * 4;
+            if (c < W) nx[ch] = *reinterpret_cast<const e4*>(src + c);
+        }
+    };
+    load_row(row);
+    for (; row < T; row += NW) {
+        const int64_t base = (int64_t)row * W;
+        float s = 0.f;
+#pragma unroll
+        for (int ch = 0; ch < NCH; ++ch) v[ch] = to_f32(nx[ch]);
+        if (row + NW < T) load_row(row + NW);
+#pragma unroll
+        for (int ch = 0; ch < NCH; ++ch) {
+            const int c = ch * 256 + lane * 4;
+            if (c < W) s += (v[ch][0] + v[ch][1]) + (v[ch][2] + v[ch][3]);
+        }
+        const float mu = wave_sum64(s) / (float)W;
+        float q = 0.f;
+#pragma unroll
+        for (int ch = 0; ch < NCH; ++ch) {
+            const int c = ch * 256 + lane * 4;
+            if (c < W) {
+                const f32x4 d = v[ch] - mu;
+                q += (d[0] * d[0] + d[1] * d[1]) + (d[2] * d[2] + d[3] * d[3]);
+            }
+        }
+        const float rs = rsqrtf(wave_sum64(q) / (float)W + eps);
+#pragma unroll
+        for (int ch = 0; ch < NCH; ++ch) {
+            const int c = ch * 256 + lane * 4;
+            if (c < W) *reinterpret_cast<f32x4*>(y + base + c) = (v[ch] - mu) * rs * gm[ch] + bt[ch];
+        }
+        if (lane == 0) {
+            mean[row] = mu;
+            rstd[row] = rs;
+        }
+    }
+}
+
+template <class E, int NCH>
+__global__ __launch_bounds__(256, 2) void embed_ln_bwd_kernel(const float* __restrict__ dy, const E* __restrict__ tokens,
+                                                              const E* __restrict__ temb, const float* __restrict__ mean,
+                                                              const float* __restrict__ rstd, const float* __restrict__ gamma,
+                                                              E* __restrict__ dtokens, E* __restrict__ dtemb,
+                                                              float* __restrict__ part_gamma, float* __restrict__ part_beta,
+                                                              float* __restrict__ part_col, int T, int N, int W, int rows_per_wave) {
+    using e4 = typename V<E>::x4;
+    extern __shared__ __attribute__((aligned(16))) unsigned char dsmem[];
+    float* red = reinterpret_cast<float*>(dsmem);
+    const int lane = threadIdx.x & 63, wave = threadIdx.x >> 6;
+    f32x4 ag[NCH], ab[NCH], ac[NCH];
+#pragma unroll
+    for (int ch = 0; ch < NCH; ++ch) ag[ch] = ab[ch] = ac[ch] = f32x4{0.f, 0.f, 0.f, 0.f};
+    const int row0 = blockIdx.x * 4 + wave, NW = gridDim.x * 4;
+    const int nrows = row0 < T ? min(rows_per_wave, (T - row0 + NW - 1) / NW) : 0;
+    f32x4 dyA[NCH], dyB[NCH];
+    e4 xA[NCH], xB[NCH];
+    float muA = 0.f, rsA = 0.f, muB = 0.f, rsB = 0.f;
+    auto load_row = [&](int row, f32x4 (&dyr)[NCH], e4 (&xr)[NCH], float& mu, float& rs) {
+        const int64_t base = (int64_t)row * W;
+        const E* src = embed_row(tokens, temb, row, N, W);
+        mu = mean[row];
+        rs = rstd[row];
+#pragma unroll
+        for (int ch = 0; ch < NCH; ++ch) {
+            const int c = ch * 256 + lane * 4;
+            if (c < W) {
+                dyr[ch] = *reinterpret_cast<const f32x4*>(dy + base + c);
+                xr[ch] = *reinterpret_cast<const e4*>(src + c);
+            }
+        }
+    };
+    if (nrows > 0) load_row(row0, dyA, xA, muA, rsA);
+    for (int rr = 0; rr < nrows; ++rr) {
+        const int row = row0 + rr * NW;
+        if (rr + 1 < nrows) load_row(row + NW, dyB, xB, muB, rsB);
+        const float mu = muA, rs = rsA;
+        f32x4 gy[NCH], xh[NCH];
+        float s1 = 0.f, s2 = 0.f;
+#pragma unroll
+        for (int ch = 0; ch < NCH; ++ch) {
+            const int c = ch * 256 + lane * 4;
+            gy[ch] = xh[ch] = f32x4{0.f, 0.f, 0.f, 0.f};
+            if (c < W) {
+                const f32x4 d = dyA[ch];
+                xh[ch] = (to_f32(xA[ch]) - mu) * rs;
+                ag[ch] += d * xh[ch];
+                ab[ch] += d;
+                gy[ch] = d * *reinterpret_cast<const f32x4*>(gamma + c);
+                const f32x4 t = gy[ch] * xh[ch];
+                s1 += (gy[ch][0] + gy[ch][1]) + (gy[ch][2] + gy[ch][3]);
+                s2 += (t[0] + t[1]) + (t[2] + t[3]);
+            }
+        }
+        const float c1 = wave_sum64(s1) / (float)W, c2 = wave_sum64(s2) / (float)W;
+        const bool token = row % (N + 1) != 0;
+        E* dst = embed_row(dtokens, dtemb, row, N, W);
+#pragma unroll
+        for (int ch = 0; ch < NCH; ++ch) {
+            const int c = ch * 256 + lane * 4;
+            if (c < W) {
+                const e4 o = from_f32<E>((gy[ch] - c1 - xh[ch] * c2) * rs);
+                *reinterpret_cast<e4*>(dst + c) = o;
+                if (token) ac[ch] += to_f32(o);
+            }
+        }
+#pragma unroll
+        for (int ch = 0; ch < NCH; ++ch) {
+            dyA[ch] = dyB[ch];
+            xA[ch] = xB[ch];
+        }
+        muA = muB;
+        rsA = rsB;
+    }
+#pragma unroll
+    for (int ch = 0; ch < NCH; ++ch) {
+        const int c = ch * 256 + lane * 4;
+        if (c < W) {
+            *reinterpret_cast<f32x4*>(red + (0 * 4 + wave) * W + c) = ag[ch];
+            *reinterpret_cast<f32x4*>(red + (1 * 4 + wave) * W + c) = ab[ch];
+            *reinterpret_cast<f32x4*>(red + (2 * 4 + wave) * W + c) = ac[ch];
+        }
+    }
+    __syncthreads();
+    float* outs[3] = {part_gamma, part_beta, part_col};
+    for (int q = 0; q < 3; ++q) {
         for (int c = threadIdx.x; c < W; c += 256) {
             const float* p = red + q * 4 * W + c;
             outs[q][(int64_t)blockIdx.x * W + c] = (p[0] + p[W]) + (p[2 * W] + p[3 * W]);
@@ -258,7 +462,18 @@
     const float* __restrict__ src = two ? fb.job[j].part + (int64_t)nblk * N : fb.job[j].part;
     const int nrows = two ? kFinSlices : nblk;
     float s = 0.f;
-    for (int k = 0; k < nrows; ++k) s += src[(int64_t)k * N + c];
+    if (two && fb.job[j].order == NPCD_COLSUM_PAIRWISE) {
+        float v[kFinSlices];
+#pragma unroll
+        for (int k = 0; k < kFinSlices; ++k) v[k] = src[(int64_t)k * N + c];
+#pragma unroll
+        for (int w = 1; w < kFinSlices; w *= 2)
+#pragma unroll
+            for (int k = 0; k < kFinSlices; k += 2 * w) v[k] += v[k + w];
+        s = v[0];
+    } else {
+        for (int k = 0; k < nrows; ++k) s += src[(int64_t)k * N + c];
+    }
     float* __restrict__ out = fb.job[j].out;
     out[c] = fb.job[j].accumulate ? out[c] + s : s;
 }
@@ -971,6 +1186,120 @@
     return NPCD_OK;
 }
 
+static inline bool al8(const void* p) { return (reinterpret_cast<uintptr_t>(p) & 7) == 0; }
+
+extern "C" int npcd_add_ln_fwd_points(const float* x_in, const void* delta, const float* gamma, const float* beta, float* x_out, void* y,
+                                      float* mean, float* rstd, int T, int W, int seq, float eps, int dtype, void* stream) {
+    if (!x_in || !gamma || !beta || !y || !mean || !rstd || T <= 0 || W <= 0 || seq < 2 || T % seq != 0) return NPCD_ERR_ARG;
+    if (W % 4 != 0 || W > 256 * kMaxChunks || !dt16(dtype)) return NPCD_ERR_UNSUPPORTED;
+    if (!al16(x_in) || !al16(gamma) || !al16(beta) || (x_out && !al16(x_out)) || !al8(y) || (delta && !al8(delta))) return NPCD_ERR_ARG;
+#define NPCD_LAUNCH_LN_FWD_P(E, NCH)                                                                                                       \
+    hipLaunchKernelGGL((add_ln_fwd_points_kernel<E, NCH>), dim3(ln_fwd_blocks(T)), dim3(256), 0, static_cast<hipStream_t>(stream), x_in, \
+                       static_cast<const E*>(delta), gamma, beta, x_out, static_cast<E*>(y), mean, rstd, T, W, eps, seq)
+#define NPCD_LN_FWD_P_W(E)                          \
+    do {                                            \
+        if (W <= 256) NPCD_LAUNCH_LN_FWD_P(E, 1);       \
+        else if (W <= 512) NPCD_LAUNCH_LN_FWD_P(E, 2);  \
+        else if (W <= 1024) NPCD_LAUNCH_LN_FWD_P(E, 4); \
+        else NPCD_LAUNCH_LN_FWD_P(E, 8);                \
+    } while (0)
+    if (dtype == NPCD_BF16) NPCD_LN_FWD_P_W(__bf16);
+    else NPCD_LN_FWD_P_W(_Float16);
+#undef NPCD_LN_FWD_P_W
+#undef NPCD_LAUNCH_LN_FWD_P
+    NPCD_HIP_CHECK(hipGetLastError());
+    return NPCD_OK;
+}
+
+extern "C" int npcd_ln_bwd_points(const void* dy, const float* x, const float* mean, const float* rstd, const float* gamma,
+                                  const float* dres, float* dx, void* dxb, float* part_gamma, float* part_beta, float* part_col, int T, int W,
+                                  int seq, int dtype, void* stream) {
+    if (!dy || !x || !mean || !rstd || !gamma || !dx || T <= 0 || W <= 0 || seq < 2 || T % seq != 0) return NPCD_ERR_ARG;
+    if (W % 4 != 0 || W > 256 * kMaxChunks || !dt16(dtype)) return NPCD_ERR_UNSUPPORTED;
+    if (!al8(dy) || !al16(x) || !al16(gamma) || !al16(dx) || (dres && !al16(dres)) || (dxb && !al8(dxb))) return NPCD_ERR_ARG;
+    const int nblk = npcd_ln_bwd_blocks(T);
+    const size_t lds = (size_t)3 * 4 * W * sizeof(float);
+    hipStream_t st = static_cast<hipStream_t>(stream);
+    static DynLds lds_attr_b, lds_attr_h;
+    if (dtype == NPCD_BF16) NPCD_HIP_CHECK(lds_attr_b.ensure(reinterpret_cast<const void*>(ln_bwd_points_kernel<__bf16, 8>), 3 * 4 * 2048 * 4));
+    else NPCD_HIP_CHECK(lds_attr_h.ensure(reinterpret_cast<const void*>(ln_bwd_points_kernel<_Float16, 8>), 3 * 4 * 2048 * 4));
+#define NPCD_LAUNCH_LN_BWD_P(E, NCH)                                                                                                     \
+    hipLaunchKernelGGL((ln_bwd_points_kernel<E, NCH>), dim3(nblk), dim3(256), lds, st, static_cast<const E*>(dy), x, mean, rstd, gamma, \
+                       dres, dx, static_cast<E*>(dxb), part_gamma, part_beta, part_col, T, W, ln_rows_per_wave(T), seq)
+#define NPCD_LN_BWD_P_W(E)                          \
+    do {                                            \
+        if (W <= 256) NPCD_LAUNCH_LN_BWD_P(E, 1);       \
+        else if (W <= 512) NPCD_LAUNCH_LN_BWD_P(E, 2);  \
+        else if (W <= 1024) NPCD_LAUNCH_LN_BWD_P(E, 4); \
+        else NPCD_LAUNCH_LN_BWD_P(E, 8);                \
+    } while (0)
+    if (dtype == NPCD_BF16) NPCD_LN_BWD_P_W(__bf16);
+    else NPCD_LN_BWD_P_W(_Float16);
+#undef NPCD_LN_BWD_P_W
+#undef NPCD_LAUNCH_LN_BWD_P
+    NPCD_HIP_CHECK(hipGetLastError());
+    return NPCD_OK;
+}
+static inline bool embed_rows_ok(int B, int N) { return B > 0 && N > 0 && (int64_t)B * (N + 1) <= 0x7fffffff; }
+
+extern "C" int npcd_embed_ln_fwd(const void* tokens, const void* temb, const float* gamma, const float* beta, float* y, float* mean,
+                                 float* rstd, int B, int N, int W, float eps, int dtype, void* stream) {
+    if (!tokens || !temb || !gamma || !beta || !y || !mean || !rstd || !embed_rows_ok(B, N) || W <= 0) return NPCD_ERR_ARG;
+    if (W % 4 != 0 || W > 256 * kMaxChunks || !dt16(dtype)) return NPCD_ERR_UNSUPPORTED;
+    if (!al8(tokens) || !al8(temb) || !al16(gamma) || !al16(beta) || !al16(y)) return NPCD_ERR_ARG;
+    const int T = B * (N + 1);
+#define NPCD_LAUNCH_EMBED_FWD(E, NCH)                                                                                                \
+    hipLaunchKernelGGL((embed_ln_fwd_kernel<E, NCH>), dim3(ln_fwd_blocks(T)), dim3(256), 0, static_cast<hipStream_t>(stream),        \
+                       static_cast<const E*>(tokens), static_cast<const E*>(temb), gamma, beta, y, mean, rstd, T, N, W, eps)
+#define NPCD_EMBED_FWD_W(E)                          \
+    do {                                             \
+        if (W <= 256) NPCD_LAUNCH_EMBED_FWD(E, 1);       \
+        else if (W <= 512) NPCD_LAUNCH_EMBED_FWD(E, 2);  \
+        else if (W <= 1024) NPCD_LAUNCH_EMBED_FWD(E, 4); \
+        else NPCD_LAUNCH_EMBED_FWD(E, 8);                \
+    } while (0)
+    if (dtype == NPCD_BF16) NPCD_EMBED_FWD_W(__bf16);
+    else NPCD_EMBED_FWD_W(_Float16);
+#undef NPCD_EMBED_FWD_W
+#undef NPCD_LAUNCH_EMBED_FWD
+    NPCD_HIP_CHECK(hipGetLastError());
+    return NPCD_OK;
+}
+
+extern "C" int npcd_embed_ln_bwd(const float* dy, const void* tokens, const void* temb, const float* mean, const float* rstd,
+                                 const float* gamma, void* dtokens, void* dtemb, float* part_gamma, float* part_beta, float* part_col,
+                                 int B, int N, int W, int dtype, void* stream) {
+    if (!dy || !tokens || !temb || !mean || !rstd || !gamma || !dtokens || !dtemb || !part_gamma || !part_beta || !part_col ||
+        !embed_rows_ok(B, N) || W <= 0)
+        return NPCD_ERR_ARG;
+    if (W % 4 != 0 || W > 256 * kMaxChunks || !dt16(dtype)) return NPCD_ERR_UNSUPPORTED;
+    if (!al16(dy) || !al8(tokens) || !al8(temb) || !al16(gamma) || !al8(dtokens) || !al8(dtemb)) return NPCD_ERR_ARG;
+    const int T = B * (N + 1);
+    const int nblk = npcd_ln_bwd_blocks(T);
+    const size_t lds = (size_t)3 * 4 * W * sizeof(float);
+    hipStream_t st = static_cast<hipStream_t>(stream);
+    static DynLds lds_attr_b, lds_attr_h;
+    if (dtype == NPCD_BF16) NPCD_HIP_CHECK(lds_attr_b.ensure(reinterpret_cast<const void*>(embed_ln_bwd_kernel<__bf16, 8>), 3 * 4 * 2048 * 4));
+    else NPCD_HIP_CHECK(lds_attr_h.ensure(reinterpret_cast<const void*>(embed_ln_bwd_kernel<_Float16, 8>), 3 * 4 * 2048 * 4));
+#define NPCD_LAUNCH_EMBED_BWD(E, NCH)                                                                                                  \
+    hipLaunchKernelGGL((embed_ln_bwd_kernel<E, NCH>), dim3(nblk), dim3(256), lds, st, dy, static_cast<const E*>(tokens),              \
+                       static_cast<const E*>(temb), mean, rstd, gamma, static_cast<E*>(dtokens), static_cast<E*>(dtemb), part_gamma, \
+                       part_beta, part_col, T, N, W, ln_rows_per_wave(T))
+#define NPCD_EMBED_BWD_W(E)                          \
+    do {                                             \
+        if (W <= 256) NPCD_LAUNCH_EMBED_BWD(E, 1);       \
+        else if (W <= 512) NPCD_LAUNCH_EMBED_BWD(E, 2);  \
+        else if (W <= 1024) NPCD_LAUNCH_EMBED_BWD(E, 4); \
+        else NPCD_LAUNCH_EMBED_BWD(E, 8);                \
+    } while (0)
+    if (dtype == NPCD_BF16) NPCD_EMBED_BWD_W(__bf16);
+    else NPCD_EMBED_BWD_W(_Float16);
+#undef NPCD_EMBED_BWD_W
+#undef NPCD_LAUNCH_EMBED_BWD
+    NPCD_HIP_CHECK(hipGetLastError());
+    return NPCD_OK;
+}
+
 
 __global__ __launch_bounds__(1024) void colsum_onepass_kernel(FinBatch fb) {
     __shared__ float red[16][64];
@@ -1009,7 +1338,7 @@
     bool any_two_stage = false;
     int n1 = 0, n2 = 0;
     for (int j = 0; j < njobs; ++j) {
-        if (!jobs[j].part || !jobs[j].out || jobs[j].nblk <= 0 || jobs[j].N <= 0) return NPCD_ERR_ARG;
+        if (!jobs[j].part || !jobs[j].out || jobs[j].nblk <= 0 || jobs[j].N <= 0 || (jobs[j].order & ~NPCD_COLSUM_PAIRWISE)) return NPCD_ERR_ARG;
         fb.job[j] = jobs[j];
         fb.first1[j] = n1;
         fb.first2[j] = n2;
@@ -1033,7 +1362,7 @@
 
 extern "C" int npcd_colsum_finalize(const float* part, int nblk, int N, float* out, int accumulate, void* stream) {
     NpcdColsumJob job;
-    job.part = part; job.out = out; job.nblk = nblk; job.N = N; job.accumulate = accumulate; job.reserved = 0;
+    job.part = part; job.out = out; job.nblk = nblk; job.N = N; job.accumulate = accumulate; job.order = 0;
     return npcd_colsum_finalize_batch(&job, 1, stream);
 }
 
diff --git a/neural-point-cloud-diffusion_amd/npcd/hip/__init__.py b/neural-point-cloud-diffusion_amd/npcd/hip/__init__.py
--- a/neural-point-cloud-diffusion_amd/npcd/hip/__init__.py
+++ b/neural-point-cloud-diffusion_amd/npcd/hip/__init__.py
@@ -81,6 +81,10 @@
     "npcd_colsum_blocks": (c_int, [c_int]),
     "npcd_add_ln_fwd_dt": (c_int, [_P] * 8 + [c_int, c_int, c_float, c_int, _P]),
     "npcd_ln_bwd_dt": (c_int, [_P] * 11 + [c_int, c_int, c_int, _P]),
+    "npcd_add_ln_fwd_points": (c_int, [_P] * 8 + [c_int, c_int, c_int, c_float, c_int, _P]),
+    "npcd_ln_bwd_points": (c_int, [_P] * 11 + [c_int, c_int, c_int, c_int, _P]),
+    "npcd_embed_ln_fwd": (c_int, [_P] * 7 + [c_int, c_int, c_int, c_float, c_int, _P]),
+    "npcd_embed_ln_bwd": (c_int, [_P] * 11 + [c_int, c_int, c_int, c_int, _P]),
     "npcd_gelu_fwd_dt": (c_int, [_P, _P, c_int64, c_int, _P]),
     "npcd_gelu_bwd_dt": (c_int, [_P, _P, _P, _P, c_int, c_int, c_int, _P]),
     "npcd_colsum_dt": (c_int, [_P, _P, c_int, c_int, c_int, _P]),
diff --git a/neural-point-cloud-diffusion_amd/npcd/hip/elementwise.py b/neural-point-cloud-diffusion_amd/npcd/hip/elementwise.py
--- a/neural-point-cloud-diffusion_amd/npcd/hip/elementwise.py
+++ b/neural-point-cloud-diffusion_amd/npcd/hip/elementwise.py
@@ -31,16 +31,16 @@
     def __init__(self):
         self.jobs = []
 
-    def add(self, part, nblk, N, out, accumulate=False):
-        self.jobs.append((part, nblk, N, out, accumulate))
+    def add(self, part, nblk, N, out, accumulate=False, pairwise=False):
+        self.jobs.append((part, nblk, N, out, accumulate, pairwise))
 
     def flush(self):
         L, s = lib(), stream_ptr()
         for i in range(0, len(self.jobs), MAX_JOBS):
             chunk = self.jobs[i:i + MAX_JOBS]
             arr = (ColsumJob * len(chunk))()
-            for a, (part, nblk, N, out, acc) in zip(arr, chunk):
-                a.part, a.out, a.nblk, a.N, a.accumulate, a.reserved = part.data_ptr(), out.data_ptr(), nblk, N, int(acc), 0
+            for a, (part, nblk, N, out, acc, pairwise) in zip(arr, chunk):
+                a.part, a.out, a.nblk, a.N, a.accumulate, a.reserved = part.data_ptr(), out.data_ptr(), nblk, N, int(acc), int(pairwise)
             check(L.npcd_colsum_finalize_batch(ctypes.cast(arr, ctypes.c_void_p), len(chunk), s), "npcd_colsum_finalize_batch")
         self.jobs = []
 
@@ -52,23 +52,31 @@
         check(lib().npcd_colsum_finalize(ptr(part), nblk, N, ptr(out), 0, stream_ptr()), "npcd_colsum_finalize")
 
 
-def add_ln_fwd(x_in, delta, gamma, beta, eps=1e-5, want_sum=True, dtype=_bf16):
+def add_ln_fwd(x_in, delta, gamma, beta, eps=1e-5, want_sum=True, dtype=_bf16, seq=0):
     require_gpu(x_in)
     T, W = x_in.shape
     dev = x_in.device
     if delta is not None:
         dtype = delta.dtype
     x_out = arena.empty_like(x_in) if (delta is not None and want_sum) else None
-    y = arena.empty((T, W), dtype, dev)
+    if seq:
+        with arena.paused():
+            y = torch.empty((T // seq, seq - 1, W), dtype=dtype, device=dev)
+    else:
+        y = arena.empty((T, W), dtype, dev)
     mean = arena.empty(T, _f32, dev)
     rstd = arena.empty(T, _f32, dev)
+    if seq:
+        check(lib().npcd_add_ln_fwd_points(ptr(x_in), ptr(delta), ptr(gamma), ptr(beta), ptr(x_out), ptr(y), ptr(mean), ptr(rstd), T, W, seq,
+                                           float(eps), dtype_code(y), stream_ptr()), "npcd_add_ln_fwd_points")
+        return x_out, y, mean, rstd
     check(_timed("add_ln_fwd" if delta is not None and want_sum else "ln_fwd",
                  lambda: lib().npcd_add_ln_fwd_dt(ptr(x_in), ptr(delta), ptr(gamma), ptr(beta), ptr(x_out), ptr(y), ptr(mean), ptr(rstd), T, W,
                                                   float(eps), dtype_code(y), stream_ptr())), "npcd_add_ln_fwd")
     return x_out, y, mean, rstd
 
 
-def ln_bwd(dy, x, mean, rstd, gamma, dres, dgamma_out, dbeta_out, dcol_out=None, want_bf16=True, batch=None):
+def ln_bwd(dy, x, mean, rstd, gamma, dres, dgamma_out, dbeta_out, dcol_out=None, want_bf16=True, batch=None, seq=0):
     T, W = x.shape
     dev = x.device
     L = lib()
@@ -77,15 +85,49 @@
     dxb = arena.empty((T, W), dy.dtype, dev) if want_bf16 else None
     parts = arena.empty((3, nblk + L.npcd_colsum_scratch_rows(), W), _f32, dev)
     full = dres is not None and want_bf16
-    check(_timed("ln_bwd" if full else "ln_bwd_partial",
-                 lambda: L.npcd_ln_bwd_dt(ptr(dy), ptr(x), ptr(mean), ptr(rstd), ptr(gamma), ptr(dres), ptr(dx), ptr(dxb), ptr(parts[0]),
-                                          ptr(parts[1]), ptr(parts[2]) if dcol_out is not None else ptr(None), T, W, dtype_code(dy), stream_ptr())),
-          "npcd_ln_bwd")
+    pcol = ptr(parts[2]) if dcol_out is not None else ptr(None)
+    if seq:
+        check(L.npcd_ln_bwd_points(ptr(dy), ptr(x), ptr(mean), ptr(rstd), ptr(gamma), ptr(dres), ptr(dx), ptr(dxb), ptr(parts[0]), ptr(parts[1]),
+                                   pcol, T, W, seq, dtype_code(dy), stream_ptr()), "npcd_ln_bwd_points")
+    else:
+        check(_timed("ln_bwd" if full else "ln_bwd_partial",
+                     lambda: L.npcd_ln_bwd_dt(ptr(dy), ptr(x), ptr(mean), ptr(rstd), ptr(gamma), ptr(dres), ptr(dx), ptr(dxb), ptr(parts[0]),
+                                              ptr(parts[1]), pcol, T, W, dtype_code(dy), stream_ptr())),
+              "npcd_ln_bwd")
     _finish(batch, parts[0], nblk, W, dgamma_out)
     _finish(batch, parts[1], nblk, W, dbeta_out)
     if dcol_out is not None:
         _finish(batch, parts[2], nblk, W, dcol_out)
     return dx, dxb
+
+
+def embed_ln_fwd(tokens, temb, gamma, beta, eps=1e-5):
+    require_gpu(tokens, temb)
+    B, N, W = tokens.shape
+    dev = tokens.device
+    y = torch.empty((B, N + 1, W), dtype=_f32, device=dev)
+    mean = torch.empty(B * (N + 1), dtype=_f32, device=dev)
+    rstd = torch.empty(B * (N + 1), dtype=_f32, device=dev)
+    check(lib().npcd_embed_ln_fwd(ptr(tokens), ptr(temb), ptr(gamma), ptr(beta), ptr(y), ptr(mean), ptr(rstd), B, N, W, float(eps),
+                                  dtype_code(tokens), stream_ptr()), "npcd_embed_ln_fwd")
+    return y, mean, rstd
+
+
+def embed_ln_bwd(dy, tokens, temb, mean, rstd, gamma):
+    B, N, W = tokens.shape
+    dev = tokens.device
+    L = lib()
+    nblk = L.npcd_ln_bwd_blocks(B * (N + 1))
+    dtokens, dtemb = torch.empty_like(tokens), torch.empty_like(temb)
+    parts = torch.empty((3, nblk + L.npcd_colsum_scratch_rows(), W), dtype=_f32, device=dev)
+    sums = torch.empty((3, W), dtype=_f32, device=dev)
+    check(L.npcd_embed_ln_bwd(ptr(dy), ptr(tokens), ptr(temb), ptr(mean), ptr(rstd), ptr(gamma), ptr(dtokens), ptr(dtemb), ptr(parts[0]),
+                              ptr(parts[1]), ptr(parts[2]), B, N, W, dtype_code(tokens), stream_ptr()), "npcd_embed_ln_bwd")
+    batch = ColsumBatch()
+    for q in range(3):
+        batch.add(parts[q], nblk, W, sums[q], pairwise=True)
+    batch.flush()
+    return dtokens, dtemb, sums[0], sums[1], sums[2]
 
 
 def gelu_fwd(h):
diff --git a/neural-point-cloud-diffusion_amd/npcd/models/diffusion/fused.py b/neural-point-cloud-diffusion_amd/npcd/models/diffusion/fused.py
--- a/neural-point-cloud-diffusion_amd/npcd/models/diffusion/fused.py
+++ b/neural-point-cloud-diffusion_amd/npcd/models/diffusion/fused.py
@@ -273,9 +273,11 @@
             self.shadow_written()
             self._stamp = v
 
-    def __call__(self, x):
+    def __call__(self, x, head=None):
         self.sync_shadow()
-        return _BackboneFn.apply(x, self)
+        if head is None:
+            return _BackboneFn.apply(x, self, None, None, 0.0)
+        return _BackboneFn.apply(x, self, *head)
 
 
 class InferenceWeights:
@@ -380,9 +382,10 @@
 
 class _BackboneFn(torch.autograd.Function):
     @staticmethod
-    def forward(ctx, x, eng):
+    def forward(ctx, x, eng, gamma, beta, eps):
         B, n, W = x.shape
         T = B * n
+        ctx.head = None if gamma is None else (gamma, beta, eps)
         arena = eng.arena if (eng.arena is not None and x.is_cuda and T <= _STEP_ARENA_MAX_T) else None
         token = arena.begin() if arena is not None else 0
         if not token:
@@ -427,9 +430,14 @@
                 delta = _linear(e["mlp_c_proj_bias_16"], g, e["mlp_c_proj_weight_16"])
                 saved.append((x_cur, mean1, rstd1, y1, qkv, a, lse, x2, mean2, rstd2, y2, h, g))
                 xs = x2
-            out = xs + delta
+            if ctx.head is None:
+                out = (xs + delta).view(B, n, W)
+            else:
+                gamma, beta, eps = ctx.head
+                x3, out, mean3, rstd3 = ew.add_ln_fwd(xs, delta, gamma, beta, eps=eps, seq=n)
+                ctx.head = (x3, mean3, rstd3, gamma)
         ctx.eng, ctx.saved, ctx.dims, ctx.scale = eng, saved, (B, n, W, H, d), scale
-        return out.view(B, n, W)
+        return out
 
     @staticmethod
     def backward(ctx, dout):
@@ -450,10 +458,22 @@
         eng, (B, n, W, H, d), scale = ctx.eng, ctx.dims, ctx.scale
         T = B * n
         with torch.autocast("cuda", enabled=False):
-            dx = dout.reshape(T, W).contiguous().float()
-            dxb = dx.to(eng.dtype)
             last = eng.blocks[-1]
-            last["mlp_c_proj_bias_g"].copy_(dx.sum(dim=0))
+            dgb = None
+            if ctx.head is None:
+                dx = dout.reshape(T, W).contiguous().float()
+                dxb = dx.to(eng.dtype)
+                last["mlp_c_proj_bias_g"].copy_(dx.sum(dim=0))
+            else:
+                x3, mean3, rstd3, gamma = ctx.head
+                ctx.head = None
+                with harena.paused():
+                    dgb = torch.empty((2, W), dtype=torch.float32, device=dout.device)
+                hsums = ew.ColsumBatch()
+                dx, dxb = ew.ln_bwd(dout.to(eng.dtype).contiguous(), x3, mean3, rstd3, gamma, None, dgb[0], dgb[1], last["mlp_c_proj_bias_g"],
+                                    want_bf16=True, batch=hsums, seq=n)
+                hsums.flush()
+                del x3, mean3, rstd3
             side, pending = _wgrad_side_ok(T), []
             dgrad_t = ctx.transposed and not _DGRAD_NN and T >= _DGRAD_T_MIN_T
 
@@ -542,7 +562,9 @@
             if side:
                 _wgrad_join(dx.device)
                 ready(eng.blocks[0])
-        return dx.view(B, n, W), None
+        if dgb is None:
+            return dx.view(B, n, W), None, None, None, None
+        return dx.view(B, n, W), None, dgb[0].to(gamma.dtype), dgb[1].to(gamma.dtype), None
 
 
 SPLIT_WIDTHS = (256, 512, 768, 1024, 2048)
diff --git a/neural-point-cloud-diffusion_amd/npcd/models/diffusion/transformer.py b/neural-point-cloud-diffusion_amd/npcd/models/diffusion/transformer.py
--- a/neural-point-cloud-diffusion_amd/npcd/models/diffusion/transformer.py
+++ b/neural-point-cloud-diffusion_amd/npcd/models/diffusion/transformer.py
@@ -9,6 +9,7 @@
 from ...hip.attention import attention_qkvpacked
 
 _NO_FAST_GLUE = bool(os.environ.get("NPCD_NO_FAST_GLUE"))
+_NO_FUSED_HEAD = bool(os.environ.get("NPCD_NO_FUSED_HEAD"))
 
 
 def timestep_embedding(t: torch.Tensor, dim: int, max_period: float = 10000.0) -> torch.Tensor:
@@ -94,7 +95,13 @@
         self._infer_weights_x2 = None
         self.fp32_class = False
 
-    def forward(self, x):
+    def takes_head(self, x) -> bool:
+        eng = self.fused_engine
+        return (eng is not None and not eng.fp32_class and x.is_cuda and x.dtype == torch.float32 and torch.is_autocast_enabled()
+                and torch.is_grad_enabled() and eng.dtype == torch.get_autocast_dtype("cuda"))
+
+    def forward(self, x, head=None):
+        assert head is None or self.takes_head(x)
         eng = self.fused_engine
         if eng is not None and eng.fp32_class:
             if x.is_cuda and x.dtype == torch.float32 and torch.is_grad_enabled() and not torch.is_autocast_enabled():
@@ -106,7 +113,7 @@
             act = torch.get_autocast_dtype("cuda")
             if torch.is_grad_enabled():
                 if eng is not None and eng.dtype == act:
-                    return eng(x)
+                    return eng(x, head)
             elif eng is not None and eng.dtype == act:
                 from . import fused
                 if eng.wait_range is not None:
@@ -156,6 +163,25 @@
         return dh[:, 0], dh[:, 1:], db
 
 
+class _EmbedLN(torch.autograd.Function):
+
+    @staticmethod
+    def forward(ctx, temb, tokens, bias, gamma, beta, eps):
+        from ...hip import elementwise as ew
+        temb, tokens = temb.contiguous(), tokens.contiguous()
+        y, mean, rstd = ew.embed_ln_fwd(tokens, temb, gamma, beta, eps)
+        ctx.save_for_backward(temb, tokens, mean, rstd, gamma)
+        ctx.bias_dtype = bias.dtype
+        return y
+
+    @staticmethod
+    def backward(ctx, dy):
+        from ...hip import elementwise as ew
+        temb, tokens, mean, rstd, gamma = ctx.saved_tensors
+        dtokens, dtemb, dgamma, dbeta, dbias = ew.embed_ln_bwd(dy.contiguous(), tokens, temb, mean, rstd, gamma)
+        return dtemb, dtokens, dbias.to(ctx.bias_dtype), dgamma.to(gamma.dtype), dbeta.to(gamma.dtype), None
+
+
 class _LayerNormToBF16(torch.autograd.Function):
 
     @staticmethod
@@ -197,20 +223,35 @@
     def forward(self, coords: torch.Tensor, feats: torch.Tensor, t: torch.Tensor) -> Tuple[torch.Tensor, torch.Tensor]:
         x = torch.cat((coords, feats), dim=1).transpose(1, 2)
         temb = self.time_embed(timestep_embedding(t, self.backbone.width))
-        if (x.is_cuda and torch.is_grad_enabled() and torch.is_autocast_enabled()
-                and torch.get_autocast_dtype("cuda") in (torch.bfloat16, torch.float16) and self.backbone.width % 8 == 0 and not _NO_FAST_GLUE):
+        fast = (x.is_cuda and torch.is_grad_enabled() and torch.is_autocast_enabled()
+                and torch.get_autocast_dtype("cuda") in (torch.bfloat16, torch.float16) and self.backbone.width % 8 == 0 and not _NO_FAST_GLUE)
+        if (fast and self.backbone.width <= 2048 and self.ln_pre.weight.dtype == torch.float32 and self.ln_pre.bias.dtype == torch.float32
+                and self.ln_pre.elementwise_affine):
             tokens = F.linear(x, self.input_proj.weight, self.input_proj.bias.detach())
-            h = _TimeTokenCat.apply(temb.to(tokens.dtype), tokens, self.input_proj.bias)
+            h = _EmbedLN.apply(temb.to(tokens.dtype), tokens, self.input_proj.bias, self.ln_pre.weight, self.ln_pre.bias, self.ln_pre.eps)
         else:
-            tokens = self.input_proj(x)
-            h = torch.cat((temb.unsqueeze(1).to(tokens.dtype), tokens), dim=1)
-        h = self.backbone(self.ln_pre(h))
+            if fast:
+                tokens = F.linear(x, self.input_proj.weight, self.input_proj.bias.detach())
+                h = _TimeTokenCat.apply(temb.to(tokens.dtype), tokens, self.input_proj.bias)
+            else:
+                tokens = self.input_proj(x)
+                h = torch.cat((temb.unsqueeze(1).to(tokens.dtype), tokens), dim=1)
+            h = self.ln_pre(h)
         W = h.shape[-1]
-        if (h.is_cuda and h.dtype == torch.float32 and torch.is_grad_enabled() and torch.is_autocast_enabled() and W % 4 == 0 and W <= 2048
+        fast = (h.is_cuda and h.dtype == torch.float32 and torch.is_grad_enabled() and torch.is_autocast_enabled() and W % 4 == 0 and W <= 2048
                 and torch.get_autocast_dtype("cuda") in (torch.bfloat16, torch.float16) and self.ln_post.weight.dtype == torch.float32
-                and not _NO_FAST_GLUE):
-            h = _LayerNormToBF16.apply(h, self.ln_post.weight, self.ln_post.bias, self.ln_post.eps)
+                and not _NO_FAST_GLUE)
+        if (fast and not _NO_FUSED_HEAD and h.shape[1] >= 2 and self.ln_post.bias.dtype == torch.float32 and self.backbone.takes_head(h)):
+            y = self.backbone(h, head=(self.ln_post.weight, self.ln_post.bias, self.ln_post.eps))
+            out = F.linear(y, self.output_proj.weight)
+            eps = (out + self.output_proj.bias.to(out.dtype)).transpose(1, 2)
+            return eps[:, :self.coords_dim], eps[:, self.coords_dim:]
         else:
-            h = self.ln_post(h)
-        eps = self.output_proj(h[:, 1:]).transpose(1, 2)
+            h = self.backbone(h)
+            if fast:
+                h = _LayerNormToBF16.apply(h, self.ln_post.weight, self.ln_post.bias, self.ln_post.eps)
+            else:
+                h = self.ln_post(h)
+            y = h[:, 1:]
+        eps = self.output_proj(y).transpose(1, 2)
         return eps[:, :self.coords_dim], eps[:, self.coords_dim:]
```

Result: no change. 12.94 steps/s, median of 6 (+0.7%).
